# hkchengrex/Cutie

Measured on AMD Instinct MI355X. Metric: frames/sec (480p, 3 objects), higher is better.
Workload: dtype bf16

## Files before the change

### cutie_amd/_lib.py

```python
import ctypes
import os

_HERE = os.path.dirname(os.path.abspath(__file__))
LIB_PATH = os.environ.get('CUTIE_AMD_LIB') or os.path.join(_HERE, 'libcutie_hip.so')
ABI_VERSION = 11
OP_STRUCT_SIZE = 256

_lib = None


class HipLibraryError(RuntimeError):
    pass


def load():
    global _lib
    if _lib is not None:
        return _lib
    if not os.path.exists(LIB_PATH):
        raise HipLibraryError(
            f'{LIB_PATH} not found: build it with `python -c "import __graft_entry__ as g; g.build()"` '
            f'(or `make -C cutie_amd/csrc`).  cutie_amd has no CPU fallback.')
    lib = ctypes.CDLL(LIB_PATH)
    lib.cutie_exec.argtypes = [ctypes.c_void_p, ctypes.c_int, ctypes.c_void_p]
    lib.cutie_exec.restype = ctypes.c_int
    lib.cutie_exec_one.argtypes = [ctypes.c_void_p, ctypes.c_void_p]
    lib.cutie_exec_one.restype = ctypes.c_int
    lib.cutie_graph_capture.argtypes = [ctypes.c_void_p, ctypes.c_int, ctypes.c_void_p]
    lib.cutie_graph_capture.restype = ctypes.c_void_p
    lib.cutie_graph_launch.argtypes = [ctypes.c_void_p, ctypes.c_void_p]
    lib.cutie_graph_launch.restype = ctypes.c_int
    lib.cutie_graph_destroy.argtypes = [ctypes.c_void_p]
    lib.cutie_graph_destroy.restype = None
    lib.cutie_time_ops.argtypes = [ctypes.c_void_p, ctypes.c_int, ctypes.c_int, ctypes.c_void_p]
    lib.cutie_time_ops.restype = ctypes.c_float
    lib.cutie_hip_last_error.argtypes = []
    lib.cutie_hip_last_error.restype = ctypes.c_char_p
    lib.cutie_hip_abi_version.restype = ctypes.c_int
    lib.cutie_op_struct_size.restype = ctypes.c_int
    lib.cutie_hip_build_flags.restype = ctypes.c_int
    if lib.cutie_hip_abi_version() != ABI_VERSION or lib.cutie_op_struct_size() != OP_STRUCT_SIZE:
        raise HipLibraryError(f'{LIB_PATH} is stale (ABI {lib.cutie_hip_abi_version()}, '
                              f'op size {lib.cutie_op_struct_size()}); rebuild it.')
    _lib = lib
    return lib


EXPORTED_SYMBOLS = ['cutie_exec', 'cutie_exec_one', 'cutie_graph_capture', 'cutie_graph_launch',
                    'cutie_graph_destroy', 'cutie_time_ops', 'cutie_hip_last_error',
                    'cutie_hip_abi_version', 'cutie_op_struct_size', 'cutie_hip_build_flags']


def has_diag_kernels():
    return bool(load().cutie_hip_build_flags() & 1)


def has_png_decode():
    return bool(load().cutie_hip_build_flags() & 2)


def has_jpeg_batch():
    return bool(load().cutie_hip_build_flags() & 4)


def has_mixed_lockstep():
    return bool(load().cutie_hip_build_flags() & 8)


def has_track_stats():
    return bool(load().cutie_hip_build_flags() & 16)


class HipExecutor:
    is_mock = False

    def __init__(self):
        import torch
        self.lib = load()
        if not torch.cuda.is_available():
            raise HipLibraryError('no HIP device visible: cutie_amd runs on MI355X only (no CPU fallback).')
        self._torch = torch
        self._raw_stream = getattr(torch._C, '_cuda_getCurrentRawStream', None)
        self.graph_stats = [0, 0]
        self._warned = False

    def stream(self):
        raw = self._raw_stream
        if raw is not None:
            return raw(self._torch.cuda.current_device())
        return self._torch.cuda.current_stream().cuda_stream

    def run(self, arr):
        rc = self.lib.cutie_exec(arr.ctypes.data, len(arr), self.stream())
        if rc != 0:
            raise RuntimeError('cutie_exec failed: ' + self.lib.cutie_hip_last_error().decode())

    def run_on(self, arr, stream):
        rc = self.lib.cutie_exec(arr.ctypes.data, len(arr), stream.cuda_stream)
        if rc != 0:
            raise RuntimeError('cutie_exec failed: ' + self.lib.cutie_hip_last_error().decode())

    GRAPH_CACHE_ENTRIES = 24

    def run_cached(self, arr, cache, head=0):
        if head:
            self.run(arr[:head])
            arr = arr[head:]
        key = arr['p'].tobytes()
        ent = cache.get(key)
        if ent is None:
            if len(cache) >= self.GRAPH_CACHE_ENTRIES:
                old = cache.pop(next(iter(cache)))
                if old not in (0, -1):
                    self.lib.cutie_graph_destroy(old)
            cache[key] = 0
            self.graph_stats[0] += 1
            return self.run(arr)
        if ent == 0:
            ent = self.lib.cutie_graph_capture(arr.ctypes.data, len(arr), self.stream()) or -1
            cache[key] = ent
            if ent == -1 and not self._warned:
                self._warned = True
                import warnings
                warnings.warn('HIP graph capture of a launch plan failed (%s); such plans keep running launch by launch'
                              % self.lib.cutie_hip_last_error().decode())
        if ent == -1:
            self.graph_stats[0] += 1
            return self.run(arr)
        self.graph_stats[1] += 1
        if self.lib.cutie_graph_launch(ent, self.stream()) != 0:
            raise RuntimeError('cutie_graph_launch failed: ' + self.lib.cutie_hip_last_error().decode())

    def time_ops(self, arr, iters):
        ms = self.lib.cutie_time_ops(arr.ctypes.data, len(arr), iters, self.stream())
        if ms < 0:
            raise RuntimeError('cutie_time_ops failed: ' + self.lib.cutie_hip_last_error().decode())
        return ms


_executor = None


def get_executor():
    global _executor
    if _executor is None:
        _executor = HipExecutor()
    return _executor


def set_executor_for_testing(ex):
    global _executor
    _executor = ex
```

### cutie_amd/csrc/api.hip

```cpp
#include "common.h"
#include <stdarg.h>
#include <stdio.h>
#include <string.h>

static thread_local char g_err[512] = "";

void cutie_set_error(const char* fmt, ...) {
    va_list ap;
    va_start(ap, fmt);
    vsnprintf(g_err, sizeof(g_err), fmt, ap);
    va_end(ap);
}

static int dispatch(const cutie_op* op, hipStream_t s) {
    switch (op->kind) {
        case CUTIE_OP_CONV: return launch_conv(op, s);
        case CUTIE_OP_QUERY_INIT: return (op->flags & 1) ? launch_attention(op, s) : launch_elementwise(op, s);
        case CUTIE_OP_QFFN: return launch_qchain(op, s);
        case CUTIE_OP_STEM: return launch_stem(op, s);
        case CUTIE_OP_ATTN_Q2P: case CUTIE_OP_ATTN_SELF: case CUTIE_OP_ATTN_P2Q:
            return (op->flags & 12) ? launch_qchain(op, s) : launch_attention(op, s);
        case CUTIE_OP_AUX_MASK:
            return launch_attention(op, s);
        case CUTIE_OP_KEY_PREP: case CUTIE_OP_AFF_SCORE: case CUTIE_OP_AFF_SELECT: case CUTIE_OP_AFF_READOUT:
            return launch_affinity(op, s);
        case CUTIE_OP_RANK_SELECT: case CUTIE_OP_GATHER_ROWS: case CUTIE_OP_CONSOL_AFF: case CUTIE_OP_CONSOL_READ:
            return launch_bank(op, s);
        default:
            if (op->kind > 0 && op->kind < CUTIE_OP__COUNT) return launch_elementwise(op, s);
            cutie_set_error("cutie_exec: unknown op kind %d", op->kind);
            return -3;
    }
}

extern "C" {

int cutie_exec(const cutie_op* ops, int n, void* stream) {
    hipStream_t s = (hipStream_t)stream;
    for (int k = 0; k < n; ++k) {
        int rc = dispatch(&ops[k], s);
        if (rc != 0) {
            if (rc > 0) cutie_set_error("op %d (kind %d): HIP error %d (%s)", k, ops[k].kind, rc, hipGetErrorString((hipError_t)rc));
            else {
                char tmp[400];
                snprintf(tmp, sizeof(tmp), "%s", g_err);
                cutie_set_error("op %d (kind %d): %s", k, ops[k].kind, tmp);
            }
            return rc > 0 ? -1 : rc;
        }
    }
    return 0;
}

int cutie_exec_one(const cutie_op* op, void* stream) { return cutie_exec(op, 1, stream); }

struct GraphHandle { hipGraph_t graph; hipGraphExec_t exec; };

void* cutie_graph_capture(const cutie_op* ops, int n, void* stream) {
    (void)stream;
    static thread_local hipStream_t cap = nullptr;
    if (!cap && hipStreamCreateWithFlags(&cap, hipStreamNonBlocking) != hipSuccess) {
        cap = nullptr;
        (void)hipGetLastError();
        cutie_set_error("graph: cannot create the capture stream");
        return nullptr;
    }
    hipGraph_t graph = nullptr;
    if (hipStreamBeginCapture(cap, hipStreamCaptureModeThreadLocal) != hipSuccess) {
        (void)hipGetLastError();
        cutie_set_error("graph: begin capture failed");
        return nullptr;
    }
    int rc = cutie_exec(ops, n, (void*)cap);
    hipError_t e = hipStreamEndCapture(cap, &graph);
    if (rc != 0 || e != hipSuccess || !graph) {
        if (graph) hipGraphDestroy(graph);
        if (rc == 0) cutie_set_error("graph: end capture failed (%d)", (int)e);
        (void)hipGetLastError();
        return nullptr;
    }
    hipGraphExec_t exec = nullptr;
    if (hipGraphInstantiate(&exec, graph, nullptr, nullptr, 0) != hipSuccess) {
        hipGraphDestroy(graph);
        (void)hipGetLastError();
        cutie_set_error("graph: instantiate failed");
        return nullptr;
    }
    GraphHandle* h = new GraphHandle{graph, exec};
    return h;
}

int cutie_graph_launch(void* graph, void* stream) {
    GraphHandle* h = (GraphHandle*)graph;
    if (!h) { cutie_set_error("graph: null handle"); return -4; }
    hipError_t e = hipGraphLaunch(h->exec, (hipStream_t)stream);
    if (e != hipSuccess) { cutie_set_error("graph launch: %s", hipGetErrorString(e)); return -1; }
    return 0;
}

void cutie_graph_destroy(void* graph) {
    GraphHandle* h = (GraphHandle*)graph;
    if (!h) return;
    hipGraphExecDestroy(h->exec);
    hipGraphDestroy(h->graph);
    delete h;
}

float cutie_time_ops(const cutie_op* ops, int n, int iters, void* stream) {
    hipStream_t s = (hipStream_t)stream;
    hipEvent_t a, b;
    if (hipEventCreate(&a) != hipSuccess || hipEventCreate(&b) != hipSuccess) { cutie_set_error("time: event create failed"); return -1.f; }
    if (cutie_exec(ops, n, stream) != 0) return -1.f;
    hipEventRecord(a, s);
    for (int it = 0; it < iters; ++it)
        if (cutie_exec(ops, n, stream) != 0) return -1.f;
    hipEventRecord(b, s);
    hipEventSynchronize(b);
    float ms = 0.f;
    hipEventElapsedTime(&ms, a, b);
    hipEventDestroy(a);
    hipEventDestroy(b);
    return ms / (float)iters;
}

const char* cutie_hip_last_error(void) { return g_err; }
int cutie_hip_abi_version(void) { return 11; }
int cutie_op_struct_size(void) { return (int)sizeof(cutie_op); }
int cutie_hip_build_flags(void) {
    const int forms = 2 | 4 | 8 | 16;
#ifdef CUTIE_DIAG
    return forms | 1;
#else
    return forms;
#endif
}

}
```

### cutie_amd/csrc/common.h

```cpp
#pragma once
#include <hip/hip_runtime.h>
#include <stdint.h>
#include "../../include/cutie_hip.h"

typedef unsigned short bf16_t;
typedef __attribute__((ext_vector_type(8))) __bf16 bf16x8;
typedef __attribute__((ext_vector_type(4))) float f32x4;

__device__ __forceinline__ float bf2f(bf16_t v) { return __uint_as_float(((uint32_t)v) << 16); }

typedef __attribute__((ext_vector_type(2))) __bf16 bf16x2_t;
__device__ __forceinline__ bf16_t f2bf(float f) { return __builtin_bit_cast(bf16_t, (__bf16)f); }

__device__ __forceinline__ uint32_t pack_bf2(float a, float b) {
    const bf16x2_t v = {(__bf16)a, (__bf16)b};
    return __builtin_bit_cast(uint32_t, v);
}

__device__ __forceinline__ uint32_t relu_bf2(uint32_t w) {
    uint32_t neg = (w >> 15) & 0x00010001u;
    return w & ~(neg * 0xffffu);
}

__device__ __forceinline__ float sigmoidf_(float x) { return 1.0f / (1.0f + __expf(-x)); }

__device__ __forceinline__ float rows_max(float v) {
    unsigned u = __float_as_uint(v);
    auto r = __builtin_amdgcn_permlane16_swap(u, u, false, false);
    unsigned a = __float_as_uint(fmaxf(__uint_as_float(r[0]), __uint_as_float(r[1])));
    auto r2 = __builtin_amdgcn_permlane32_swap(a, a, false, false);
    return fmaxf(__uint_as_float(r2[0]), __uint_as_float(r2[1]));
}
__device__ __forceinline__ float rows_sum(float v) {
    unsigned u = __float_as_uint(v);
    auto r = __builtin_amdgcn_permlane16_swap(u, u, false, false);
    unsigned a = __float_as_uint(__uint_as_float(r[0]) + __uint_as_float(r[1]));
    auto r2 = __builtin_amdgcn_permlane32_swap(a, a, false, false);
    return __uint_as_float(r2[0]) + __uint_as_float(r2[1]);
}

__device__ __forceinline__ int wave_sum_i32(int v) {
    v += __builtin_amdgcn_update_dpp(0, v, 0xB1, 0xf, 0xf, false);
    v += __builtin_amdgcn_update_dpp(0, v, 0x4E, 0xf, 0xf, false);
    v += __builtin_amdgcn_update_dpp(0, v, 0x141, 0xf, 0xf, false);
    v += __builtin_amdgcn_update_dpp(0, v, 0x140, 0xf, 0xf, false);
    auto r = __builtin_amdgcn_permlane16_swap((unsigned)v, (unsigned)v, false, false);
    const unsigned a = r[0] + r[1];
    auto r2 = __builtin_amdgcn_permlane32_swap(a, a, false, false);
    return (int)(r2[0] + r2[1]);
}

__device__ __forceinline__ float wave_sum(float v) {
#pragma unroll
    for (int o = 32; o > 0; o >>= 1) v += __shfl_xor(v, o, 64);
    return v;
}
__device__ __forceinline__ float wave_sum_dpp(float v) {
    v += __uint_as_float(__builtin_amdgcn_update_dpp(0, (int)__float_as_uint(v), 0xB1, 0xf, 0xf, false));
    v += __uint_as_float(__builtin_amdgcn_update_dpp(0, (int)__float_as_uint(v), 0x4E, 0xf, 0xf, false));
    v += __uint_as_float(__builtin_amdgcn_update_dpp(0, (int)__float_as_uint(v), 0x141, 0xf, 0xf, false));
    v += __uint_as_float(__builtin_amdgcn_update_dpp(0, (int)__float_as_uint(v), 0x140, 0xf, 0xf, false));
    return rows_sum(v);
}
__device__ __forceinline__ float wave_max(float v) {
#pragma unroll
    for (int o = 32; o > 0; o >>= 1) v = fmaxf(v, __shfl_xor(v, o, 64));
    return v;
}

__host__ __device__ __forceinline__ int mixed_count(unsigned word, int clip) { return (int)((word >> (3 * clip)) & 7u); }
__host__ __device__ __forceinline__ int mixed_start(unsigned word, int clip) {
    int s = 0;
    for (int c = 0; c < clip; ++c) s += mixed_count(word, c);
    return s;
}
__host__ __device__ __forceinline__ int mixed_clip_of(unsigned word, int b, int& start) {
    int c = 0, s = 0;
#pragma unroll
    for (int q = 0; q < 7; ++q) {
        const int n = mixed_count(word, c);
        const bool past = b >= s + n;
        s += past ? n : 0;
        c += past ? 1 : 0;
    }
    start = s;
    return c;
}
static inline int mixed_clips(unsigned word, int* objects) {
    int n = 0, total = 0;
    if (word >> 24) { *objects = 0; return 0; }
    while (n < 8 && mixed_count(word, n)) total += mixed_count(word, n++);
    if (n < 8 && (word >> (3 * n))) { *objects = 0; return 0; }
    *objects = total;
    return n;
}

int launch_conv(const cutie_op* op, hipStream_t s);
int launch_elementwise(const cutie_op* op, hipStream_t s);
int launch_attention(const cutie_op* op, hipStream_t s);
int launch_stem(const cutie_op* op, hipStream_t s);
int launch_qchain(const cutie_op* op, hipStream_t s);
int launch_affinity(const cutie_op* op, hipStream_t s);
int launch_bank(const cutie_op* op, hipStream_t s);
int launch_resize_ingest(const cutie_op* op, hipStream_t s);
int launch_jpeg(const cutie_op* op, hipStream_t s);
int launch_png_decode(const cutie_op* op, hipStream_t s);
int launch_png_deflate(const cutie_op* op, int H, int W, hipStream_t s);
int launch_rle_encode(const cutie_op* op, hipStream_t s);
int launch_jf_counts(const cutie_op* op, hipStream_t s);
int launch_jpeg_encode(const cutie_op* op, hipStream_t s);
int launch_matte_composite(const cutie_op* op, hipStream_t s);
int launch_matte_soft(const cutie_op* op, hipStream_t s);
int launch_track_stats(const cutie_op* op, hipStream_t s);
void cutie_set_error(const char* fmt, ...);
```

### cutie_amd/csrc/conv_common.h

```cpp
#pragma once
#include "common.h"

struct ConvParams {
    const bf16_t* x1; const bf16_t* x2; const bf16_t* w; const float* bias; const bf16_t* res; void* y;
    int B, H, W, C1, C2, ldx1, ldx2, OH, OW, Cout, ldy, KH, KW, stride, pad, ldr, Kpad;
    int flags, M, Cin, OHW;
    float* part; int splitk, ldp, Kslice;
    long long* gap; unsigned long long* zero; int nzero;
    const unsigned char* pf; int pf_bytes;
    const unsigned char* pf2; int pf2_bytes;
    int res_grp_rows, res_grp_stride;
};
#define GAP_FIXED_SCALE 16777216.f
#define GAP_ELEM_SHIFT 4
__device__ __forceinline__ long long conv_gapfx(float v) {
    if (__builtin_expect(fabsf(v) < 2048.f, 1)) return (long long)__float2int_rn(v * 1048576.f);
    if (v != v) return 0;
    const float c = fminf(fmaxf(v, -1048576.f), 1048576.f);
    const float hi = truncf(c);
    return (long long)(int)hi * 1048576LL + (long long)__float2int_rn((c - hi) * 1048576.f);
}

typedef __attribute__((ext_vector_type(4))) unsigned int u32x4;
typedef const __attribute__((address_space(1))) u32x4* gptr16;
#define GLOAD16(ptr) (*(gptr16)(ptr))

template <int CPR>
__device__ __forceinline__ int swz(int row) {
    return CPR == 4 ? ((row >> 3) & 1) * 3 : (row & (CPR - 1));
}

__device__ __forceinline__ int conv_res_row(const ConvParams& p, int m) {
    if (!(p.flags & CUTIE_F_RES_BCAST)) return m;
    int r = m % p.OHW;
    if (p.res_grp_rows > 0) r += (m / p.res_grp_rows) * p.res_grp_stride;
    return r;
}

__device__ __forceinline__ void conv_finish(const ConvParams& p, float* v, int m, int ch0) {
    const int act = (p.flags >> CUTIE_ACT_SHIFT) & 7;
    const bool out_f32 = p.flags & CUTIE_F_OUT_F32;
    const bool vec_y = out_f32 ? ((p.ldy & 3) == 0) : ((p.ldy & 7) == 0);
    const bool vec_r = (p.ldr & 7) == 0;
    const bool full = ch0 + 7 < p.Cout;
    if (p.bias) {
        if (full && (reinterpret_cast<uintptr_t>(p.bias) & 15) == 0) {
            const float4 b0 = *reinterpret_cast<const float4*>(p.bias + ch0), b1 = *reinterpret_cast<const float4*>(p.bias + ch0 + 4);
            v[0] += b0.x; v[1] += b0.y; v[2] += b0.z; v[3] += b0.w; v[4] += b1.x; v[5] += b1.y; v[6] += b1.z; v[7] += b1.w;
        } else {
#pragma unroll
            for (int r = 0; r < 8; ++r) if (ch0 + r < p.Cout) v[r] += p.bias[ch0 + r];
        }
    }
    if (p.res) {
        const int mres = conv_res_row(p, m);
        const bf16_t* rp = p.res + (long)mres * p.ldr + ch0;
        if (full && vec_r) {
            const uint4 rr = *reinterpret_cast<const uint4*>(rp);
            v[0] += __uint_as_float(rr.x << 16); v[1] += __uint_as_float(rr.x & 0xffff0000u);
            v[2] += __uint_as_float(rr.y << 16); v[3] += __uint_as_float(rr.y & 0xffff0000u);
            v[4] += __uint_as_float(rr.z << 16); v[5] += __uint_as_float(rr.z & 0xffff0000u);
            v[6] += __uint_as_float(rr.w << 16); v[7] += __uint_as_float(rr.w & 0xffff0000u);
        } else {
#pragma unroll
            for (int r = 0; r < 8; ++r) if (ch0 + r < p.Cout) v[r] += bf2f(rp[r]);
        }
    }
#pragma unroll
    for (int r = 0; r < 8; ++r) {
        if (act == CUTIE_ACT_RELU) v[r] = fmaxf(v[r], 0.f);
        else if (act == CUTIE_ACT_SIGMOID) v[r] = sigmoidf_(v[r]);
        else if (act == CUTIE_ACT_SQ1) v[r] = v[r] * v[r] + 1.f;
    }
    if (out_f32) {
        float* yp = reinterpret_cast<float*>(p.y) + (long)m * p.ldy + ch0;
        if (full && vec_y) {
            *reinterpret_cast<float4*>(yp) = make_float4(v[0], v[1], v[2], v[3]);
            *reinterpret_cast<float4*>(yp + 4) = make_float4(v[4], v[5], v[6], v[7]);
        } else {
#pragma unroll
            for (int r = 0; r < 8; ++r) if (ch0 + r < p.Cout) yp[r] = v[r];
        }
    } else {
        bf16_t* yp = reinterpret_cast<bf16_t*>(p.y) + (long)m * p.ldy + ch0;
        if (full && vec_y) {
            *reinterpret_cast<uint4*>(yp) = make_uint4(pack_bf2(v[0], v[1]), pack_bf2(v[2], v[3]), pack_bf2(v[4], v[5]), pack_bf2(v[6], v[7]));
        } else {
#pragma unroll
            for (int r = 0; r < 8; ++r) if (ch0 + r < p.Cout) yp[r] = f2bf(v[r]);
        }
    }
}

template <int BM, int BN, int BK, int WK>
constexpr int conv_lds_bytes() {
    constexpr int pipe = WK * 2 * (BM + BN) * (BK / 8) * 16, epi = BM * (BN + 4) * 4;
    return pipe > epi ? pipe : epi;
}

__device__ __forceinline__ void conv_preload_args(const ConvParams& p) {
#ifndef CONV_NO_PRELOAD
    asm volatile("" :: "s"(p.x1), "s"(p.w), "s"(p.bias), "s"(p.res), "s"(p.y), "s"(p.zero),
                 "s"(p.B), "s"(p.H), "s"(p.W), "s"(p.C1), "s"(p.C2), "s"(p.ldx1), "s"(p.ldx2), "s"(p.OH), "s"(p.OW), "s"(p.Cout), "s"(p.ldy),
                 "s"(p.KH), "s"(p.KW), "s"(p.stride), "s"(p.pad), "s"(p.ldr), "s"(p.Kpad), "s"(p.flags), "s"(p.M), "s"(p.Cin), "s"(p.OHW),
                 "s"(p.nzero), "s"(gridDim.x), "s"(gridDim.y));
#endif
}

#ifdef CONV_TIMELINE
#define TL_MAX 96
#define TL_BYTES (16 * TL_MAX * 8)
#define TL_DECL(...) unsigned long long* const tlp_ = reinterpret_cast<unsigned long long*>(__VA_ARGS__) + wave * TL_MAX; int tln_ = 0;
#define TL_PUT_(ID, CAP) { if (tln_ < (CAP)) { const unsigned long long t_ = (__builtin_readcyclecounter() << 8) | (unsigned)(ID); if ((threadIdx.x & 63) == 0) tlp_[tln_] = t_; ++tln_; } }
#define TL(ID) TL_PUT_(ID, TL_MAX - 6)
#define TLE(ID) TL_PUT_(ID, TL_MAX)
#define TL_DUMP(LOGICAL, NB, NWAVES)                                                                                        \
    {                                                                                                                       \
        const int slot_ = (LOGICAL) == 0 ? 0 : (LOGICAL) == 1 ? 1 : (LOGICAL) == (NB) / 2 ? 2 : (LOGICAL) == (NB) - 1 ? 3 : -1; \
        if (slot_ >= 0 && p.part) {                                                                                         \
            __builtin_amdgcn_s_waitcnt(0);                                                                                  \
            unsigned long long* o_ = reinterpret_cast<unsigned long long*>(p.part) + ((long)slot_ * 16 + wave) * (TL_MAX + 2); \
            if ((threadIdx.x & 63) == 0) { o_[0] = 0x544c0000ull | (unsigned)tln_; o_[1] = ((unsigned long long)(LOGICAL) << 32) | (unsigned)(NWAVES); } \
            for (int q_ = threadIdx.x & 63; q_ < tln_; q_ += 64) o_[2 + q_] = tlp_[q_];                                     \
        }                                                                                                                   \
    }
#else
#define TL_BYTES 0
#define TL_DECL(...)
#define TL(ID)
#define TLE(ID)
#define TL_DUMP(LOGICAL, NB, NWAVES)
#endif

int launch_conv_dma(const ConvParams& p, int tile, hipStream_t s);
int launch_conv_pc(const ConvParams& p, int tile, hipStream_t s);
```

### cutie_amd/csrc/conv_igemm.hip

```cpp
#include "conv_common.h"

template <int BM, int BN, int WM, int WN, int BK, int S, int OCC, int WK>
__global__ __launch_bounds__(WM * WN * WK * 64) void conv_igemm_kernel(ConvParams p) {
    if (p.flags & CUTIE_F_PRIO) __builtin_amdgcn_s_setprio(1);
    constexpr int NTB = WM * WN * WK * 64;
    constexpr int NT = WM * WN * 64;
    constexpr int CPR = BK / 8;
    constexpr int RPT = NT / CPR;
    constexpr int NX = (BM * CPR) / NT;
    constexpr int NWC = (BN * CPR + NT - 1) / NT;
    constexpr int TM = BM / WM / 16;
    constexpr int TN = BN / WN / 16;
    constexpr int KSUB = BK / 32;
    constexpr int NWRAP = BK == 32 ? 4 : BK / 32;
    static_assert((NT == 256 || NT == 512) && NTB <= 1024 && NX >= 1 && TM >= 1 && TN >= 1 && S >= 2 && (BM * CPR) % NT == 0, "bad tile");
    constexpr int LDC = BN + 4;
    constexpr int GRP_CHUNKS = 2 * (BM + BN) * CPR;
    extern __shared__ __attribute__((aligned(16))) u32x4 smem_raw[];
    const int grp = threadIdx.x / NT;
    u32x4 (*smem)[(BM + BN) * CPR] = reinterpret_cast<u32x4 (*)[(BM + BN) * CPR]>(smem_raw + grp * GRP_CHUNKS);

    const int tid = threadIdx.x % NT, lane = tid & 63, wave = tid >> 6;
    int m0, n0;
    {
// ... 119 lines not shown
                afr[t] = __builtin_bit_cast(bf16x8, smem[buf][(BM + row) * CPR + ((j * 4 + l4) ^ swz<CPR>(row))]); \
            }                                                                                              \
            _Pragma("unroll") for (int a = 0; a < TN; ++a)                                                 \
                _Pragma("unroll") for (int b = 0; b < TM; ++b)                                             \
                    acc[a][b] = __builtin_amdgcn_mfma_f32_16x16x32_bf16(afr[a], bfr[b], acc[a][b], 0, 0, 0); \
        }                                                                                                  \
        if (DO_STORE) STORE_TILE(buf ^ 1, ((U) + 1) % S);                                                  \
        __syncthreads();                                                                                   \
    }
    int ks0 = 0;
    for (; ks0 + 2 * S - 1 <= nk; ks0 += S) {
#pragma unroll
        for (int u = 0; u < S; ++u) K_ITER(ks0 + u, u, true, true)
    }
    for (; ks0 < nk; ks0 += S) {
#pragma unroll
        for (int u = 0; u < S; ++u) {
            const int ks = ks0 + u;
            if (ks < nk) K_ITER(ks, u, ks + S - 1 < nk, ks + 1 < nk)
        }
    }

    float* ctile = reinterpret_cast<float*>(smem_raw);
#pragma unroll
    for (int g = WK - 1; g >= 0; --g) {
        if (grp == g) {
#pragma unroll
            for (int b = 0; b < TM; ++b)
#pragma unroll
                for (int a = 0; a < TN; ++a) {
                    const int px = pm0 + b * 16 + l15, ch = cn0 + a * 16 + l4 * 4;
                    f32x4* dst = reinterpret_cast<f32x4*>(ctile + px * LDC + ch);
                    if (g == WK - 1) *dst = acc[a][b];
                    else { f32x4 t = *dst; t[0] += acc[a][b][0]; t[1] += acc[a][b][1]; t[2] += acc[a][b][2]; t[3] += acc[a][b][3]; *dst = t; }
                }
        }
        __syncthreads();
    }
    constexpr int CH8 = BN / 8;
    if (p.splitk == 1) {
        for (int q = threadIdx.x; q < BM * CH8; q += NTB) {
            const int px = q / CH8, c8 = q - px * CH8;
            const int m = m0 + px, ch0 = n0 + c8 * 8;
            if (m >= p.M || ch0 >= p.Cout) continue;
            const f32x4 lo = *reinterpret_cast<const f32x4*>(ctile + px * LDC + c8 * 8);
            const f32x4 hi = *reinterpret_cast<const f32x4*>(ctile + px * LDC + c8 * 8 + 4);
            float v[8] = {lo[0], lo[1], lo[2], lo[3], hi[0], hi[1], hi[2], hi[3]};
            conv_finish(p, v, m, ch0);
        }
        return;
    }
    float* part = p.part + (long)blockIdx.z * p.M * p.ldp;
    for (int q = threadIdx.x; q < BM * CH8; q += NTB) {
        const int px = q / CH8, c8 = q - px * CH8;
        const int m = m0 + px, ch0 = n0 + c8 * 8;
        if (m >= p.M || ch0 >= p.Cout) continue;
        float* dst = part + (long)m * p.ldp + ch0;
        *reinterpret_cast<f32x4*>(dst) = *reinterpret_cast<const f32x4*>(ctile + px * LDC + c8 * 8);
        *reinterpret_cast<f32x4*>(dst + 4) = *reinterpret_cast<const f32x4*>(ctile + px * LDC + c8 * 8 + 4);
    }
}

__global__ __launch_bounds__(256) void conv_splitk_reduce_kernel(ConvParams p) {
    const int c8n = p.ldp >> 3;
    const long q = (long)blockIdx.x * 256 + threadIdx.x;
    if (q >= (long)p.M * c8n) return;
    const int m = (int)(q / c8n), ch0 = (int)(q - (long)m * c8n) * 8;
    float v[8] = {0.f, 0.f, 0.f, 0.f, 0.f, 0.f, 0.f, 0.f};
    for (int z = 0; z < p.splitk; ++z) {
        const float* src = p.part + ((long)z * p.M + m) * p.ldp + ch0;
        const f32x4 lo = *reinterpret_cast<const f32x4*>(src);
        const f32x4 hi = *reinterpret_cast<const f32x4*>(src + 4);
        v[0] += lo[0]; v[1] += lo[1]; v[2] += lo[2]; v[3] += lo[3];
        v[4] += hi[0]; v[5] += hi[1]; v[6] += hi[2]; v[7] += hi[3];
    }
    conv_finish(p, v, m, ch0);
}

__global__ __launch_bounds__(256) void conv_cout1_kernel(ConvParams p) {
    if (p.flags & CUTIE_F_PRIO) __builtin_amdgcn_s_setprio(1);
    extern __shared__ __attribute__((aligned(16))) unsigned char wlds_raw[];
    u32x4* wlds = reinterpret_cast<u32x4*>(wlds_raw);
    const int LP = p.Cin >> 3;
    const int ntap = p.KH * p.KW;
    const int ppb = 256 / LP;
    const int sub = threadIdx.x / LP, cl = threadIdx.x % LP;
    const int m = blockIdx.x * ppb + sub;
    const bool is33 = p.KH == 3 && p.KW == 3;
    const bool relu_in = p.flags & CUTIE_F_RELU_IN;
    const float bias0 = p.bias ? p.bias[0] : 0.f;
    u32x4 xv[9];
    float ok[9];
    if (is33) {
        const int mc = min(m, p.M - 1);
        const int b = mc / p.OHW, rem = mc - b * p.OHW, oh = rem / p.OW, ow = rem - oh * p.OW;
#pragma unroll
        for (int t = 0; t < 9; ++t) {
            const int ih = oh * p.stride - p.pad + t / 3, iw = ow * p.stride - p.pad + t % 3;
            const bool v = (unsigned)ih < (unsigned)p.H && (unsigned)iw < (unsigned)p.W;
            const int ihc = min(max(ih, 0), p.H - 1), iwc = min(max(iw, 0), p.W - 1);
            xv[t] = *reinterpret_cast<const u32x4*>(p.x1 + (((long)b * p.H + ihc) * p.W + iwc) * p.ldx1 + cl * 8);
            ok[t] = v ? 1.f : 0.f;
        }
    }
    for (int t = threadIdx.x; t < ntap * LP; t += 256) wlds[t] = *reinterpret_cast<const u32x4*>(p.w + (long)t * 8);
    __syncthreads();
    float acc = 0.f;
    if (m < p.M) {
        const int b = m / p.OHW, rem = m - b * p.OHW, oh = rem / p.OW, ow = rem - oh * p.OW;
        if (is33) {
#pragma unroll
            for (int t = 0; t < 9; ++t) {
                u32x4 x = xv[t];
                if (relu_in) { x.x = relu_bf2(x.x); x.y = relu_bf2(x.y); x.z = relu_bf2(x.z); x.w = relu_bf2(x.w); }
                const u32x4 wv = wlds[t * LP + cl];
                float a = 0.f;
#pragma unroll
                for (int i = 0; i < 4; ++i) {
                    a += __uint_as_float(x[i] << 16) * __uint_as_float(wv[i] << 16);
                    a += __uint_as_float(x[i] & 0xffff0000u) * __uint_as_float(wv[i] & 0xffff0000u);
                }
                acc += a * ok[t];
            }
        } else
        for (int kh = 0; kh < p.KH; ++kh) {
            const int ih = oh * p.stride - p.pad + kh;
            if ((unsigned)ih >= (unsigned)p.H) continue;
            for (int kw = 0; kw < p.KW; ++kw) {
                const int iw = ow * p.stride - p.pad + kw;
                if ((unsigned)iw >= (unsigned)p.W) continue;
                u32x4 xv = *reinterpret_cast<const u32x4*>(p.x1 + (((long)b * p.H + ih) * p.W + iw) * p.ldx1 + cl * 8);
                if (relu_in) { xv.x = relu_bf2(xv.x); xv.y = relu_bf2(xv.y); xv.z = relu_bf2(xv.z); xv.w = relu_bf2(xv.w); }
                const u32x4 wv = wlds[(kh * p.KW + kw) * LP + cl];
#pragma unroll
                for (int i = 0; i < 4; ++i) {
                    acc += __uint_as_float(xv[i] << 16) * __uint_as_float(wv[i] << 16);
                    acc += __uint_as_float(xv[i] & 0xffff0000u) * __uint_as_float(wv[i] & 0xffff0000u);
                }
            }
        }
    }
    for (int o = LP >> 1; o > 0; o >>= 1) acc += __shfl_xor(acc, o, 64);
    if (cl == 0 && m < p.M) {
        float v = acc + bias0;
        const int act = (p.flags >> CUTIE_ACT_SHIFT) & 7;
        if (act == CUTIE_ACT_RELU) v = fmaxf(v, 0.f);
        else if (act == CUTIE_ACT_SIGMOID) v = sigmoidf_(v);
        else if (act == CUTIE_ACT_SQ1) v = v * v + 1.f;
        if (p.flags & CUTIE_F_OUT_F32) reinterpret_cast<float*>(p.y)[(long)m * p.ldy] = v;
        else reinterpret_cast<bf16_t*>(p.y)[(long)m * p.ldy] = f2bf(v);
    }
}

template <int TR>
__global__ __launch_bounds__(256) void conv_cout1_tile_kernel(ConvParams p) {
    if (p.flags & CUTIE_F_PRIO) __builtin_amdgcn_s_setprio(1);
    static_assert(TR % 4 == 0, "rows per wave");
    constexpr int TC = 16, PW = TC + 2, NPIX = (TR + 2) * PW, RW = TR / 4;
    __shared__ u32x4 tile[NPIX * 16];
    const int tid = threadIdx.x, lane = tid & 63, wave = tid >> 6, n = lane & 15, g = lane >> 4;
    const int tiles_x = (p.W + TC - 1) / TC, tiles_y = (p.H + TR - 1) / TR;
    const int b = blockIdx.x / (tiles_x * tiles_y), rem = blockIdx.x - b * tiles_x * tiles_y;
    const int ty = rem / tiles_x, tx = rem - ty * tiles_x;
    const int x0 = tx * TC, y0 = ty * TR;
    const bool relu_in = p.flags & CUTIE_F_RELU_IN;
    const float bias0 = p.bias ? p.bias[0] : 0.f;
    __shared__ u32x4 wl[36 * 4];
    const u32x4 wmine = tid < 144 ? *reinterpret_cast<const u32x4*>(p.w + (long)((tid >> 4) * 16 + (tid & 15)) * 8) : (u32x4){0u, 0u, 0u, 0u};
    constexpr int NCH = (NPIX * 16 + 255) / 256;
    u32x4 st[NCH];
#pragma unroll
    for (int i = 0; i < NCH; ++i) {
        const int q = tid + 256 * i, px = q >> 4, c = q & 15;
        const int iy = y0 + px / PW - 1, ix = x0 + px % PW - 1;
        const bool in = q < NPIX * 16 && (unsigned)iy < (unsigned)p.H && (unsigned)ix < (unsigned)p.W;
        const long o = in ? (((long)b * p.H + iy) * p.W + ix) * p.ldx1 + c * 8 : 0;
        const u32x4 v = *reinterpret_cast<const u32x4*>(p.x1 + o);
        st[i] = in ? v : (u32x4){0u, 0u, 0u, 0u};
    }
#pragma unroll
    for (int i = 0; i < NCH; ++i) {
        const int q = tid + 256 * i, px = q >> 4, c = q & 15;
        u32x4 v = st[i];
        if (relu_in) { v.x = relu_bf2(v.x); v.y = relu_bf2(v.y); v.z = relu_bf2(v.z); v.w = relu_bf2(v.w); }
        if (q < NPIX * 16) tile[px * 16 + (c ^ (px & 15))] = v;
    }
    if (tid < 144) wl[tid] = wmine;
    __syncthreads();
    f32x4 acc[RW];
#pragma unroll
    for (int r = 0; r < RW; ++r) acc[r] = (f32x4){0.f, 0.f, 0.f, 0.f};
    const u32x4 zero4 = {0u, 0u, 0u, 0u};
#pragma unroll
    for (int sidx = 0; sidx < 36; ++sidx) {
        const int tap = sidx >> 2, ky = tap / 3, kx = tap - 3 * ky, ch = (sidx & 3) * 4 + g;
        const u32x4 wv = wl[sidx * 4 + g];
        const bf16x8 wb = __builtin_bit_cast(bf16x8, n == 0 ? wv : zero4);
#pragma unroll
        for (int r = 0; r < RW; ++r) {
            const int px = (wave * RW + r + ky) * PW + n + kx;
            const bf16x8 a = __builtin_bit_cast(bf16x8, tile[px * 16 + (ch ^ (px & 15))]);
            acc[r] = __builtin_amdgcn_mfma_f32_16x16x32_bf16(a, wb, acc[r], 0, 0, 0);
        }
    }
    if (n == 0) {
        const int act = (p.flags >> CUTIE_ACT_SHIFT) & 7;
#pragma unroll
        for (int r = 0; r < RW; ++r) {
            const int oy = y0 + wave * RW + r;
#pragma unroll
            for (int q = 0; q < 4; ++q) {
                const int x = x0 + 4 * g + q;
                if (x < p.W && oy < p.H) {
                    float v = acc[r][q] + bias0;
                    if (act == CUTIE_ACT_RELU) v = fmaxf(v, 0.f);
                    else if (act == CUTIE_ACT_SIGMOID) v = sigmoidf_(v);
                    else if (act == CUTIE_ACT_SQ1) v = v * v + 1.f;
                    const long m = ((long)b * p.H + oy) * p.W + x;
                    if (p.flags & CUTIE_F_OUT_F32) reinterpret_cast<float*>(p.y)[m * p.ldy] = v;
                    else reinterpret_cast<bf16_t*>(p.y)[m * p.ldy] = f2bf(v);
                }
            }
        }
    }
}

template <int R>
__global__ __launch_bounds__(256) void conv_cout1_rows_kernel(ConvParams p) {
    if (p.flags & CUTIE_F_PRIO) __builtin_amdgcn_s_setprio(1);
    const int LP = p.Cin >> 3;
    const int ppb = 256 / LP;
    const int sub = threadIdx.x / LP, cl = threadIdx.x % LP;
    const int tiles_x = (p.W + ppb - 1) / ppb, tiles_y = (p.H + R - 1) / R;
    const int b = blockIdx.x / (tiles_x * tiles_y), rem = blockIdx.x - b * tiles_x * tiles_y;
    const int ty = rem / tiles_x, tx = rem - ty * tiles_x;
    const int x = tx * ppb + sub, y0 = ty * R;
    const bool relu_in = p.flags & CUTIE_F_RELU_IN;
    const float bias0 = p.bias ? p.bias[0] : 0.f;
    u32x4 wv[9];
#pragma unroll
    for (int t = 0; t < 9; ++t) wv[t] = *reinterpret_cast<const u32x4*>(p.w + (long)(t * LP + cl) * 8);
    u32x4 xv[R + 2][3];
    float okc[3];
#pragma unroll
    for (int kx = 0; kx < 3; ++kx) okc[kx] = ((unsigned)(x + kx - 1) < (unsigned)p.W) ? 1.f : 0.f;
#pragma unroll
    for (int r = 0; r < R + 2; ++r) {
        const int iy = min(max(y0 + r - 1, 0), p.H - 1);
#pragma unroll
        for (int kx = 0; kx < 3; ++kx) {
            const int ix = min(max(x + kx - 1, 0), p.W - 1);
            xv[r][kx] = *reinterpret_cast<const u32x4*>(p.x1 + (((long)b * p.H + iy) * p.W + ix) * p.ldx1 + cl * 8);
        }
    }
    if (relu_in) {
#pragma unroll
        for (int r = 0; r < R + 2; ++r)
#pragma unroll
            for (int kx = 0; kx < 3; ++kx) { u32x4& v = xv[r][kx]; v.x = relu_bf2(v.x); v.y = relu_bf2(v.y); v.z = relu_bf2(v.z); v.w = relu_bf2(v.w); }
    }
    const int act = (p.flags >> CUTIE_ACT_SHIFT) & 7;
#pragma unroll
    for (int j = 0; j < R; ++j) {
        const int oy = y0 + j;
        float acc = 0.f;
#pragma unroll
        for (int ky = 0; ky < 3; ++ky) {
            const float okr = ((unsigned)(oy + ky - 1) < (unsigned)p.H) ? 1.f : 0.f;
#pragma unroll
            for (int kx = 0; kx < 3; ++kx) {
                const u32x4 xx = xv[j + ky][kx], ww = wv[ky * 3 + kx];
                float a = 0.f;
#pragma unroll
                for (int i = 0; i < 4; ++i) {
                    a += __uint_as_float(xx[i] << 16) * __uint_as_float(ww[i] << 16);
                    a += __uint_as_float(xx[i] & 0xffff0000u) * __uint_as_float(ww[i] & 0xffff0000u);
                }
                acc += a * (okr * okc[kx]);
            }
        }
        for (int o = LP >> 1; o > 0; o >>= 1) acc += __shfl_xor(acc, o, 64);
        if (cl == 0 && x < p.W && oy < p.H) {
            float v = acc + bias0;
            if (act == CUTIE_ACT_RELU) v = fmaxf(v, 0.f);
            else if (act == CUTIE_ACT_SIGMOID) v = sigmoidf_(v);
            else if (act == CUTIE_ACT_SQ1) v = v * v + 1.f;
            const long m = ((long)b * p.H + oy) * p.W + x;
            if (p.flags & CUTIE_F_OUT_F32) reinterpret_cast<float*>(p.y)[m * p.ldy] = v;
            else reinterpret_cast<bf16_t*>(p.y)[m * p.ldy] = f2bf(v);
        }
    }
}

template <int BM, int BN, int WM, int WN, int BK, int S, int OCC, int WK = 1>
static int launch_cfg(ConvParams p, hipStream_t s) {
    if (p.Kpad % BK) { cutie_set_error("conv: Kpad %d not a multiple of BK %d", p.Kpad, BK); return -2; }
    if (BK > 32 && p.Cin < 32) { cutie_set_error("conv: BK %d needs Cin >= 32 (Cin=%d)", BK, p.Cin); return -2; }
    const int nk_all = p.Kpad / BK;
    if (p.splitk > nk_all) { cutie_set_error("conv: splitk %d > K tiles %d", p.splitk, nk_all); return -2; }
    if (nk_all % (p.splitk * WK)) { cutie_set_error("conv: splitk %d x %d K groups must divide the %d K tiles", p.splitk, WK, nk_all); return -2; }
    p.Kslice = p.Kpad / p.splitk;
    constexpr int lds = conv_lds_bytes<BM, BN, BK, WK>();
    static bool attr_set = false;
    if (!attr_set) {
        if (lds > 65536 && hipFuncSetAttribute(reinterpret_cast<const void*>(conv_igemm_kernel<BM, BN, WM, WN, BK, S, OCC, WK>),
                                               hipFuncAttributeMaxDynamicSharedMemorySize, lds) != hipSuccess) {
            cutie_set_error("conv: cannot raise the dynamic LDS limit to %d bytes", lds);
            return -2;
        }
        attr_set = true;
    }
    dim3 grid((p.M + BM - 1) / BM, (p.Cout + BN - 1) / BN, p.splitk);
    hipLaunchKernelGGL((conv_igemm_kernel<BM, BN, WM, WN, BK, S, OCC, WK>), grid, dim3(WM * WN * WK * 64), lds, s, p);
    if (p.splitk > 1) {
        const long nq = (long)p.M * (p.ldp >> 3);
        hipLaunchKernelGGL(conv_splitk_reduce_kernel, dim3((unsigned)((nq + 255) / 256)), dim3(256), 0, s, p);
    }
    return (int)hipGetLastError();
}

int launch_conv(const cutie_op* op, hipStream_t s) {
    ConvParams p;
    p.x1 = (const bf16_t*)op->p[0]; p.x2 = (const bf16_t*)op->p[1]; p.w = (const bf16_t*)op->p[2];
    p.bias = (const float*)op->p[3]; p.res = (const bf16_t*)op->p[4]; p.y = (void*)op->p[5];
    const int32_t* i = op->i;
    p.B = i[0]; p.H = i[1]; p.W = i[2]; p.C1 = i[3]; p.C2 = i[4]; p.ldx1 = i[5]; p.ldx2 = i[6];
    p.OH = i[7]; p.OW = i[8]; p.Cout = i[9]; p.ldy = i[10]; p.KH = i[11]; p.KW = i[12];
    p.stride = i[13]; p.pad = i[14]; p.ldr = i[15]; p.Kpad = i[16];
    p.flags = op->flags; p.OHW = p.OH * p.OW; p.M = p.B * p.OHW; p.Cin = p.C1 + p.C2;
    p.splitk = i[19] > 1 ? i[19] : 1; p.part = (float*)op->p[6];
    p.ldp = (p.Cout + 7) & ~7;
    p.gap = (long long*)op->p[7]; p.zero = (unsigned long long*)op->p[8]; p.nzero = i[21];
    p.pf = (const unsigned char*)op->p[9]; p.pf_bytes = op->p[9] ? i[22] : 0;
    p.pf2 = (const unsigned char*)op->p[10]; p.pf2_bytes = op->p[10] ? i[23] : 0;
    p.res_grp_rows = p.res_grp_stride = 0;
    if ((p.flags & CUTIE_F_RES_BCAST) && op->f[0] > 0.f) {
        const int kg = (int)op->f[0];
        if (kg <= 0 || p.B % kg || op->f[1] < (float)p.OHW || op->f[1] != (float)(int)op->f[1]) { cutie_set_error("conv: residual groups of %d objects do not divide B = %d (or stride %g < OH*OW)", kg, p.B, (double)op->f[1]); return -2; }
        p.res_grp_rows = kg * p.OHW; p.res_grp_stride = (int)op->f[1];
    }
    if ((p.gap || p.zero) && (i[17] < 60 || i[17] >= 200 || ((p.flags & CUTIE_F_OUT_F32) && p.gap) || (p.Cout & 7) || (p.ldy & 7) || (p.res && (p.ldr & 7)))) {
        cutie_set_error("conv: GAP accumulation / zero job need an LDS-DMA tile (60..199), bf16 output, Cout %% 8 == 0 (tile %d)", i[17]);
        return -2;
    }
    if (p.splitk > 1 && (!p.part || (long)p.splitk * p.M * p.ldp > (long)i[20] * 1024)) {
        cutie_set_error("conv: split-K %d needs the fp32 partial scratch (p6, capacity i20 KiB-floats)", p.splitk);
        return -2;
    }
    if ((p.C1 & 7) || (p.C2 & 7) || (p.ldx1 & 7) || (p.C2 && (p.ldx2 & 7)) || (p.Kpad & 31) ||
        p.Kpad < p.KH * p.KW * p.Cin || p.M <= 0 || p.Cout <= 0) {
        cutie_set_error("conv: bad geometry C1=%d C2=%d ldx1=%d ldx2=%d Kpad=%d M=%d Cout=%d",
                        p.C1, p.C2, p.ldx1, p.ldx2, p.Kpad, p.M, p.Cout);
        return -2;
    }
    if (i[17] == 19) {
        const int LP = p.Cin >> 3;
        if (p.Cout != 1 || p.C2 != 0 || p.res || LP > 64 || (LP & (LP - 1)) || LP < 1) {
            cutie_set_error("conv cout1: needs Cout=1, single source, no residual, Cin/8 a power of two <= 64 (Cin=%d)", p.Cin);
            return -2;
        }
        const int ppb = 256 / LP;
        if (!(p.flags & CUTIE_F_PLAIN) && p.KH == 3 && p.KW == 3 && p.stride == 1 && p.pad == 1 && p.OH == p.H && p.OW == p.W && LP >= 8 && LP <= 32 && p.H * p.W >= 4096) {
            if (LP == 16 && !(p.flags & CUTIE_F_TILE_OFF)) {
                constexpr int TR = 8;
                const int blocks = p.B * ((p.H + TR - 1) / TR) * ((p.W + 15) / 16);
                hipLaunchKernelGGL(conv_cout1_tile_kernel<TR>, dim3(blocks), dim3(256), 0, s, p);
                return (int)hipGetLastError();
            }
            constexpr int R = 4;
            const int blocks = p.B * ((p.H + R - 1) / R) * ((p.W + ppb - 1) / ppb);
            hipLaunchKernelGGL(conv_cout1_rows_kernel<R>, dim3(blocks), dim3(256), 0, s, p);
            return (int)hipGetLastError();
        }
        hipLaunchKernelGGL(conv_cout1_kernel, dim3((p.M + ppb - 1) / ppb), dim3(256), (size_t)p.KH * p.KW * LP * 16, s, p);
        return (int)hipGetLastError();
    }
    if (i[17] >= 60 && i[17] < 90) return launch_conv_dma(p, i[17], s);
    if (i[17] >= 100 && i[17] < 200) return launch_conv_pc(p, i[17], s);
    switch (i[17]) {
        case 0: return launch_cfg<128, 128, 2, 2, 32, 4, 2>(p, s);
        case 1: return launch_cfg<128, 64, 2, 2, 32, 4, 3>(p, s);
        case 2: return launch_cfg<64, 64, 2, 2, 32, 4, 4>(p, s);
        case 3: return launch_cfg<256, 16, 4, 1, 32, 4, 3>(p, s);
        case 4: return launch_cfg<64, 128, 2, 2, 32, 4, 3>(p, s);
        case 5: return launch_cfg<64, 64, 2, 2, 64, 4, 3>(p, s);
        case 6: return launch_cfg<64, 128, 2, 2, 64, 3, 2>(p, s);
        case 7: return launch_cfg<128, 128, 2, 2, 64, 2, 2>(p, s);
        case 8: return launch_cfg<64, 64, 2, 2, 128, 3, 2>(p, s);
        case 9: return launch_cfg<32, 64, 2, 2, 64, 4, 4>(p, s);
        case 10: return launch_cfg<128, 64, 2, 2, 64, 3, 2>(p, s);
        case 11: return launch_cfg<32, 64, 2, 2, 128, 3, 3>(p, s);
        case 12: return launch_cfg<32, 128, 2, 2, 64, 3, 2>(p, s);
        case 13: return launch_cfg<64, 64, 2, 4, 64, 4, 5>(p, s);
        case 14: return launch_cfg<128, 64, 4, 2, 64, 4, 4>(p, s);
        case 15: return launch_cfg<64, 128, 2, 4, 64, 4, 4>(p, s);
        case 16: return launch_cfg<128, 128, 2, 4, 64, 3, 3>(p, s);
        case 17: return launch_cfg<64, 64, 2, 4, 128, 3, 4>(p, s);
        case 18: return launch_cfg<128, 128, 2, 4, 32, 4, 4>(p, s);
        case 20: return launch_cfg<64, 64, 2, 2, 64, 4, 3, 2>(p, s);
        case 21: return launch_cfg<64, 64, 2, 2, 128, 3, 2, 2>(p, s);
        case 22: return launch_cfg<32, 64, 2, 2, 128, 3, 3, 2>(p, s);
        case 23: return launch_cfg<128, 64, 2, 2, 64, 3, 2, 2>(p, s);
        case 24: return launch_cfg<64, 128, 2, 2, 64, 3, 2, 2>(p, s);
        case 25: return launch_cfg<128, 128, 2, 2, 64, 2, 2, 2>(p, s);
        case 26: return launch_cfg<32, 64, 2, 2, 64, 4, 4, 2>(p, s);
        case 27: return launch_cfg<64, 64, 2, 2, 64, 3, 3, 4>(p, s);
        case 28: return launch_cfg<32, 64, 2, 2, 64, 4, 4, 4>(p, s);
        case 29: return launch_cfg<64, 128, 2, 2, 32, 4, 3, 2>(p, s);
        case 30: return launch_cfg<64, 64, 2, 2, 32, 4, 4, 2>(p, s);
        default: cutie_set_error("conv: bad tile id %d", i[17]); return -2;
    }
}
```

### cutie_amd/csrc/elementwise.hip

```cpp
#include "common.h"
#include <math.h>

#define GRID1D(n, bs) dim3((unsigned)(((long)(n) + (bs) - 1) / (bs)))
__global__ void memset32_kernel(uint32_t* d, long n, uint32_t v);

__global__ void maxpool_kernel(const uint4* __restrict__ x, uint4* __restrict__ y, int B, int H, int W, int C8,
                               int OH, int OW, int relu) {
    long idx = (long)blockIdx.x * blockDim.x + threadIdx.x;
    long total = (long)B * OH * OW * C8;
    if (idx >= total) return;
    int c = idx % C8; long t = idx / C8;
    int ow = t % OW; t /= OW; int oh = t % OH; int b = t / OH;
    float m[8];
#pragma unroll
    for (int i = 0; i < 8; ++i) m[i] = relu ? 0.f : -INFINITY;
    for (int dy = 0; dy < 3; ++dy) {
        int ih = oh * 2 - 1 + dy;
        if ((unsigned)ih >= (unsigned)H) continue;
        for (int dx = 0; dx < 3; ++dx) {
            int iw = ow * 2 - 1 + dx;
            if ((unsigned)iw >= (unsigned)W) continue;
            uint4 v = x[(((long)b * H + ih) * W + iw) * C8 + c];
            uint32_t u[4] = {v.x, v.y, v.z, v.w};
#pragma unroll
            for (int i = 0; i < 4; ++i) {
                m[2 * i] = fmaxf(m[2 * i], __uint_as_float(u[i] << 16));
                m[2 * i + 1] = fmaxf(m[2 * i + 1], __uint_as_float(u[i] & 0xffff0000u));
            }
        }
    }
    y[idx] = make_uint4(pack_bf2(m[0], m[1]), pack_bf2(m[2], m[3]), pack_bf2(m[4], m[5]), pack_bf2(m[6], m[7]));
}

__global__ void img_prep_kernel(const float* __restrict__ img, const float* __restrict__ masks, uint4* __restrict__ y,
                                int h0, int w0, int H, int W, int pl, int pt, int K,
                                float m0, float m1, float m2, float s0, float s1, float s2) {
    long idx = (long)blockIdx.x * blockDim.x + threadIdx.x;
    long HW = (long)H * W;
    if (idx >= HW * K) return;
    int k = idx / HW; long pix = idx - (long)k * HW;
    int yy = pix / W, xx = pix - (long)yy * W;
    int sy = yy - pt, sx = xx - pl;
    float r = 0.f, g = 0.f, b = 0.f;
    if ((unsigned)sy < (unsigned)h0 && (unsigned)sx < (unsigned)w0) {
        long o = (long)sy * w0 + sx, plane = (long)h0 * w0;
        r = img[o]; g = img[plane + o]; b = img[2 * plane + o];
    }
    r = (r - m0) / s0; g = (g - m1) / s1; b = (b - m2) / s2;
    float mk = 0.f, others = 0.f;
    if (masks) {
        float sum = 0.f;
        for (int j = 0; j < K; ++j) sum += masks[(long)j * HW + pix];
        mk = masks[(long)k * HW + pix];
        others = fminf(fmaxf(sum - mk, 0.f), 1.f);
    }
    y[idx] = make_uint4(pack_bf2(r, g), pack_bf2(b, mk), pack_bf2(others, 0.f), 0u);
}

__device__ __forceinline__ void up_coord(int o, int n_in, float scale, int& i0, int& i1, float& lam) {
    float src = ((float)o + 0.5f) * scale - 0.5f;
    if (src < 0.f) src = 0.f;
    i0 = (int)src;
    if (i0 > n_in - 1) i0 = n_in - 1;
    i1 = i0 + (i0 < n_in - 1 ? 1 : 0);
    lam = src - (float)i0;
}

template <bool MIXED = false>
__global__ void upsample2x_add_kernel(const uint4* __restrict__ g, const uint4* __restrict__ skip, uint4* __restrict__ y,
                                      int B, int h, int w, int C8, int Kg, long gstride, int prio) {
    if (prio) __builtin_amdgcn_s_setprio(1);
    long idx = (long)blockIdx.x * blockDim.x + threadIdx.x;
    int OH = 2 * h, OW = 2 * w;
    long total = (long)B * OH * OW * C8;
    if (idx >= total) return;
    int c = idx % C8; long t = idx / C8;
    int ox = t % OW; t /= OW; int oy = t % OH; int b = t / OH;
    int y0, y1, x0, x1; float ly, lx;
    up_coord(oy, h, 0.5f, y0, y1, ly);
    up_coord(ox, w, 0.5f, x0, x1, lx);
    const uint4* gb = g + (long)b * h * w * C8;
    uint4 v00 = gb[((long)y0 * w + x0) * C8 + c], v01 = gb[((long)y0 * w + x1) * C8 + c];
    uint4 v10 = gb[((long)y1 * w + x0) * C8 + c], v11 = gb[((long)y1 * w + x1) * C8 + c];
    long grp;
    if (MIXED) { int st; grp = mixed_clip_of((unsigned)Kg, b, st); }
    else grp = Kg > 0 ? b / Kg : 0;
    uint4 sk = skip[(grp * gstride + (long)oy * OW + ox) * C8 + c];
    const uint32_t* a = &v00.x; const uint32_t* bq = &v01.x; const uint32_t* cq = &v10.x; const uint32_t* d = &v11.x;
    const uint32_t* s = &sk.x;
    float w00 = (1.f - ly) * (1.f - lx), w01 = (1.f - ly) * lx, w10 = ly * (1.f - lx), w11 = ly * lx;
    uint32_t out[4];
#pragma unroll
    for (int i = 0; i < 4; ++i) {
        float lo = w00 * __uint_as_float(a[i] << 16) + w01 * __uint_as_float(bq[i] << 16) +
                   w10 * __uint_as_float(cq[i] << 16) + w11 * __uint_as_float(d[i] << 16) + __uint_as_float(s[i] << 16);
        float hi = w00 * __uint_as_float(a[i] & 0xffff0000u) + w01 * __uint_as_float(bq[i] & 0xffff0000u) +
                   w10 * __uint_as_float(cq[i] & 0xffff0000u) + w11 * __uint_as_float(d[i] & 0xffff0000u) +
                   __uint_as_float(s[i] & 0xffff0000u);
        out[i] = pack_bf2(lo, hi);
    }
    y[idx] = make_uint4(out[0], out[1], out[2], out[3]);
}

template <int R = 0>
__device__ __forceinline__ void area_down_bf16_body(const bf16_t* __restrict__ x, bf16_t* __restrict__ y, int B, int H, int W, int C,
                                                    int ldx, int ldy, int rrt, long idx) {
    const int r = R > 0 ? R : rrt;
    int C8 = C >> 3, OH = H / r, OW = W / r;
    long total = (long)B * OH * OW * C8;
    if (idx >= total) return;
    int c = idx % C8; long t = idx / C8;
    int ox = t % OW; t /= OW; int oy = t % OH; int b = t / OH;
    float acc[8] = {0, 0, 0, 0, 0, 0, 0, 0};
    if (R > 0) {
        uint4 v[R > 0 ? R * R : 1];
#pragma unroll
        for (int dy = 0; dy < R; ++dy)
#pragma unroll
            for (int dx = 0; dx < R; ++dx)
                v[dy * R + dx] = *reinterpret_cast<const uint4*>(x + (((long)b * H + oy * R + dy) * W + ox * R + dx) * ldx + c * 8);
#pragma unroll
        for (int e = 0; e < R * R; ++e) {
            const uint32_t* u = &v[e].x;
#pragma unroll
            for (int i = 0; i < 4; ++i) {
                acc[2 * i] += __uint_as_float(u[i] << 16);
                acc[2 * i + 1] += __uint_as_float(u[i] & 0xffff0000u);
            }
        }
    } else
    for (int dy = 0; dy < r; ++dy)
        for (int dx = 0; dx < r; ++dx) {
            const uint4 v = *reinterpret_cast<const uint4*>(x + (((long)b * H + oy * r + dy) * W + ox * r + dx) * ldx + c * 8);
            const uint32_t* u = &v.x;
#pragma unroll
            for (int i = 0; i < 4; ++i) {
                acc[2 * i] += __uint_as_float(u[i] << 16);
                acc[2 * i + 1] += __uint_as_float(u[i] & 0xffff0000u);
            }
        }
    float inv = 1.f / (float)(r * r);
    uint4 o = make_uint4(pack_bf2(acc[0] * inv, acc[1] * inv), pack_bf2(acc[2] * inv, acc[3] * inv),
                         pack_bf2(acc[4] * inv, acc[5] * inv), pack_bf2(acc[6] * inv, acc[7] * inv));
    *reinterpret_cast<uint4*>(y + (((long)b * OH + oy) * OW + ox) * ldy + c * 8) = o;
}
__global__ void area_down_bf16_kernel(const bf16_t* __restrict__ x, bf16_t* __restrict__ y, int B, int H, int W, int C,
                                      int ldx, int ldy, int r) {
    area_down_bf16_body(x, y, B, H, W, C, ldx, ldy, r, (long)blockIdx.x * blockDim.x + threadIdx.x);
}

template <int R = 0>
__device__ __forceinline__ void area_down_f32_body(const float* __restrict__ x, bf16_t* __restrict__ y, int B, int H, int W, int C,
                                                   int ldx, int ldy, int rrt, int Cz, long idx) {
    const int r = R > 0 ? R : rrt;
    int OH = H / r, OW = W / r;
    long total = (long)B * OH * OW;
    if (idx >= total) return;
    int ox = idx % OW; long t = idx / OW; int oy = t % OH; int b = t / OH;
    float inv = 1.f / (float)(r * r);
    bf16_t* yp = y + idx * ldy;
    for (int c = 0; c < C; ++c) {
        float acc = 0.f;
        if (R > 0) {
            float v[R > 0 ? R * R : 1];
#pragma unroll
            for (int dy = 0; dy < R; ++dy)
#pragma unroll
                for (int dx = 0; dx < R; ++dx) v[dy * R + dx] = x[(((long)b * H + oy * R + dy) * W + ox * R + dx) * ldx + c];
#pragma unroll
            for (int e = 0; e < R * R; ++e) acc += v[e];
        } else
        for (int dy = 0; dy < r; ++dy)
            for (int dx = 0; dx < r; ++dx) acc += x[(((long)b * H + oy * r + dy) * W + ox * r + dx) * ldx + c];
        yp[c] = f2bf(acc * inv);
    }
    for (int c = C; c < Cz; ++c) yp[c] = 0;
}
__global__ void area_down_f32_kernel(const float* __restrict__ x, bf16_t* __restrict__ y, int B, int H, int W, int C,
                                     int ldx, int ldy, int r, int Cz) {
    area_down_f32_body(x, y, B, H, W, C, ldx, ldy, r, Cz, (long)blockIdx.x * blockDim.x + threadIdx.x);
}
struct AreaSeg { const void* x; bf16_t* y; int B, H, W, C, ldx, ldy, r, Cz, f32; long n; };
struct Area3 { AreaSeg s[3]; int rt; int prio; };
__global__ void area_down3_kernel(Area3 a) {
    const int prio = a.prio;
    if (prio) __builtin_amdgcn_s_setprio(1);
    long idx = (long)blockIdx.x * blockDim.x + threadIdx.x;
#pragma unroll
    for (int q = 0; q < 3; ++q) {
        const AreaSeg& g = a.s[q];
        if (idx < g.n) {
            const int rr = a.rt ? 0 : g.r;
            if (g.f32) {
                if (rr == 2) area_down_f32_body<2>((const float*)g.x, g.y, g.B, g.H, g.W, g.C, g.ldx, g.ldy, 2, g.Cz, idx);
                else if (rr == 4) area_down_f32_body<4>((const float*)g.x, g.y, g.B, g.H, g.W, g.C, g.ldx, g.ldy, 4, g.Cz, idx);
                else area_down_f32_body<0>((const float*)g.x, g.y, g.B, g.H, g.W, g.C, g.ldx, g.ldy, g.r, g.Cz, idx);
            } else {
                if (rr == 2) area_down_bf16_body<2>((const bf16_t*)g.x, g.y, g.B, g.H, g.W, g.C, g.ldx, g.ldy, 2, idx);
                else if (rr == 4) area_down_bf16_body<4>((const bf16_t*)g.x, g.y, g.B, g.H, g.W, g.C, g.ldx, g.ldy, 4, idx);
                else area_down_bf16_body<0>((const bf16_t*)g.x, g.y, g.B, g.H, g.W, g.C, g.ldx, g.ldy, g.r, idx);
            }
            return;
        }
        idx -= g.n;
    }
}

__global__ void mask_down_mean_kernel(const float* __restrict__ m, float* __restrict__ m16, int K, int H, int W, int r) {
    int h = H / r, w = W / r;
    long idx = (long)blockIdx.x * (blockDim.x >> 6) + (threadIdx.x >> 6);
    int lane = threadIdx.x & 63;
    if (idx >= (long)K * h * w) return;
    int ox = idx % w; long t = idx / w; int oy = t % h; int k = t / h;
    float acc = 0.f;
    for (int e = lane; e < r * r; e += 64) {
        int dy = e / r, dx = e - dy * r;
        acc += m[((long)k * H + oy * r + dy) * W + ox * r + dx];
    }
    acc = wave_sum(acc);
    if (lane == 0) m16[idx] = acc / (float)(r * r);
}
__global__ void mask_down_pair_kernel(const float* __restrict__ m, float* __restrict__ m16, uint4* __restrict__ y, int K, int H, int W, int r,
                                      int ld8) {
    const int h = H / r, w = W / r, hw = h * w;
    const long px = (long)blockIdx.x * (blockDim.x >> 6) + (threadIdx.x >> 6);
    const int lane = threadIdx.x & 63;
    if (px >= hw) return;
    const int ox = px % w, oy = px / w;
    float sum = 0.f;
    for (int k0 = 0; k0 < K; k0 += 4) {
        float acc[4] = {0.f, 0.f, 0.f, 0.f};
        for (int e = lane; e < r * r; e += 64) {
            const int dy = e / r, dx = e - dy * r;
            float v[4];
#pragma unroll
            for (int u = 0; u < 4; ++u) v[u] = m[((long)min(k0 + u, K - 1) * H + oy * r + dy) * W + ox * r + dx];
#pragma unroll
            for (int u = 0; u < 4; ++u) acc[u] += v[u];
        }
#pragma unroll
        for (int u = 0; u < 4; ++u) {
            if (k0 + u >= K) break;
            const float a = wave_sum(acc[u]) / (float)(r * r);
            sum += a;
            if (lane == 0) m16[(long)(k0 + u) * hw + px] = a;
        }
    }
    if (lane == 0)
        for (int k = 0; k < K; ++k) {
            const float mk = m16[(long)k * hw + px];
            const float others = fminf(fmaxf(sum - mk, 0.f), 1.f);
            y[((long)k * hw + px) * ld8] = make_uint4(pack_bf2(mk, others), 0u, 0u, 0u);
        }
}
__global__ void mask_pair_kernel(const float* __restrict__ m16, uint4* __restrict__ y, int K, int hw) {
    long idx = (long)blockIdx.x * blockDim.x + threadIdx.x;
    if (idx >= (long)K * hw) return;
    int k = idx / hw; int p = idx - (long)k * hw;
    float sum = 0.f;
    for (int j = 0; j < K; ++j) sum += m16[(long)j * hw + p];
    float mk = m16[idx];
    float others = fminf(fmaxf(sum - mk, 0.f), 1.f);
    y[idx] = make_uint4(pack_bf2(mk, others), 0u, 0u, 0u);
}

__global__ __launch_bounds__(256) void gap_partial_kernel(const bf16_t* __restrict__ x, float* __restrict__ part, int HW, int C) {
    __shared__ float red[2048 + 32];
    const int b = blockIdx.y, p0 = blockIdx.x * 64;
    const int C8 = C >> 3;
    const int c8 = threadIdx.x % C8, rg = threadIdx.x / C8, nrg = 256 / C8;
    float acc[8] = {0, 0, 0, 0, 0, 0, 0, 0};
    for (int r = rg; r < 64; r += nrg) {
        int p = p0 + r;
        if (p < HW) {
            uint4 v = *reinterpret_cast<const uint4*>(x + ((long)b * HW + p) * C + c8 * 8);
            acc[0] += __uint_as_float(v.x << 16); acc[1] += __uint_as_float(v.x & 0xffff0000u);
            acc[2] += __uint_as_float(v.y << 16); acc[3] += __uint_as_float(v.y & 0xffff0000u);
            acc[4] += __uint_as_float(v.z << 16); acc[5] += __uint_as_float(v.z & 0xffff0000u);
            acc[6] += __uint_as_float(v.w << 16); acc[7] += __uint_as_float(v.w & 0xffff0000u);
        }
    }
#pragma unroll
    for (int i = 0; i < 8; ++i) red[rg * (C + 1) + c8 * 8 + i] = acc[i];
    __syncthreads();
    for (int c = threadIdx.x; c < C; c += 256) {
        float sum = 0.f;
        for (int g = 0; g < nrg; ++g) sum += red[g * (C + 1) + c];
        part[((long)b * gridDim.x + blockIdx.x) * C + c] = sum;
    }
}
__global__ void gap_final_kernel(const float* __restrict__ part, float* __restrict__ y, int nchunk, int C, float inv) {
    const int b = blockIdx.x;
    for (int c = threadIdx.x; c < C; c += blockDim.x) {
        float sum = 0.f;
        for (int k = 0; k < nchunk; ++k) sum += part[((long)b * nchunk + k) * C + c];
        y[(long)b * C + c] = sum * inv;
    }
}
// ... 913 lines not shown
    const float v = alpha * src[r * slds + (W - 1 - x)];
    float* d = dst + r * dlds + x;
    *d = beta != 0.f ? v + beta * *d : v;
}

template <typename OUT>
__global__ void prob_to_id_kernel(const float* __restrict__ prob, const int* __restrict__ lut, OUT* __restrict__ out,
                                  int P, int H, int W, long plane, int ldrow) {
    const long idx = (long)blockIdx.x * blockDim.x + threadIdx.x;
    if (idx >= (long)H * W) return;
    const int yy = (int)(idx / W), xx = (int)(idx - (long)yy * W);
    const float* src = prob + (long)yy * ldrow + xx;
    float best = src[0];
    int arg = 0;
    for (int q = 1; q < P; ++q) {
        const float v = src[(long)q * plane];
        if (v > best) { best = v; arg = q; }
    }
    out[idx] = (OUT)lut[arg];
}

template <typename OUT>
__global__ void prob_to_id_resample_kernel(const float* __restrict__ prob, const int* __restrict__ lut, OUT* __restrict__ out,
                                           int P, int H, int W, int OH, int OW, long plane, int ldrow, int packed) {
    const int OW4 = (OW + 3) >> 2;
    const long idx = (long)blockIdx.x * blockDim.x + threadIdx.x;
    if (idx >= (long)OH * OW4) return;
    const int oy = (int)(idx / OW4), ox0 = (int)(idx - (long)oy * OW4) * 4;
    const float sy = (float)H / (float)OH, sx = (float)W / (float)OW;
    const float fy = fmaxf((oy + 0.5f) * sy - 0.5f, 0.f);
    const int y0 = min((int)fy, H - 1), y1 = min(y0 + 1, H - 1);
    const float ly = fy - (float)y0;
    int x0[4], x1[4];
    float lx[4], best[4];
    int arg[4];
#pragma unroll
    for (int k = 0; k < 4; ++k) {
        const int ox = min(ox0 + k, OW - 1);
        const float fx = fmaxf((ox + 0.5f) * sx - 0.5f, 0.f);
        x0[k] = min((int)fx, W - 1);
        x1[k] = min(x0[k] + 1, W - 1);
        lx[k] = fx - (float)x0[k];
        arg[k] = 0;
    }
    for (int q = 0; q < P; ++q) {
        const float* r0 = prob + (long)q * plane + (long)y0 * ldrow;
        const float* r1 = prob + (long)q * plane + (long)y1 * ldrow;
#pragma unroll
        for (int k = 0; k < 4; ++k) {
            const float a = r0[x0[k]], b = r0[x1[k]], cc = r1[x0[k]], d = r1[x1[k]];
            const float v = (1.f - ly) * ((1.f - lx[k]) * a + lx[k] * b) + ly * ((1.f - lx[k]) * cc + lx[k] * d);
            if (q == 0) best[k] = v;
            else if (v > best[k]) { best[k] = v; arg[k] = q; }
        }
    }
    OUT* o = out + (long)oy * OW + ox0;
    if constexpr (sizeof(OUT) == 1) {
        if (packed) {
            *(uint32_t*)o = (uint32_t)(uint8_t)lut[arg[0]] | (uint32_t)(uint8_t)lut[arg[1]] << 8 | (uint32_t)(uint8_t)lut[arg[2]] << 16 |
                            (uint32_t)(uint8_t)lut[arg[3]] << 24;
            return;
        }
    } else {
        if (packed) {
            *(int4*)o = make_int4(lut[arg[0]], lut[arg[1]], lut[arg[2]], lut[arg[3]]);
            return;
        }
    }
#pragma unroll
    for (int k = 0; k < 4; ++k)
        if (ox0 + k < OW) o[k] = (OUT)lut[arg[k]];
}

template <typename OUT>
__global__ void prob_to_id_merge_kernel(const uint64_t* __restrict__ srcs, const int4* __restrict__ geom, const int* __restrict__ lut,
                                        OUT* __restrict__ out, int S, int P, int OH, int OW, int packed) {
    const int OW4 = (OW + 3) >> 2;
    const long idx = (long)blockIdx.x * blockDim.x + threadIdx.x;
    if (idx >= (long)OH * OW4) return;
    const int oy = (int)(idx / OW4), ox0 = (int)(idx - (long)oy * OW4) * 4;
    int best[4], arg[4];
#pragma unroll
    for (int k = 0; k < 4; ++k) { best[k] = 0; arg[k] = 0; }
    for (int q = 0; q < P; ++q) {
        int sum[4] = {0, 0, 0, 0};
        for (int sI = 0; sI < S; ++sI) {
            const int4 g = geom[sI];
            const int H = g.x, W = g.y;
            if (H < 1 || W < 1) continue;
            const float* prob = (const float*)srcs[sI] + (long)q * g.z;
            const float sy = (float)H / (float)OH, sx = (float)W / (float)OW;
            const float fy = fmaxf((oy + 0.5f) * sy - 0.5f, 0.f);
            const int y0 = min((int)fy, H - 1), y1 = min(y0 + 1, H - 1);
            const float ly = fy - (float)y0;
            const float* r0 = prob + (long)y0 * g.w;
            const float* r1 = prob + (long)y1 * g.w;
#pragma unroll
            for (int k = 0; k < 4; ++k) {
                const int ox = min(ox0 + k, OW - 1);
                const float fx = fmaxf((ox + 0.5f) * sx - 0.5f, 0.f);
                const int x0 = min((int)fx, W - 1), x1 = min(x0 + 1, W - 1);
                const float lx = fx - (float)x0;
                const float a = r0[x0], b = r0[x1], cc = r1[x0], d = r1[x1];
                const float v = (1.f - ly) * ((1.f - lx) * a + lx * b) + ly * ((1.f - lx) * cc + lx * d);
                sum[k] += (int)(uint8_t)(int)(v * 255.f);
            }
        }
#pragma unroll
        for (int k = 0; k < 4; ++k)
            if (q == 0 || sum[k] > best[k]) { best[k] = sum[k]; arg[k] = q; }
    }
    OUT* o = out + (long)oy * OW + ox0;
    if constexpr (sizeof(OUT) == 1) {
        if (packed) {
            *(uint32_t*)o = (uint32_t)(uint8_t)lut[arg[0]] | (uint32_t)(uint8_t)lut[arg[1]] << 8 | (uint32_t)(uint8_t)lut[arg[2]] << 16 |
                            (uint32_t)(uint8_t)lut[arg[3]] << 24;
            return;
        }
    } else {
        if (packed) {
            *(int4*)o = make_int4(lut[arg[0]], lut[arg[1]], lut[arg[2]], lut[arg[3]]);
            return;
        }
    }
#pragma unroll
    for (int k = 0; k < 4; ++k)
        if (ox0 + k < OW) o[k] = (OUT)lut[arg[k]];
}

int launch_elementwise(const cutie_op* op, hipStream_t s) {
    const int32_t* i = op->i;
    const uint64_t* p = op->p;
    const int BS = 256;
    const int PRIO = (op->flags & CUTIE_F_PRIO) ? 1 : 0;
    switch (op->kind) {
        case CUTIE_OP_MAXPOOL: {
            int C8 = i[3] / 8;
            long n = (long)i[0] * i[4] * i[5] * C8;
            hipLaunchKernelGGL(maxpool_kernel, GRID1D(n, BS), dim3(BS), 0, s, (const uint4*)p[0], (uint4*)p[1], i[0], i[1], i[2], C8, i[4], i[5], op->flags & 1);
            break;
        }
        case CUTIE_OP_IMG_PREP: {
            int K = p[1] ? i[6] : 1;
            long n = (long)i[2] * i[3] * K;
            hipLaunchKernelGGL(img_prep_kernel, GRID1D(n, BS), dim3(BS), 0, s, (const float*)p[0], (const float*)p[1], (uint4*)p[2],
                               i[0], i[1], i[2], i[3], i[4], i[5], K, op->f[0], op->f[1], op->f[2], op->f[3], op->f[4], op->f[5]);
            break;
        }
        case CUTIE_OP_UPSAMPLE2X_ADD: {
            int C8 = i[3] / 8;
            long n = (long)i[0] * 4 * i[1] * i[2] * C8;
            if (i[6]) {
                int objs; const int nc = mixed_clips((unsigned)i[6], &objs);
                if (nc < 1 || objs != i[0] || i[4] != 0 || i[5] < 4 * i[1] * i[2]) { cutie_set_error("upsample2x_add (mixed form): the counts 0x%x do not add up to B = %d (or i4 != 0, or the stride is below one map)", i[6], i[0]); return -2; }
                hipLaunchKernelGGL(upsample2x_add_kernel<true>, GRID1D(n, BS), dim3(BS), 0, s, (const uint4*)p[0], (const uint4*)p[1], (uint4*)p[2], i[0], i[1], i[2], C8, i[6], (long)i[5], PRIO);
                break;
            }
            if (i[4] < 0 || (i[4] > 0 && (i[0] % i[4] || i[5] < 4 * i[1] * i[2]))) { cutie_set_error("upsample2x_add: skip groups of %d objects do not divide B = %d (or their stride is below one map)", i[4], i[0]); return -2; }
            hipLaunchKernelGGL(upsample2x_add_kernel<false>, GRID1D(n, BS), dim3(BS), 0, s, (const uint4*)p[0], (const uint4*)p[1], (uint4*)p[2], i[0], i[1], i[2], C8, i[4], (long)i[5], PRIO);
            break;
        }
        case CUTIE_OP_AREA_DOWN: {
            int r = i[6];
            long np = (long)i[0] * (i[1] / r) * (i[2] / r);
            if (op->flags & 1)
                hipLaunchKernelGGL(area_down_f32_kernel, GRID1D(np, BS), dim3(BS), 0, s, (const float*)p[0], (bf16_t*)p[1], i[0], i[1], i[2], i[3], i[4], i[5], r, i[7]);
            else
                hipLaunchKernelGGL(area_down_bf16_kernel, GRID1D(np * (i[3] / 8), BS), dim3(BS), 0, s, (const bf16_t*)p[0], (bf16_t*)p[1], i[0], i[1], i[2], i[3], i[4], i[5], r);
            break;
        }
        case CUTIE_OP_AREA_DOWN3: {
            Area3 a;
            long total = 0;
            for (int q = 0; q < 3; ++q) {
                const int32_t* j = i + 8 * q;
                AreaSeg& g = a.s[q];
                g.x = (const void*)p[2 * q]; g.y = (bf16_t*)p[2 * q + 1];
                g.B = j[0]; g.H = j[1]; g.W = j[2]; g.C = j[3]; g.ldx = j[4]; g.ldy = j[5]; g.r = j[6]; g.Cz = j[7];
                g.f32 = (op->flags >> q) & 1;
                if (g.r < 1 || (!g.f32 && (g.C & 7))) { cutie_set_error("area_down3: segment %d: r >= 1, C %% 8 for bf16 input", q); return -2; }
                const long np = (long)g.B * (g.H / g.r) * (g.W / g.r);
                g.n = g.f32 ? np : np * (g.C / 8);
                total += g.n;
            }
            a.rt = (op->flags >> 3) & 1;
            a.prio = PRIO;
            hipLaunchKernelGGL(area_down3_kernel, GRID1D(total, BS), dim3(BS), 0, s, a);
            break;
        }
        case CUTIE_OP_MASK_DOWN: {
            int K = i[0], r = i[3], h = i[1] / r, w = i[2] / r;
            long n = (long)K * h * w;
            float* m16 = (float*)p[2];
            if (!m16) { cutie_set_error("mask_down: m16 buffer required"); return -2; }
            hipLaunchKernelGGL(mask_down_pair_kernel, GRID1D((long)h * w * 64, BS), dim3(BS), 0, s, (const float*)p[0], m16, (uint4*)p[1], K, i[1], i[2], r,
                               i[4] > 8 ? i[4] / 8 : 1);
            break;
        }
        case CUTIE_OP_GAP: {
            if (i[2] > 256 || (i[2] & 7) || 256 % (i[2] / 8)) { cutie_set_error("gap: C must divide 256 octet-wise (C=%d)", i[2]); return -2; }
            if (!p[2]) { cutie_set_error("gap: scratch buffer required"); return -2; }
            int nchunk = (i[1] + 63) / 64;
            hipLaunchKernelGGL(gap_partial_kernel, dim3(nchunk, i[0]), dim3(256), 0, s, (const bf16_t*)p[0], (float*)p[2], i[1], i[2]);
            if (!(op->flags & 1))
                hipLaunchKernelGGL(gap_final_kernel, dim3(i[0]), dim3(256), 0, s, (const float*)p[2], (float*)p[1], nchunk, i[2], 1.f / (float)i[1]);
            break;
        }
        case CUTIE_OP_ECA_APPLY: {
            if (i[2] > 256 || (i[2] & 7)) { cutie_set_error("eca: C <= 256, C %% 8"); return -2; }
            if (p[6] && (i[2] != 256 || !p[8])) { cutie_set_error("eca: the fused 1x1 head needs C = 256 and an output"); return -2; }
            int nchunk = (i[1] + 63) / 64;
            hipLaunchKernelGGL(eca_apply_kernel, dim3((i[1] + 31) / 32, i[0]), dim3(256), 0, s, (const bf16_t*)p[0], (const float*)p[5], (const float*)p[2],
                               (const bf16_t*)p[3], (bf16_t*)p[4], (float*)p[1], i[1], i[2], nchunk, (op->flags & 1) ? (const long long*)p[5] : nullptr,
                               (const bf16_t*)p[6], (const float*)p[7], (float*)p[8], PRIO);
            break;
        }
        case CUTIE_OP_GRU: {
            long n = (long)i[0] * i[1];
            if (!(op->flags & 1) && (i[1] & 3) == 0 && (((uintptr_t)p[0] | (uintptr_t)p[1]) & 15) == 0 && ((uintptr_t)p[2] & 7) == 0)
                hipLaunchKernelGGL(gru4_kernel, GRID1D(n / 4, BS), dim3(BS), 0, s, (const float*)p[0], (float*)p[1], (bf16_t*)p[2], (long)i[0], i[1], PRIO);
            else
                hipLaunchKernelGGL(gru_kernel, GRID1D(n, BS), dim3(BS), 0, s, (const float*)p[0], (float*)p[1], (bf16_t*)p[2], (long)i[0], i[1]);
            break;
        }
        case CUTIE_OP_SEG_AGG:
            hipLaunchKernelGGL(seg_agg_kernel, GRID1D(i[1], BS), dim3(BS), 0, s, (const float*)p[0], (float*)p[1], i[0], i[1]);
            break;
        case CUTIE_OP_UP4_SOFTMAX: {
            long n = (long)16 * i[1] * i[2];
            if (op->flags & 1) {
                if (i[0] > 16) { cutie_set_error("up4_softmax: the fused form holds P <= 16 planes in registers (P=%d)", i[0]); return -2; }
                const bool vec = !(op->flags & 2) && i[0] <= 8 && (((uintptr_t)p[1] | (uintptr_t)p[2]) & 15) == 0;
                const int nclip = i[4] > 1 ? i[4] : 1;
                if (nclip > 1 && !vec) { cutie_set_error("up4_softmax: several clips per launch need the four-pixel form (P <= 8, aligned outputs)"); return -2; }
                if (i[5]) {
                    int objs; const int nc = mixed_clips((unsigned)i[5], &objs);
                    if (nc < 1 || nc != i[4] || !vec || (op->flags & 8)) { cutie_set_error("up4_softmax (mixed form): %d clips in the counts 0x%x, i4 = %d; needs the four-pixel form with compile-time object counts", nc, i[5], i[4]); return -2; }
                    if (op->flags & 4) {
                        if (!p[3] || !p[4] || (i[1] & 3) || (i[2] & 3) || i[3] < 8 || (i[3] & 7)) { cutie_set_error("up4_softmax: the mask-down form needs h, w multiples of 4, m16 and pair"); return -2; }
                        const int ncell = (i[1] / 4) * (i[2] / 4);
                        if (op->flags & 16)
                            hipLaunchKernelGGL((up4_softmax_md_mixed_kernel<8, false>), dim3((ncell + 3) / 4, nc), dim3(256), 0, s, (const float*)p[0], (float*)p[1], (float*)p[2], (unsigned)i[5],
                                               i[1], i[2], (float*)p[3], (uint4*)p[4], i[3] / 8, PRIO);
                        else
                            hipLaunchKernelGGL((up4_softmax_md_mixed_kernel<8, true>), dim3((ncell + 3) / 4, nc), dim3(256), 0, s, (const float*)p[0], (float*)p[1], (float*)p[2], (unsigned)i[5],
                                               i[1], i[2], (float*)p[3], (uint4*)p[4], i[3] / 8, PRIO);
                    } else {
                        const long n4 = (long)4 * i[1] * i[2];
                        hipLaunchKernelGGL(up4_softmax_fused4_mixed_kernel<8>, dim3((unsigned)((n4 + BS - 1) / BS), nc), dim3(BS), 0, s, (const float*)p[0], (float*)p[1], (float*)p[2], (unsigned)i[5], i[1], i[2], PRIO);
                    }
                    break;
                }
                if (op->flags & 4) {
                    if (!vec || !p[3] || !p[4] || (i[1] & 3) || (i[2] & 3) || i[3] < 8 || (i[3] & 7)) { cutie_set_error("up4_softmax: the mask-down form needs P <= 8, h, w multiples of 4, m16 and pair"); return -2; }
                    const int ncell = (i[1] / 4) * (i[2] / 4);
#define UP4_MD_(KC, SH) hipLaunchKernelGGL((up4_softmax_md_kernel<8, KC, SH>), dim3((ncell + 3) / 4, nclip), dim3(256), 0, s, (const float*)p[0], (float*)p[1], (float*)p[2], i[0] - 1, \
                                       i[1], i[2], (float*)p[3], (uint4*)p[4], i[3] / 8, PRIO)
#define UP4_MD(KC) { if (op->flags & 16) UP4_MD_(KC, false); else UP4_MD_(KC, true); }
                    switch ((op->flags & 8) ? 0 : i[0] - 1) {
                        case 1: UP4_MD(1); break; case 2: UP4_MD(2); break; case 3: UP4_MD(3); break; case 4: UP4_MD(4); break;
                        case 5: UP4_MD(5); break; case 6: UP4_MD(6); break; case 7: UP4_MD(7); break; default: UP4_MD(0); break;
                    }
#undef UP4_MD
#undef UP4_MD_
                    break;
                }
                if (vec) {
                    const long n4 = (long)4 * i[1] * i[2];
#define UP4_F4(KC) hipLaunchKernelGGL((up4_softmax_fused4_kernel<8, KC>), dim3((unsigned)((n4 + BS - 1) / BS), nclip), dim3(BS), 0, s, (const float*)p[0], (float*)p[1], (float*)p[2], i[0] - 1, i[1], i[2], PRIO)
                    switch ((op->flags & 8) ? 0 : i[0] - 1) {
                        case 1: UP4_F4(1); break; case 2: UP4_F4(2); break; case 3: UP4_F4(3); break; case 4: UP4_F4(4); break;
                        case 5: UP4_F4(5); break; case 6: UP4_F4(6); break; case 7: UP4_F4(7); break; default: UP4_F4(0); break;
                    }
#undef UP4_F4
                    break;
                }
                if (i[0] <= 8) hipLaunchKernelGGL(up4_softmax_fused_kernel<8>, GRID1D(n, BS), dim3(BS), 0, s, (const float*)p[0], (float*)p[1], (float*)p[2], i[0] - 1, i[1], i[2]);
                else hipLaunchKernelGGL(up4_softmax_fused_kernel<16>, GRID1D(n, BS), dim3(BS), 0, s, (const float*)p[0], (float*)p[1], (float*)p[2], i[0] - 1, i[1], i[2]);
                break;
            }
            hipLaunchKernelGGL(up4_softmax_kernel, GRID1D(n, BS), dim3(BS), 0, s, (const float*)p[0], (float*)p[1], (float*)p[2], i[0], i[1], i[2]);
            break;
        }
        case CUTIE_OP_MASK_MERGE: {
            long n = (long)i[2] * i[3];
            hipLaunchKernelGGL(mask_merge_kernel, GRID1D(n, BS), dim3(BS), 0, s, (const void*)p[0], (const float*)p[1], (const int*)p[2], (float*)p[3],
                               i[0], i[1], i[2], i[3], i[4], i[5], i[6], i[7], i[8], op->flags & 1);
            break;
        }
        case CUTIE_OP_AGG_SOFTMAX:
            hipLaunchKernelGGL(agg_softmax_kernel, GRID1D(i[1], BS), dim3(BS), 0, s, (const float*)p[0], (float*)p[1], i[0], (long)i[1]);
            break;
        case CUTIE_OP_LINEAR: {
            if ((i[2] & 7) || (i[3] & 3) || i[2] < 256) { cutie_set_error("linear: Kd %% 8, ldx %% 4, Kd >= 256 required (Kd=%d)", i[2]); return -2; }
            const int add_rows = i[5] > 0 ? i[5] : 1;
            const bool ln = op->flags & 2;
            if (ln && (i[2] != 256 || !p[6] || !p[7] || (i[3] & 3))) { cutie_set_error("linear: fused LayerNorm needs Kd == 256, gamma and beta"); return -2; }
            if ((ln || i[6] > 0) && (i[2] & 127)) { cutie_set_error("linear: LayerNorm / add_cols need Kd %% 128 == 0"); return -2; }
            if (i[6] > 0 && (i[6] & 15)) { cutie_set_error("linear: add_cols must be a multiple of 16"); return -2; }
            if ((i[2] & 511) == 0 && i[2] >= 1024 && !ln)
                hipLaunchKernelGGL(linear_mfma_kernel<16>, dim3((i[1] + 15) / 16, (i[0] + 15) / 16), dim3(1024), 0, s, (const float*)p[0], (const float*)p[1], (const bf16_t*)p[2],
                                   (const float*)p[3], (const float*)p[4], (float*)p[5], i[0], i[1], i[2], i[3], i[4], add_rows, op->flags & 1, i[6],
                                   (const float*)nullptr, (const float*)nullptr, (float*)nullptr, 1e-5f);
            else if ((i[2] & 127) == 0)
                hipLaunchKernelGGL(linear_mfma_kernel<4>, dim3((i[1] + 15) / 16, (i[0] + 15) / 16), dim3(256), 0, s, (const float*)p[0], (const float*)p[1], (const bf16_t*)p[2],
                                   (const float*)p[3], (const float*)p[4], (float*)p[5], i[0], i[1], i[2], i[3], i[4], add_rows, op->flags & 1, i[6],
                                   ln ? (const float*)p[6] : nullptr, (const float*)p[7], (float*)p[8], op->f[0] > 0.f ? op->f[0] : 1e-5f);
            else if (i[2] >= 512)
                hipLaunchKernelGGL(linear_small_kernel<64>, dim3((i[1] + 3) / 4, (i[0] + 15) / 16), dim3(256), 0, s, (const float*)p[0], (const float*)p[1], (const bf16_t*)p[2],
                                   (const float*)p[3], (const float*)p[4], (float*)p[5], i[0], i[1], i[2], i[3], i[4], add_rows, op->flags & 1);
            else
                hipLaunchKernelGGL(linear_small_kernel<32>, dim3((i[1] + 7) / 8, (i[0] + 15) / 16), dim3(256), 0, s, (const float*)p[0], (const float*)p[1], (const bf16_t*)p[2],
// ... 157 lines not shown
```

### cutie_amd/model/plans.py

```python
import math
import os

import numpy as np
import torch

from .. import _lib
from .. import ops as O
from ..ops import Dyn
from .param_spec import resnet_layers

BF16, F32 = torch.bfloat16, torch.float32


class Act:
    __slots__ = ('t', 'B', 'H', 'W', 'C', 'ld')

    def __init__(self, t, B, H, W, C, ld=None):
        self.t, self.B, self.H, self.W, self.C, self.ld = t, B, H, W, C, (C if ld is None else ld)


def positional_encoding(h, w, dim_total, scale, temperature):
    dim = int(math.ceil(dim_total / 4) * 2)
    inv_freq = 1.0 / (temperature ** (torch.arange(0, dim, 2).float() / dim))
    py = torch.arange(h, dtype=torch.float32)
    px = torch.arange(w, dtype=torch.float32)
    py = py / (py[-1] + 1e-6) * scale
    px = px / (px[-1] + 1e-6) * scale
    sy, sx = py[:, None] * inv_freq[None], px[:, None] * inv_freq[None]
    ey = torch.stack((sy.sin(), sy.cos()), -1).flatten(-2)
    ex = torch.stack((sx.sin(), sx.cos()), -1).flatten(-2)
    emb = torch.zeros(h, w, dim * 2)
    emb[:, :, :dim] = ex[None]
    emb[:, :, dim:] = ey[:, None]
    return emb


TILE_CACHE_ENV = 'CUTIE_AMD_TILE_CACHE'
TUNE_REPS, TUNE_ITERS = (int(v) for v in os.environ.get('CUTIE_AMD_TUNE', '3x8').lower().split('x'))


GRAPHS = os.environ.get('CUTIE_AMD_GRAPHS', '0') not in ('', '0')
GRAPH_MIN_OPS = 8
QINIT_SKIP = os.environ.get('CUTIE_AMD_QINIT_SKIP', '1') not in ('', '0')
AUTOTUNE = os.environ.get('CUTIE_AMD_AUTOTUNE', '0') not in ('', '0')
PACKAGED_TILES = os.path.join(os.path.dirname(os.path.abspath(__file__)), '..', 'tiles_gfx950.json')


def load_tile_cache():
    import json
    path = os.environ.get(TILE_CACHE_ENV)
    if path == 'none':
        return {}
    cache = {}
    for f in (PACKAGED_TILES, path):
        if f and os.path.exists(f):
            try:
                cache.update({tuple(k): tuple(v) for k, v in json.load(open(f))['tiles']})
            except Exception:
                pass
    return cache


def save_tile_cache(cache):
    import json
    path = os.environ.get(TILE_CACHE_ENV)
    if not path or path == 'none':
        return
    tmp = path + '.tmp%d' % os.getpid()
    with open(tmp, 'w') as f:
        json.dump({'tiles': [[list(k), list(v)] for k, v in cache.items()]}, f)
    os.replace(tmp, path)


ARENA_POISON = os.environ.get('CUTIE_AMD_ARENA_POISON', '0') not in ('', '0')
ARENA_ALIGN = 256


class Arena:

    def __init__(self, device):
        self.device = device
        self.tensor = None
        self.size = 0
        self.plans = []

    def require(self, nbytes):
        if nbytes <= self.size:
            return
        self.size = -(-int(nbytes * 1.1) // (1 << 20)) * (1 << 20)
        if self.tensor is not None:
            self._old = [self.tensor]
        self.tensor = torch.zeros(self.size, dtype=torch.uint8, device=self.device)
        for p in self.plans:
            p.rebind_arena()

    def base(self):
        return self.tensor.data_ptr()


_USE_COUNT = getattr(torch._C, '_storage_Use_Count', None)


def _storage_users(t):
    return _USE_COUNT(t.untyped_storage()._cdata) - 2


class SlotPool:
    SLOTS = int(os.environ.get('CUTIE_AMD_POOL_SLOTS', '6'))

    IDLE_FRAMES = int(os.environ.get('CUTIE_AMD_POOL_IDLE', '512'))

    def __init__(self):
        self.groups = {}
        self.last_used = {}
        self.frame = 0
        self.offset = 0

    def tick(self):
        self.frame += 1
        if self.frame % 64 == 0 and self.IDLE_FRAMES > 0:
            for k in [k for k, f in self.last_used.items() if self.frame - f > self.IDLE_FRAMES]:
                self.groups.pop(k, None)
                del self.last_used[k]

    @staticmethod
    def _make_slot(specs, dev):
        names = tuple(specs)
        tensors = [torch.zeros(sh, dtype=dt, device=dev) for (sh, dt, z) in specs.values()]
        stores = [t.untyped_storage() for t in tensors]
        return names, tensors, stores, [st._cdata for st in stores]

    @staticmethod
    def _free(slot):
        for c in slot[3]:
            if _USE_COUNT(c) != 2:
                return False
        return True

    @staticmethod
    def _hand_out(slot):
        return {nm: t.detach() for nm, t in zip(slot[0], slot[1])}

    def get(self, key, specs, dev):
        if self.SLOTS <= 0 or _USE_COUNT is None:
            return {n: (torch.zeros if z else torch.empty)(sh, dtype=dt, device=dev) for n, (sh, dt, z) in specs.items()}
        slots = self.groups.get(key)
        if slots is None:
            slots = self.groups[key] = {}
        self.last_used[key] = self.frame
        i = (self.frame + self.offset) % self.SLOTS
        slot = slots.get(i)
        if slot is None:
            slot = slots[i] = self._make_slot(specs, dev)
        if self._free(slot):
            return self._hand_out(slot)
        return {n: (torch.zeros if z else torch.empty)(sh, dtype=dt, device=dev) for n, (sh, dt, z) in specs.items()}

    def get_ring(self, key, specs, dev, ring=3):
        if self.SLOTS <= 0 or _USE_COUNT is None:
            return {n: (torch.zeros if z else torch.empty)(sh, dtype=dt, device=dev) for n, (sh, dt, z) in specs.items()}
        slots = self.groups.setdefault(key, {'next': 0})
        self.last_used[key] = self.frame
        i = slots['next'] % ring
        slots['next'] = i + 1
        slot = slots.get(i)
        if slot is None:
            slot = slots[i] = self._make_slot(specs, dev)
        if self._free(slot):
            return self._hand_out(slot)
        return {n: (torch.zeros if z else torch.empty)(sh, dtype=dt, device=dev) for n, (sh, dt, z) in specs.items()}


def weights_go_cold(px16, K=None):
    return 1400 <= px16 < 4500 if K is None else 4800 <= px16 * (1 + K) < 18000


class Plan:
    def __init__(self, eng, touch=True, prio=True):
        self.eng = eng
        self.prio = prio
        self.dev = eng.device
        self.ol = O.OpList(scratch_owner=eng, touch_next_weights=touch, prio=prio)
        self.bufs = {}
        self.meta = {}
        self.tuned = False
        self.persistent = set()
        self.arena = None
        self._arena_slots = []
        self._arena_views = {}
        self._graphs = {}
        self.korder_ref = 0
        self.mixed = None
        self.kref = {}

    def buf(self, name, shape, dtype=BF16, persistent=False):
        assert name not in self.bufs, name
        t = torch.zeros(tuple(int(s) for s in shape), dtype=dtype, device=self.dev)
        self.bufs[name] = t
        if persistent:
            self.persistent.add(name)
        return t

    def pack_into(self, arena):
        arr = self.ol.finalize()
        ptrs = arr['p'].astype(np.int64)
        items = []
        for name, t in self.bufs.items():
            if name in self.persistent or t.numel() == 0:
                continue
            base, nbytes = t.data_ptr(), t.numel() * t.element_size()
            hit = (ptrs >= base) & (ptrs < base + nbytes)
            if not hit.any():
                continue
            rows = np.nonzero(hit.any(axis=1))[0]
            items.append(dict(name=name, base=base, nbytes=nbytes, first=int(rows[0]), last=int(rows[-1]), hit=hit, t=t))
        items.sort(key=lambda b: (b['first'], -b['nbytes']))
        placed = []
        total = 0
        for b in items:
            size = -(-b['nbytes'] // ARENA_ALIGN) * ARENA_ALIGN
            live = sorted((o, e) for (o, e, last) in placed if last >= b['first'])
            off = 0
            for o, e in live:
                if off + size <= o:
                    break
                off = max(off, e)
            b['off'] = off
            placed.append((off, off + size, b['last']))
            total = max(total, off + size)
        self.arena = arena
        self._arena_slots = []
        for b in items:
            idx, slot = np.nonzero(b['hit'])
            for i, sl in zip(idx, slot):
                self._arena_slots.append((int(i), int(sl), b['off'] + int(ptrs[i, sl] - b['base'])))
            self._arena_views[b['name']] = (b['off'], tuple(b['t'].shape), b['t'].dtype)
        self.ol.keep = [k for k in self.ol.keep if not any(k is b['t'] for b in items)]
        arena.plans.append(self)
        arena.require(total)
        self.rebind_arena()
        self.meta['arena_bytes'] = total
        self.meta['unpacked_bytes'] = sum(b['nbytes'] for b in items)

    def rebind_arena(self):
        if self.arena is None or self.arena.tensor is None:
            return
        base = self.arena.base()
        p = self.ol.arr['p']
        for (i, sl, off) in self._arena_slots:
            p[i, sl] = base + off
            self.ol.recs[i][4][sl] = base + off
        for name, (off, shape, dtype) in self._arena_views.items():
            n = int(np.prod(shape)) * torch.empty((), dtype=dtype).element_size()
            self.bufs[name] = self.arena.tensor[off:off + n].view(dtype).view(shape)

    graph_head = 0

    def run(self, **dyn):
        if not self.tuned:
            self.tuned = True
            self.autotune_convs(**dyn)
        if ARENA_POISON and self.arena is not None and self.arena.tensor is not None:
            self.arena.tensor.fill_(0xFF)
        ol = self.ol
        ex = _lib.get_executor()
        if GRAPHS and len(ol.recs) >= GRAPH_MIN_OPS and hasattr(ex, 'run_cached'):
            if ol.arr is None:
                ol.finalize()
            if dyn:
                ol.bind(**dyn)
            ex.run_cached(ol.arr, self._graphs, self.graph_head)
        else:
            ol.run(**dyn)

    def run_part(self, lo, hi, first=True, **dyn):
        if not self.tuned:
            self.tuned = True
            self.autotune_convs(**dyn)
        if first and ARENA_POISON and self.arena is not None and self.arena.tensor is not None:
            self.arena.tensor.fill_(0xFF)
        ol = self.ol
        if ol.arr is None:
            ol.finalize()
        if dyn:
            ol.bind(**dyn)
        _lib.get_executor().run(ol.arr[lo:hi])

    def autotune_convs(self, **dyn):
        from .. import _lib
        ex = _lib.get_executor()
        ex = getattr(ex, 'ex', ex)
        if ex.is_mock or not hasattr(ex, 'time_ops'):
            return
        ol = self.ol
        if ol.arr is None:
            ol.finalize()
        ol.bind(**dyn)
        arr = ol.arr
        cache = self.eng.tile_cache
        tuned_any = False
        for n in range(len(arr)):
            if arr['kind'][n] != O.CONV:
                continue
            i = arr['i'][n]
            M, cout, cin = int(i[0]) * int(i[7]) * int(i[8]), int(i[9]), int(i[3]) + int(i[4])
            fl = int(arr['flags'][n])
            key = O.conv_tile_key(M, cout, cin, int(i[11]), int(i[13]), fl & O.F_RELU_IN, fl & O.F_OUT_F32, int(i[1]), int(i[2]))
            best = cache.get(key)
            twin = self.korder_ref and int(i[0]) % self.korder_ref == 0
            kref = self.kref.get(n)
            twin = twin or kref is not None
            if twin:
                M1 = M // self.korder_ref if kref is None else M * kref // int(i[0])
                key1 = (M1,) + key[1:]
                ref = cache.get(key1) or (O.static_tile(M1, cout, cin, int(i[11]), int(i[4]), cout1=int(i[17]) == O.COUT1_TILE), 1)
                want = O.korder_class(*ref)
                if isinstance(want, str) and cache.get(key + (want,)) is not None:
                    best = cache[key + (want,)]
                if best is None or O.korder_class(*best) != want:
                    best = (int(i[17]), 1) if O.korder_class(int(i[17]), int(i[19])) == want else tuple(ref)
                assert O.korder_class(*best) == want, (key, best, ref)
            if best is None and not getattr(self.eng, 'autotune', AUTOTUNE):
                continue
            if best is None:
                one = arr[n:n + 1].copy()
                best, best_t = (int(i[17]), 1), None
                cands = O.tile_candidates(M, cout, cin, int(i[16]),
                                          geom=dict(kh=int(i[11]), stride=int(i[13]), pad=int(i[14]), W=int(i[2]), c2=int(i[4])))
                if int(i[4]) or arr['p'][n, 4]:
                    cands = [t for t in cands if t != O.COUT1_TILE]
                for t in cands:
                    for sk in O.splitk_candidates(M, cout, int(i[16]), t):
                        one['i'][0, 17], one['i'][0, 19] = t, sk
                        ms = min(ex.time_ops(one, TUNE_ITERS) for _ in range(TUNE_REPS))
                        if best_t is None or ms < best_t:
                            best, best_t = (t, sk), ms
                cache[key] = best
                tuned_any = True
            apply = True
            if (best[0] in O.DMA_TILES or best[0] in O.PC_TILES) and not O.dma_tiles_enabled():
                apply = False
            if (arr['p'][n, 7] or arr['p'][n, 8]) and best[0] not in O.DMA_TILES and best[0] not in O.PC_TILES:
                apply = False
            if apply:
                arr['i'][n, 17], arr['i'][n, 19] = best
            if twin:
                assert O.korder_class(int(arr['i'][n, 17]), int(arr['i'][n, 19])) == want, (key, int(arr['i'][n, 17]), int(arr['i'][n, 19]), want)
        ol.wire_next_weights()
        self.tuned = True
        if tuned_any:
            save_tile_cache(cache)

    def conv(self, wname, x, *, name=None, out=None, stride=1, pad=None, x2=None, res=None, res_bcast=False,
             relu_in=False, act=O.ACT_NONE, out_f32=False, ldy=None, gap_acc=None, zero=None, persistent=False, res_group=None):
        w = self.eng.w[wname]
        if pad is None:
            pad = (w.kh - 1) // 2
        OH = (x.H + 2 * pad - w.kh) // stride + 1
        OW = (x.W + 2 * pad - w.kw) // stride + 1
        if out is None:
            t = self.buf(name or wname, (x.B, OH, OW, w.cout), F32 if out_f32 else BF16, persistent=persistent)
            out = Act(t, x.B, OH, OW, w.cout, w.cout if ldy is None else ldy)
        else:
            assert out.B == x.B and out.H == OH and out.W == OW and out.C == w.cout, (wname, out.B, out.H, out.W, out.C, OH, OW, w.cout)
        if res is not None:
            assert res.C == w.cout and res.H == OH and res.W == OW

        def emit(s0, s1, zero):
            whole = s0 == 0 and s1 == x.B
            cut = (lambda a, elem: a.t) if whole else (lambda a, elem: _objects_from(a, s0, elem))
            return self.ol.conv(cut(x, 2), w, cut(out, 4 if out_f32 else 2), B=s1 - s0, H=x.H, W=x.W, C1=x.C, ldx1=x.ld, OH=OH, OW=OW, ldy=out.ld, stride=stride,
                                pad=pad, x2=None if x2 is None else cut(x2, 2), C2=0 if x2 is None else x2.C,
                                ldx2=0 if x2 is None else x2.ld, res=None if res is None else (res.t if res_bcast else cut(res, 2)),
                                ldr=0 if res is None else res.ld, res_bcast=res_bcast, relu_in=relu_in, act=act, out_f32=out_f32,
                                gap_acc=gap_acc if (gap_acc is None or whole) else gap_acc[s0:], zero=zero, prio=self.prio, res_group=res_group)
        if self.mixed is None or x.B != sum(self.mixed):
            emit(0, x.B, zero)
            return out
        assert res_group is None
        counts, st = self.mixed, O.clip_starts(self.mixed)
        side = gap_acc is not None or zero is not None
        cin = x.C + (0 if x2 is None else x2.C)

        def one_clip_class(Kc):
            M1 = Kc * OH * OW
            key1 = O.conv_tile_key(M1, w.cout, cin, w.kh, stride, relu_in, out_f32, x.H, x.W)
            static = O.static_tile(M1, w.cout, cin, w.kh, 0 if x2 is None else x2.C, res is not None, side)
            return O.korder_class(*(self.eng.tile_cache.get(key1) or (static, 1)))
        cls = [one_clip_class(k) for k in counts]
        c0 = 0
        for c in range(1, len(counts) + 1):
            if c < len(counts) and cls[c] == cls[c0]:
                continue
            z = zero
            if zero is not None and c - c0 < len(counts):
                per_obj = zero.dim() == 2 and zero.shape[0] == x.B
                z = zero[st[c0]:st[c]] if per_obj else (zero if c0 == 0 else None)
            n = emit(st[c0], st[c], z)
            if c - c0 > 1:
                self.kref[n] = counts[c0]
            c0 = c
        return out

    def ca_block(self, prefix, x, name, out=None, head=None):
        if head is not None:
            head = (self.eng.w[head[0]], head[1])
        w = self.eng.w[prefix + '.conv2']
        gap = self.buf(name + '.gap', (x.B, x.C), F32)
        HW = x.H * x.W
        if O.conv_side_jobs_ok(cin=x.C, cout=w.cout, kh=w.kh):
            sums = self.buf(name + '.gapsum', (x.B, x.C), torch.int64)
            t1 = self.conv(prefix + '.conv1', x, name=name + '.t1', relu_in=True, act=O.ACT_RELU, zero=sums)
            t2 = self.conv(prefix + '.conv2', t1, name=name + '.t2', gap_acc=sums)
            if out is None:
                out = Act(self.buf(name + '.out', (x.B, x.H, x.W, x.C)), x.B, x.H, x.W, x.C)
            self.ol.eca_apply(t2.t, gap, self.eng.w[prefix + '.conv.weight'], x.t, out.t, B=x.B, HW=HW, C=x.C, fixed_sums=sums, head=head)
            return out
        t1 = self.conv(prefix + '.conv1', x, name=name + '.t1', relu_in=True, act=O.ACT_RELU)
        t2 = self.conv(prefix + '.conv2', t1, name=name + '.t2')
        self.ol.gap(t2.t, gap, B=x.B, HW=HW, C=x.C, partial_only=True)
        if out is None:
            out = Act(self.buf(name + '.out', (x.B, x.H, x.W, x.C)), x.B, x.H, x.W, x.C)
        self.ol.eca_apply(t2.t, gap, self.eng.w[prefix + '.conv.weight'], x.t, out.t, B=x.B, HW=HW, C=x.C, head=head)
        return out

    def fusion_block(self, prefix, x, g, name, out=None, xt=None, xt_group=None):
        if xt is None:
            xt = self.conv(prefix + '.distributor.x_transform', x, name=name + '.xt')
        if xt_group is not None and not isinstance(xt_group[0], int):
            counts, stride = xt_group
            xte = self.buf(name + '.xte', (g.B, xt.H, xt.W, xt.C))
            self.ol.copy2d(xt.t, xte, rows=g.B, rowbytes=xt.H * xt.W * xt.C * 2, src_stride=stride * xt.ld * 2, dst_stride=xt.H * xt.W * xt.C * 2, clips=counts)
            g0 = self.conv(prefix + '.distributor.g_transform', g, name=name + '.g0', res=Act(xte, g.B, xt.H, xt.W, xt.C))
        else:
            g0 = self.conv(prefix + '.distributor.g_transform', g, name=name + '.g0', res=xt, res_bcast=True, res_group=xt_group)
        g1 = self.ca_block(prefix + '.block1', g0, name + '.b1')
        return self.ca_block(prefix + '.block2', g1, name + '.b2', out=out)

    def resnet(self, prefix, x, taps=None):
        bottleneck, layers = resnet_layers(self.eng.m, prefix)
        feats = {}
        for (lname, planes, nb, lstride) in layers:
            for bi in range(nb):
                p = f'{prefix}.{lname}.{bi}'
                s = lstride if bi == 0 else 1
                last = bi == nb - 1
                out = taps.get(lname) if (taps and last) else None
                if bottleneck:
                    t1 = self.conv(p + '.conv1', x, act=O.ACT_RELU)
                    t2 = self.conv(p + '.conv2', t1, stride=s, act=O.ACT_RELU)
                    r = self.conv(p + '.downsample.0', x, stride=s) if (p + '.downsample.0') in self.eng.w else x
                    x = self.conv(p + '.conv3', t2, res=r, act=O.ACT_RELU, out=out)
                else:
                    t1 = self.conv(p + '.conv1', x, stride=s, act=O.ACT_RELU)
                    r = self.conv(p + '.downsample.0', x, stride=s) if (p + '.downsample.0') in self.eng.w else x
                    x = self.conv(p + '.conv2', t1, res=r, act=O.ACT_RELU, out=out)
            feats[lname] = x
        return x, feats


def _objects_from(a, s0, elem):
    per_obj = a.H * a.W * a.ld
    if isinstance(a.t, Dyn):
        return Dyn(a.t.name, a.t.offset + s0 * per_obj * elem)
    assert a.t.is_contiguous() and a.t.element_size() == elem, (a.t.shape, a.t.dtype, elem)
    return a.t.reshape(-1)[s0 * per_obj:]


MIXED_FUSION_EXTRA = 1


def clip_layout(K, clips):
    if isinstance(clips, int):
        counts = (int(K),) * clips
    else:
        counts = tuple(int(k) for k in clips)
    return len(counts), counts, O.clip_starts(counts), len(set(counts)) > 1


def stem_ok(eng, name):
    w = eng.w.get(name)
    return w is not None and w.cout == 64 and w.kh == 7 and w.kw == 7 and w.cin_padded == 8 and w.bias is not None


def build_encode(eng, h0, w0, H, W, pad_left, pad_top, B=1, qrows=64):
    P = Plan(eng, touch=weights_go_cold(B * (H // 16) * (W // 16)), prio=False)
    m = eng.m
    img = (lambda b: Dyn('image')) if B == 1 else (lambda b: Dyn('image%d' % b))
    if stem_ok(eng, 'pixel_encoder.conv1'):
        pool = P.buf('pool', (B, H // 4, W // 4, 64))
        SM = O.OpList.STEM_MAX_IMAGES
        for b0 in range(0, B, SM):
            P.ol.stem(img(b0), None, eng.w['pixel_encoder.conv1'], pool[b0:], h0=h0, w0=w0, H=H, W=W, pad_left=pad_left, pad_top=pad_top, K=1,
                      mean=m['pixel_mean'], std=m['pixel_std'], relu=True, more_images=[img(b) for b in range(b0 + 1, min(B, b0 + SM))])
        x = Act(pool, B, H // 4, W // 4, 64)
    else:
        img8 = P.buf('img8', (B, H, W, 8))
        for b in range(B):
            P.ol.img_prep(img(b), None, img8[b], h0=h0, w0=w0, H=H, W=W, pad_left=pad_left, pad_top=pad_top, K=1,
                          mean=m['pixel_mean'], std=m['pixel_std'])
        x = P.conv('pixel_encoder.conv1', Act(img8, B, H, W, 8), stride=2, pad=3, act=O.ACT_RELU)
        pool = P.buf('pool', (B, x.H // 2, x.W // 2, 64))
        P.ol.maxpool(x.t, pool, B=B, H=x.H, W=x.W, C=64)
        x = Act(pool, B, x.H // 2, x.W // 2, 64)
    h4, w4, h8, w8, h, w = H // 4, W // 4, H // 8, W // 8, H // 16, W // 16
    ms = m['pixel_encoder']['ms_dims']
    taps = {'res2': Act(Dyn('f4'), B, h4, w4, ms[2]), 'layer2': Act(Dyn('f8'), B, h8, w8, ms[1]),
            'layer3': Act(Dyn('f16'), B, h, w, ms[0])}
    f16, _ = P.resnet('pixel_encoder', x, taps)
    pix = P.conv('pix_feat_proj', f16, out=Act(Dyn('pix_feat'), B, h, w, m['pixel_dim']))
    build_key_ops(P, f16, h, w, qrows)
    W_ = eng.w
    for wname, src, dname in (('mask_decoder.decoder_feat_proc.transforms.0', taps['layer2'], 'f8p'),
                              ('mask_decoder.decoder_feat_proc.transforms.1', taps['res2'], 'f4p'),
                              ('pixel_fuser.fuser.distributor.x_transform', pix, 'fuse_xt')):
        P.conv(wname, src, out=Act(Dyn(dname), B, src.H, src.W, W_[wname].cout))
    P.meta.update(h=h, w=w, B=B)
    if B > 1:
        P.korder_ref = B
    return P


def build_key_ops(P, f16, h, w, qrows=64):
    m = P.eng.m
    CK = m['key_dim']
    B = f16.B
    kx = P.conv('key_proj.pix_feat_proj', f16, name='keyx')
    P.conv('key_proj.key_proj', kx, out=Act(Dyn('key'), B, h, w, CK), out_f32=True)
# ... 25 lines not shown
        P.ol.keep.append(pair)
    else:
        pair = P.buf('pair', (K, h, w, 64), persistent=True)
        m16 = P.buf('m16', (K, h, w), F32)
        for c in range(G):
            P.ol.mask_down(Dyn('last_mask' if G == 1 else 'last_mask%d' % c), pair[st[c]:], m16[st[c]:], K=counts[c], H=16 * h, W=16 * w, pair_channels=64)
    if G > 1 and not stacked:
        px = P.buf('pixel_all', (K, h, w, m['value_dim']))
        nb = h * w * m['value_dim'] * 2
        P.ol.bank_write([(Dyn('pixel%d' % c), px[st[c]:], counts[c] * nb) for c in range(G)])
        pixel = Act(px, K, h, w, m['value_dim'])
    else:
        pixel = Act(Dyn('pixel'), K, h, w, m['value_dim'])
    p16 = P.conv('pixel_fuser.sensory_compress', Act(Dyn('sensory_bf16'), K, h, w, m['sensory_dim']),
                 x2=Act(pair, K, h, w, 64), res=pixel, name='p16')
    xt = Act(Dyn('fuse_xt'), G, h, w, eng.w['pixel_fuser.fuser.distributor.x_transform'].cout) if pre else None
    P.fusion_block('pixel_fuser.fuser', Act(Dyn('pix_feat'), 1, h, w, m['pixel_dim']), p16, 'fuse',
                   out=Act(Dyn('fused'), K, h, w, m['embed_dim']), xt=xt, xt_group=(counts if mixed else counts[0], wstride * h * w) if G > 1 else None)
    if G > 1 and not mixed:
        P.korder_ref = G
    return P


def build_readout_query(eng, K, h, w, last_aux=True, fresh=True, clips=1):
    G, counts, st, mixed = clip_layout(K, clips)
    K = st[-1]
    Kc = counts if mixed else counts[0]
    P = Plan(eng, touch=weights_go_cold(h * w, K))
    P.mixed = counts if mixed else None
    if G > 1 and not mixed:
        P.korder_ref = G
    m, ol, W = eng.m, P.ol, eng.w
    ot = m['object_transformer']
    C, Q, heads, nb = m['embed_dim'], ot['num_queries'], ot['num_heads'], ot['num_blocks']
    HW, M = h * w, K * Q
    t = 'object_transformer'
    f = lambda name, shape: P.buf(name, shape, F32)
    query, query_emb = eng.query_bufs(K)
    use_chain = C == 256 and Q == 16 and heads == 8 and HW <= 24576 and ot['ff_dim'] % 64 == 0
    assert G == 1 or use_chain, 'clips in lock step need the chain form of the query side'
    qacc = P.buf('qacc', (3 * nb, M, C), torch.int64) if use_chain else None
    zero_on_conv = None
    if C == 256 and Q == 16:
        if fresh or not use_chain:
            ol.query_init2(Dyn('obj_mem'), query, query_emb, rows=M, w_init=W[t + '.summary_to_query_init'], res_init=eng.rep_embedding('query_init', K),
                           w_emb=W[t + '.summary_to_query_emb'], res_emb=eng.rep_embedding('query_emb', K), zero=qacc)
        elif O.conv_side_jobs_ok(cin=C, cout=C, kh=1):
            zero_on_conv = qacc
        else:
            ol.memset32(qacc, 2 * qacc.numel(), 0)
    else:
        vals = f('vals', (M, C))
        ol.query_init(Dyn('obj_mem'), vals, rows=M, C=C)
        ol.linear(vals, W[t + '.summary_to_query_init'], query, M=M, res=eng.rep_embedding('query_init', K))
        ol.linear(vals, W[t + '.summary_to_query_emb'], query_emb, M=M, res=eng.rep_embedding('query_emb', K))
    pix_in = Act(Dyn('pixel'), K, h, w, C)
    pixel = P.conv(t + '.pixel_init_proj', pix_in, name='pixel_init', zero=zero_on_conv)
    aux = P.buf('aux_logits', (nb + 1, K, HW), F32, persistent=True)
    fused_mask = HW <= 24576
    fg = None if fused_mask else P.buf('fg', (K, HW), torch.uint8)
    nfg = None if fused_mask else P.buf('nfg', (K,), torch.int32)
    P.conv(t + '.mask_pred.0.1', pixel, relu_in=True, out_f32=True, out=Act(aux[0], K, h, w, 1))
    if not fused_mask:
        ol.aux_mask(aux[0], fg, nfg, K=K, HW=HW)
    x = query
    prev_acc = q_pre = xn_next = None
    for b in range(nb):
        q = f'{t}.blocks.{b}'
        n = f'b{b}.'
        kvq = P.conv(q + '.pixel_proj_x', pixel, x2=pix_in, name=n + 'kvq', res=Act(eng.pe_rb(h, w, b), 1, h, w, 3 * C), res_bcast=True)
        ln = lambda name: (W[q + name + '.weight'], W[q + name + '.bias'])
        xn = xn_next if xn_next is not None else f(n + 'xn', (M, C))
        xn_next = None
        fuse_proj = fused_mask and C == 256
        chain = fuse_proj and use_chain
        if chain:
            Wo1, Wo2 = W[q + '.read_from_pixel.out'], W[q + '.self_attn.out']
            W1, W2 = W[q + '.ffn.linear1'], W[q + '.ffn.linear2']
            a1, a2, a3 = qacc[3 * b], qacc[3 * b + 1], qacc[3 * b + 2]
            if q_pre is not None:
                ol.attn_q2p(None, kvq.t, None, None, None, K=K, Q=Q, HW=HW, C=C, heads=heads, ldkv=3 * C, voff=C, logits=aux[b],
                            q_pre=q_pre, out_proj=(Wo1, a1), clip_objects=Kc)
            else:
                ol.attn_q2p(None, kvq.t, None, None, None, K=K, Q=Q, HW=HW, C=C, heads=heads, ldkv=3 * C, voff=C, logits=aux[b],
                            proj=dict(x=x, W=W[q + '.read_from_pixel.q'], emb=query_emb, ln=ln('.read_from_pixel.norm'), ln_out=xn),
                            acc_in=prev_acc, out_proj=(Wo1, a1), clip_objects=Kc)
            y = f(n + 'y', (M, C))
            ol.attn_self(None, None, None, K=K, Q=Q, C=C, heads=heads,
                         proj=dict(x=xn, W=W[q + '.self_attn.qkv'], emb=query_emb, ln=ln('.self_attn.norm'), ln_out=y),
                         acc_in=(a1, Wo1.bias), out_proj=(Wo2, a2))
            x2 = f(n + 'x2', (M, C))
            ol.qffn(y, x2, a3, rows=M, ln=ln('.ffn.norm'), W1=W1, W2=W2, acc_in=(a2, Wo2.bias), hid_slice=64)
            x = x2
            prev_acc = (a3, W2.bias)
            next_q = None
            if b + 1 < nb:
                qn = f'{t}.blocks.{b + 1}'
                q_pre, xn_next = f(f'b{b + 1}.q', (M, C)), f(f'b{b + 1}.xn', (M, C))
                next_q = dict(ln=(W[qn + '.read_from_pixel.norm.weight'], W[qn + '.read_from_pixel.norm.bias']), W=W[qn + '.read_from_pixel.q'],
                              q_out=q_pre, xn_out=xn_next)
            else:
                q_pre = None
            pa = P.buf(n + 'pa', (K, h, w, C))
            ol.attn_p2q(kvq.t.view(-1)[2 * C:], None, None, pa, K=K, Q=Q, HW=HW, C=C, heads=heads, ldq=3 * C,
                        proj=dict(x=x, W=W[q + '.read_from_query.kv'], emb=query_emb), acc_in=prev_acc, next_q=next_q)
        else:
            att = f(n + 'att', (M, C))
            if fuse_proj:
                ol.attn_q2p(None, kvq.t, None, None, att, K=K, Q=Q, HW=HW, C=C, heads=heads, ldkv=3 * C, voff=C, logits=aux[b],
                            proj=dict(x=x, W=W[q + '.read_from_pixel.q'], emb=query_emb, ln=ln('.read_from_pixel.norm'), ln_out=xn))
            else:
                qp = f(n + 'qp', (M, C))
                ol.linear(x, W[q + '.read_from_pixel.q'], qp, M=M, x_add=query_emb, add_rows=M, ln=ln('.read_from_pixel.norm'), ln_out=xn)
                ol.attn_q2p(qp, kvq.t, fg, nfg, att, K=K, Q=Q, HW=HW, C=C, heads=heads, ldkv=3 * C, voff=C, logits=aux[b] if fused_mask else None)
            x1 = f(n + 'x1', (M, C))
            ol.linear(att, W[q + '.read_from_pixel.out'], x1, M=M, res=xn)
            y = f(n + 'y', (M, C))
            sa = f(n + 'sa', (M, C))
            if fuse_proj:
                ol.attn_self(None, None, sa, K=K, Q=Q, C=C, heads=heads,
                             proj=dict(x=x1, W=W[q + '.self_attn.qkv'], emb=query_emb, ln=ln('.self_attn.norm'), ln_out=y))
            else:
                qkv = f(n + 'qkv', (M, 3 * C))
                ol.linear(x1, W[q + '.self_attn.qkv'], qkv, M=M, x_add=query_emb, add_rows=M, add_cols=2 * C, ln=ln('.self_attn.norm'), ln_out=y)
                ol.attn_self(qkv, qkv.view(-1)[2 * C:], sa, K=K, Q=Q, C=C, heads=heads, ldqk=3 * C, ldv=3 * C)
            x2 = f(n + 'x2', (M, C))
            ol.linear(sa, W[q + '.self_attn.out'], x2, M=M, res=y)
            hid = f(n + 'hid', (M, ot['ff_dim']))
            ol.linear(x2, W[q + '.ffn.linear1'], hid, M=M, relu=True, ln=ln('.ffn.norm'))
            x3 = f(n + 'x3', (M, C))
            ol.linear(hid, W[q + '.ffn.linear2'], x3, M=M, res=x2)
            x = x3
            pa = P.buf(n + 'pa', (K, h, w, C))
            if fuse_proj:
                ol.attn_p2q(kvq.t.view(-1)[2 * C:], None, None, pa, K=K, Q=Q, HW=HW, C=C, heads=heads, ldq=3 * C,
                            proj=dict(x=x, W=W[q + '.read_from_query.kv'], emb=query_emb))
            else:
                kv2 = f(n + 'kv2', (M, 2 * C))
                ol.linear(x, W[q + '.read_from_query.kv'], kv2, M=M, x_add=query_emb, add_rows=M, add_cols=C)
                ol.attn_p2q(kvq.t.view(-1)[2 * C:], kv2, kv2.view(-1)[C:], pa, K=K, Q=Q, HW=HW, C=C, heads=heads, ldq=3 * C, ldkv=2 * C)
        pf = P.conv(q + '.read_from_query.out', Act(pa, K, h, w, C), name=n + 'pf', res=pixel)
        last = b == nb - 1
        want_aux = not last or last_aux
        fuse_head = want_aux and C == 256
        pixel = P.ca_block(q + '.pixel_ffn.conv', pf, n + 'ffn', out=Act(Dyn('out'), K, h, w, C) if last else None,
                           head=(f'{t}.mask_pred.{b + 1}.1', aux[b + 1]) if fuse_head else None)
        if want_aux and not fuse_head:
            P.conv(f'{t}.mask_pred.{b + 1}.1', pixel, relu_in=True, out_f32=True, out=Act(aux[b + 1], K, h, w, 1))
        if not last and not fused_mask:
            ol.aux_mask(aux[b + 1], fg, nfg, K=K, HW=HW)
    return P


def build_segment(eng, K, h, w, update_sensory, pre=False, md=False, clips=1, wstride=1):
    G, counts, st, mixed = clip_layout(K, clips)
    K = st[-1]
    Kc = max(counts)
    assert G == 1 or (pre and Kc + 1 <= 8), 'clips in lock step: image-only decoder convs from the encoder plan, <= 7 objects per clip'
    P = Plan(eng, touch=weights_go_cold(h * w, K))
    P.mixed = counts if mixed else None
    gkey = counts if mixed else G
    sgrp = counts if mixed else counts[0]
    if G > 1 and not mixed:
        P.korder_ref = G
    m, ol = eng.m, P.ol
    up = m['mask_decoder']['up_dims']
    ms = m['pixel_encoder']['ms_dims']
    CS = m['sensory_dim']
    h8, w8, h4, w4 = 2 * h, 2 * w, 4 * h, 4 * w
    if pre:
        f8p, f4p = Act(Dyn('f8p'), G, h8, w8, up[0]), Act(Dyn('f4p'), G, h4, w4, up[1])
    else:
        f8p = P.conv('mask_decoder.decoder_feat_proc.transforms.0', Act(Dyn('f8'), 1, h8, w8, ms[1]), name='f8p')
        f4p = P.conv('mask_decoder.decoder_feat_proc.transforms.1', Act(Dyn('f4'), 1, h4, w4, ms[2]), name='f4p')
    p16 = Act(Dyn('p16'), K, h, w, up[0])
    u8 = P.buf('u8', (K, h8, w8, up[0]))
    ol.upsample2x_add(p16.t, f8p.t, u8, B=K, h=h, w=w, C=up[0], skip_group=(sgrp, wstride * h8 * w8) if G > 1 else None)
    u8 = Act(u8, K, h8, w8, up[0])
    t1 = P.conv('mask_decoder.up_16_8.out_conv.conv1', u8, relu_in=True, act=O.ACT_RELU)
    ds = P.conv('mask_decoder.up_16_8.out_conv.downsample', u8)
    p8 = P.conv('mask_decoder.up_16_8.out_conv.conv2', t1, res=ds, name='p8')
    u4 = P.buf('u4', (K, h4, w4, up[1]))
    ol.upsample2x_add(p8.t, f4p.t, u4, B=K, h=h8, w=w8, C=up[1], skip_group=(sgrp, wstride * h4 * w4) if G > 1 else None)
    u4 = Act(u4, K, h4, w4, up[1])
    t2 = P.conv('mask_decoder.up_8_4.out_conv.conv1', u4, relu_in=True, act=O.ACT_RELU)
    p4 = P.conv('mask_decoder.up_8_4.out_conv.conv2', t2, res=u4, name='p4')
    logits = P.buf('logits', (K, h4, w4), F32)
    P.conv('mask_decoder.pred', p4, relu_in=True, out_f32=True, out=Act(logits, K, h4, w4, 1))
    P.meta['logits_done'] = len(ol.recs)
    if update_sensory:
        CT = up[1] + up[2] + 64
        gcat = P.buf('gcat', (K, h, w, CT), persistent=True)
        ol.area_down3([dict(x=p8.t, y=gcat, B=K, H=h8, W=w8, C=up[1], ldx=up[1], ldy=CT, r=2),
                       dict(x=p4.t, y=gcat.view(-1)[up[1]:], B=K, H=h4, W=w4, C=up[2], ldx=up[2], ldy=CT, r=4),
                       dict(x=logits, y=gcat.view(-1)[up[1] + up[2]:], B=K, H=h4, W=w4, C=1, ldx=1, ldy=CT, r=4, f32_in=True, Cz=8)])
        g3 = P.conv('mask_decoder.sensory_update.g_all', p16, x2=Act(gcat, K, h, w, CT), name='g3')
        vals = P.conv('mask_decoder.sensory_update.transform', g3, x2=Act(Dyn('sensory_bf16'), K, h, w, CS),
                      out_f32=True, name='gru_vals')
        ol.gru(vals.t, Dyn('sensory_f32'), Dyn('sensory_bf16'), n=K * h * w, C=CS)
    if Kc + 1 <= 16:
        ol.up4_softmax(logits, Dyn('prob'), Dyn('logits_up'), P=Kc + 1, h=h4, w=w4, from_logits=True, clips=counts if mixed else G,
                       mask_down=(eng.mask_down_bufs(K, h, w, gkey)[1], eng.mask_down_bufs(K, h, w, gkey)[0], 64) if md else None)
    else:
        agg = P.buf('agg', (K + 1, h4, w4), F32)
        ol.seg_agg(logits, agg, K=K, hw=h4 * w4)
        ol.up4_softmax(agg, Dyn('prob'), Dyn('logits_up'), P=K + 1, h=h4, w=w4)
    return P


def build_encode_mask(eng, K, h0, w0, H, W, pad_left, pad_top, deep_update=True, pre_md=False, clips=1, wstride=1):
    G, counts, st, mixed = clip_layout(K, clips)
    K = st[-1]
    Kc = counts[0]
    P = Plan(eng, touch=weights_go_cold((H // 16) * (W // 16), K))
    P.mixed = counts if mixed else None
    if G > 1 and not mixed:
        P.korder_ref = G
    m, ol = eng.m, P.ol
    h, w = H // 16, W // 16
    CV, CS, CE, Q = m['value_dim'], m['sensory_dim'], m['embed_dim'], m['object_summarizer']['num_summaries']
    masks_of = (lambda c: Dyn('masks')) if G == 1 else (lambda c: Dyn('masks', 4 * (st[c] + c + 1) * H * W))
    assert G == 1 or stem_ok(eng, 'mask_encoder.conv1')
    if stem_ok(eng, 'mask_encoder.conv1'):
        pool = P.buf('pool', (K, H // 4, W // 4, 64))
        iname = lambda c: Dyn('image' if G == 1 else 'image%d' % c)
        SM = O.OpList.STEM_MAX_IMAGES
        for c0 in range(0, G, SM):
            ol.stem(iname(c0), masks_of(c0), eng.w['mask_encoder.conv1'], pool[st[c0]:], h0=h0, w0=w0, H=H, W=W, pad_left=pad_left, pad_top=pad_top,
                    K=Kc, mean=m['pixel_mean'], std=m['pixel_std'], relu=True, more_images=[iname(c) for c in range(c0 + 1, min(G, c0 + SM))],
                    mask_stride=(Kc + 1) * H * W, counts=counts if mixed else None)
    else:
        x8 = P.buf('x8', (K, H, W, 8))
        ol.img_prep(Dyn('image'), Dyn('masks'), x8, h0=h0, w0=w0, H=H, W=W, pad_left=pad_left, pad_top=pad_top, K=K,
                    mean=m['pixel_mean'], std=m['pixel_std'])
        x = P.conv('mask_encoder.conv1', Act(x8, K, H, W, 8), stride=2, pad=3)
        pool = P.buf('pool', (K, x.H // 2, x.W // 2, 64))
        ol.maxpool(x.t, pool, B=K, H=x.H, W=x.W, C=64, relu=True)
    g16, _ = P.resnet('mask_encoder', Act(pool, K, H // 4, W // 4, 64))
    xt = xt_group = None
    if G > 1:
        wx = eng.w['mask_encoder.fuser.distributor.x_transform']
        xt_t = P.buf('fuse.xt', (G, h, w, wx.cout))
        for c in range(G):
            P.conv('mask_encoder.fuser.distributor.x_transform', Act(Dyn('pix_feat', 2 * c * wstride * h * w * m['pixel_dim']), 1, h, w, m['pixel_dim']),
                   out=Act(xt_t[c:c + 1], 1, h, w, wx.cout))
        xt, xt_group = Act(xt_t, G, h, w, wx.cout), (counts if mixed else Kc, h * w)
    value = P.fusion_block('mask_encoder.fuser', Act(Dyn('pix_feat'), 1, h, w, m['pixel_dim']), g16, 'fuse',
                           out=Act(Dyn('value'), K, h, w, CV), xt=xt, xt_group=xt_group)
    P.meta['value_done'] = len(ol.recs)
    if deep_update:
        vals = P.conv('mask_encoder.sensory_update.transform', value, x2=Act(Dyn('sensory_bf16'), K, h, w, CS),
                      out_f32=True, name='gru_vals')
        ol.gru(vals.t, Dyn('sensory_f32'), Dyn('sensory_bf16'), n=K * h * w, C=CS)
    if pre_md:
        m16 = eng.mask_down_bufs(K, h, w, counts if mixed else G)[1]
    else:
        pair = P.buf('pair', (K, h, w, 8))
        m16 = P.buf('m16', (K, h, w), F32)
        for c in range(G):
            ol.mask_down(masks_of(c), pair[st[c]:], m16[st[c]:], K=counts[c], H=H, W=W)
    fw1 = P.conv('object_summarizer.in_fw0', value, res=Act(eng.pe_sum(h, w), 1, h, w, 2 * CE), res_bcast=True, act=O.ACT_RELU, name='sum.fw1')
    fw2 = P.conv('object_summarizer.fw2', fw1, out_f32=True, name='sum.fw2')
    ol.summarize(fw2.t, fw2.t.view(-1)[CE:], m16, Dyn('summ'), K=K, HW=h * w, C=CE, Q=Q, feat_f32=True, ldf=CE + Q, ldw=CE + Q)
    return P


def build_mask_to_prob(eng, Knew, Kold, h0, w0, H, W, pad_left, pad_top, float_mode, nfloat):
    P = Plan(eng)
    planes = P.buf('planes', (Knew, H, W), F32)
    P.ol.mask_merge(Dyn('inmask'), Dyn('pred'), Dyn('src'), planes, h0=h0, w0=w0, H=H, W=W, pad_left=pad_left,
                    pad_top=pad_top, Knew=Knew, Kold=Kold, nfloat=nfloat, float_mode=float_mode)
    P.ol.agg_softmax(planes, Dyn('prob'), K=Knew, HW=H * W)
    return P
```

### cutie_amd/ops.py

```python
import os

import numpy as np
import torch

from . import _lib

NI, NF, NP = 24, 6, 16
OP_DTYPE = np.dtype([('kind', '<i4'), ('flags', '<i4'), ('i', '<i4', (NI,)), ('f', '<f4', (NF,)), ('p', '<u8', (NP,))])
assert OP_DTYPE.itemsize == _lib.OP_STRUCT_SIZE

(CONV, MAXPOOL, IMG_PREP, UPSAMPLE2X_ADD, AREA_DOWN, MASK_DOWN, GAP, ECA_APPLY, GRU, SEG_AGG, UP4_SOFTMAX,
 MASK_MERGE, AGG_SOFTMAX, LINEAR, LAYERNORM, QUERY_INIT, AUX_MASK, ATTN_Q2P, ATTN_SELF, ATTN_P2Q, SUMMARIZE,
 ADD_PE, KEY_PREP, AFF_SCORE, AFF_SELECT, AFF_READOUT, MEMSET32, COPY2D, AXPY, USAGE_TICK, RANK_SELECT,
 GATHER_ROWS, CONSOL_AFF, CONSOL_READ, CAST, PROB_TO_ID, RESIZE, FLIP_W, AREA_DOWN3, QFFN, STEM, BANK_WRITE) = range(1, 43)

KIND_NAMES = {}
for _n in ('CONV MAXPOOL IMG_PREP UPSAMPLE2X_ADD AREA_DOWN MASK_DOWN GAP ECA_APPLY GRU SEG_AGG UP4_SOFTMAX MASK_MERGE '
           'AGG_SOFTMAX LINEAR LAYERNORM QUERY_INIT AUX_MASK ATTN_Q2P ATTN_SELF ATTN_P2Q SUMMARIZE ADD_PE KEY_PREP '
           'AFF_SCORE AFF_SELECT AFF_READOUT MEMSET32 COPY2D AXPY USAGE_TICK RANK_SELECT GATHER_ROWS CONSOL_AFF '
           'CONSOL_READ CAST PROB_TO_ID RESIZE FLIP_W AREA_DOWN3 QFFN STEM').split():
    KIND_NAMES[globals()[_n]] = _n

F_RELU_IN, F_OUT_F32, F_RES_BCAST = 1, 2, 4
F_PRIO, F_AFF_PRIO = 256, 64
F_TILE_OFF = 128 if os.environ.get('CUTIE_AMD_COUT1_TILE', '1') in ('', '0') else 0
ACT_NONE, ACT_RELU, ACT_SIGMOID, ACT_SQ1 = 0, 1, 2, 3
ACT_SHIFT = 4
AREA_RT = 8 if os.environ.get('CUTIE_AMD_AREA_R', '1') in ('', '0') else 0
GRU_SCALAR = 1 if os.environ.get('CUTIE_AMD_GRU4', '1') in ('', '0') else 0
KEYPREP_LOOP = 2 if os.environ.get('CUTIE_AMD_KEYPREP_LOOP', '0') not in ('', '0') else 0
UP4_LANES = 16 if os.environ.get('CUTIE_AMD_UP4_SHARED', '1') in ('', '0') else 0
SELECT_COARSE = 2 if os.environ.get('CUTIE_AMD_SELECT_FINE', '1') in ('', '0') else 0
UP4_RTK = 8 if os.environ.get('CUTIE_AMD_UP4_KC', '1') in ('', '0') else 0

TILES = {0: (128, 128, 32), 1: (128, 64, 32), 2: (64, 64, 32), 3: (256, 16, 32), 4: (64, 128, 32),
         5: (64, 64, 64), 6: (64, 128, 64), 7: (128, 128, 64), 8: (64, 64, 128), 9: (32, 64, 64),
         10: (128, 64, 64), 11: (32, 64, 128), 12: (32, 128, 64),
         13: (64, 64, 64), 14: (128, 64, 64), 15: (64, 128, 64), 16: (128, 128, 64), 17: (64, 64, 128), 18: (128, 128, 32),
         20: (64, 64, 64), 21: (64, 64, 128), 22: (32, 64, 128), 23: (128, 64, 64), 24: (64, 128, 64), 25: (128, 128, 64),
         26: (32, 64, 64), 27: (64, 64, 64), 28: (32, 64, 64), 29: (64, 128, 32), 30: (64, 64, 32)}
TILE_WK = {20: 2, 21: 2, 22: 2, 23: 2, 24: 2, 25: 2, 26: 2, 27: 4, 28: 4, 29: 2, 30: 2}

DMA_TILES = {60: (128, 128, 64), 61: (128, 128, 64), 62: (128, 128, 64), 63: (128, 64, 64), 64: (64, 128, 64), 65: (64, 64, 64),
             66: (64, 64, 64), 67: (32, 64, 64), 68: (256, 128, 64), 69: (32, 128, 64), 70: (128, 128, 64), 71: (128, 64, 64),
             72: (64, 64, 64), 73: (64, 64, 64), 74: (64, 64, 64), 75: (32, 64, 64), 76: (128, 64, 64), 77: (64, 128, 64), 78: (32, 128, 64),
             80: (64, 64, 128), 81: (64, 64, 128), 82: (32, 64, 128), 83: (32, 64, 128), 84: (64, 128, 128), 85: (128, 64, 128),
             86: (96, 64, 64), 87: (96, 64, 64), 88: (64, 64, 64), 89: (64, 64, 64)}


PC_TILES = {100: (64, 64, 64), 101: (64, 64, 64), 102: (32, 64, 64), 103: (128, 64, 64), 104: (64, 128, 64), 105: (128, 128, 64),
            106: (128, 128, 64), 107: (64, 64, 64), 108: (128, 128, 64), 109: (32, 64, 64), 110: (96, 64, 64), 111: (96, 128, 64),
            120: (64, 64, 64), 121: (64, 64, 64), 122: (128, 64, 64), 123: (128, 128, 64), 124: (64, 128, 64), 125: (32, 64, 64),
            126: (128, 128, 64), 127: (64, 128, 64), 129: (96, 64, 64), 130: (32, 64, 64), 131: (64, 128, 64),
            132: (64, 64, 64), 133: (96, 128, 64), 134: (320, 64, 64),
            140: (64, 64, 64), 141: (96, 64, 64), 142: (96, 64, 64), 143: (32, 64, 64), 144: (128, 64, 64),
            145: (96, 64, 64), 146: (128, 64, 64), 147: (32, 64, 64)}
PC_HALO = {120: (8, 8), 121: (4, 16), 122: (8, 16), 123: (8, 16), 124: (8, 8), 125: (4, 8), 126: (8, 16), 127: (4, 16),
           129: (10, 9), 130: (5, 6), 131: (6, 9), 132: (6, 9), 133: (10, 9), 134: (20, 16),
           145: (10, 9), 146: (8, 16), 147: (5, 6)}

ALL_TILES = {**TILES, **DMA_TILES, **PC_TILES}


def korder_class(tile, splitk=1):
    if tile in PC_HALO:
        return 'halo'
    if tile in TILE_WK or splitk != 1:
        return ('split', tile, splitk)
    if tile in (3, COUT1_TILE):
        return ('small', tile)
    return 'stream' if (tile in DMA_TILES or tile in PC_TILES) else 'igemm'


def pc_tile_ok(tile, *, cin, kh, stride=1, pad=None, c2=0):
    if cin % 64 or (c2 and (c2 % 64 or (cin - c2) % 64)) or kh > 5:
        return False
    if tile in PC_HALO:
        return kh == 3 and stride == 1 and (pad is None or pad == 1)
    return True


def pc_blocks(tile, B, OH, OW, cout):
    bm, bn, _ = PC_TILES[tile]
    if tile in PC_HALO:
        th, tw = PC_HALO[tile]
        return B * -(-OH // th) * -(-OW // tw) * -(-cout // bn)
    return -(-(B * OH * OW) // bm) * -(-cout // bn)


def dma_tiles_enabled():
    return os.environ.get('CUTIE_AMD_DMA_TILES', '1') not in ('', '0')


def dma_tile_ok(tile, *, cin, kh, c2=0):
    bk = DMA_TILES[tile][2]
    return cin % bk == 0 and (c2 == 0 or (c2 % bk == 0 and (cin - c2) % bk == 0)) and kh * kh <= 32


def conv_side_jobs_ok(*, cin, cout, kh, c2=0):
    return dma_tiles_enabled() and dma_tile_ok(60, cin=cin, kh=kh, c2=c2) and cout % 8 == 0 and cout > 16


NUM_CU = 256
WEIGHT_PREFETCH = int(os.environ.get('CUTIE_AMD_WPF', str(8 << 20)))
WEIGHT_PREFETCH_BLOCK = int(os.environ.get('CUTIE_AMD_WPF_BLOCK', str(48 << 10)))


COUT1_TILE = 19


def cout1_ok(cout, cin, c2=0, res=False):
    lp = cin // 8
    return cout == 1 and c2 == 0 and not res and cin % 8 == 0 and 1 <= lp <= 64 and (lp & (lp - 1)) == 0


def tile_candidates(M, cout, cin, kpad=None, geom=None):
    if cout <= 16:
        return [3] + ([COUT1_TILE] if cout1_ok(cout, cin) else [])
    out = []
    for t, (bm, bn, bk) in TILES.items():
        if t == 3 or (bk > 32 and cin < 32):
            continue
        wk = TILE_WK.get(t, 1)
        if wk > 1 and (kpad is None or (kpad // bk) % wk or kpad // bk < 2 * wk):
            continue
        if bn == 128 and cout <= 64:
            continue
        if bm * 2 > max(M, 64) * 2 and bm > 64:
            continue
        out.append(t)
    if dma_tiles_enabled() and geom is not None and dma_tile_ok(60, cin=cin, kh=geom['kh'], c2=geom.get('c2', 0)):
        for t, (bm, bn, bk) in DMA_TILES.items():
            if not (bn == 128 and cout <= 64) and not (bm > 64 and bm > max(M, 64)) and not (bm == 256 and M < 16384) \
                    and dma_tile_ok(t, cin=cin, kh=geom['kh'], c2=geom.get('c2', 0)):
                out.append(t)
    if dma_tiles_enabled() and geom is not None:
        for t, (bm, bn, bk) in PC_TILES.items():
            if pc_tile_ok(t, cin=cin, kh=geom['kh'], stride=geom.get('stride', 1), pad=geom.get('pad'), c2=geom.get('c2', 0)) \
                    and not (bn == 128 and cout <= 64) and not (bm > 64 and bm > max(M, 64)) and not (bm == 256 and M < 16384):
                out.append(t)
    return out


SPLITK_PART_FLOATS = 16 << 20
_splitk_scratch = {}


def splitk_scratch(device, owner=None):
    dev = torch.device(device)
    store = _splitk_scratch if owner is None else owner.__dict__.setdefault('_splitk_part', {})
    key = str(dev)
    if key not in store:
        n = SPLITK_PART_FLOATS if dev.type == 'cuda' else 1024
        store[key] = torch.zeros(n, dtype=torch.float32, device=device)
    return store[key]


def splitk_candidates(M, cout, kpad, tile):
    if tile == COUT1_TILE or tile == 3 or tile in DMA_TILES or tile in PC_TILES:
        return [1]
    bm, bn, bk = TILES[tile]
    blocks = -(-M // bm) * -(-cout // bn)
    nk = kpad // bk // TILE_WK.get(tile, 1)
    ldp = (cout + 7) & ~7
    out = [1]
    for sk in (2, 3, 4, 6, 8, 9, 12, 16, 18):
        if blocks >= NUM_CU or blocks * sk > 6 * NUM_CU or nk // sk < 2:
            break
        if sk * M * ldp > SPLITK_PART_FLOATS:
            break
        if nk % sk == 0:
            out.append(sk)
    return out


def pick_tile(M, cout, cin=64, geom=None):
    if cout <= 16:
        return 3
    if geom is not None and dma_tiles_enabled() and dma_tile_ok(60, cin=cin, kh=geom['kh'], c2=geom.get('c2', 0)):
        cands = [t for t in (108, 103, 110, 101, 102) if pc_tile_ok(t, cin=cin, kh=geom['kh'], c2=geom.get('c2', 0))]
    else:
        cands = [6, 5, 9] if cin >= 32 else [4, 2]
    if cout <= 64:
        cands = [c for c in cands if ALL_TILES[c][1] <= 64] or [2]
    best, best_blocks = None, -1
    for t in cands:
        bm, bn, _ = ALL_TILES[t]
        blocks = -(-M // bm) * -(-cout // bn)
        if blocks >= NUM_CU:
            return t
        if blocks > best_blocks:
            best, best_blocks = t, blocks
    return best


def static_tile(M, cout, cin, kh, c2=0, res=False, side=False, cout1=None):
    if (cout1_ok(cout, cin, c2, res) and not side) if cout1 is None else cout1:
        return COUT1_TILE
    return pick_tile(M, cout, cin, dict(kh=kh, c2=c2))


def conv_tile_key(M, cout, cin, kh, stride, relu_in, out_f32, H, W):
    return (int(M), int(cout), int(cin), int(kh), int(stride), (1 if relu_in else 0) | (2 if out_f32 else 0), int(H), int(W))


def aa_taps(n_in, n_out):
    f32 = np.float32
    i = np.arange(n_out)
    if n_in == n_out:
        return i, np.ones(n_out, dtype=np.int64), np.ones((n_out, 1), dtype=f32)
    scale = f32(n_in) / f32(n_out)
    support = scale if scale >= 1 else f32(1.0)
    invscale = f32(1.0 / np.float64(scale)) if scale >= 1 else f32(1.0)
    max_taps = int(np.ceil(support)) * 2 + 1
    center = (np.float64(scale) * (i + 0.5)).astype(f32)
    first = np.maximum(((center - support).astype(np.float64) + 0.5).astype(np.int64), 0)
    count = np.minimum(((center + support).astype(np.float64) + 0.5).astype(np.int64), n_in) - first
    count = np.clip(count, 0, max_taps)
    j = np.arange(max_taps)
    pos = (first[:, None] + j[None, :]).astype(f32)
    arg = (((pos - center[:, None]).astype(np.float64) + 0.5) * np.float64(invscale)).astype(f32)
    arg = np.abs(arg)
    w = np.where(arg < 1, f32(1.0) - arg, f32(0.0)).astype(f32)
    w[j[None, :] >= count[:, None]] = 0
    total = np.zeros(n_out, dtype=f32)
    for k in range(max_taps):
        total = (total + w[:, k]).astype(f32)
    nz = total != 0
    w[nz] = (w[nz] / total[nz, None]).astype(f32)
    return first, count, w


def resize_aa_table(H, W, OH, OW):
    parts = [aa_taps(W, OW), aa_taps(H, OH)]
    K = max(int(w.shape[1]) for _, _, w in parts)
    tab = np.zeros((OW + OH, K + 2), dtype=np.int32)
    r = 0
    for first, count, w in parts:
        n = len(first)
        tab[r:r + n, 0], tab[r:r + n, 1] = first, count
        tab[r:r + n, 2:2 + w.shape[1]] = w.view(np.int32)
        r += n
    return tab


def pack_counts(counts):
    counts = [int(k) for k in counts]
    assert 1 <= len(counts) <= 8 and all(1 <= k <= 7 for k in counts), counts
    return sum(k << (3 * c) for c, k in enumerate(counts))


def clip_starts(counts):
    st = [0]
    for k in counts:
        st.append(st[-1] + int(k))
    return st


class Dyn:
    __slots__ = ('name', 'offset')

    def __init__(self, name, offset=0):
        self.name, self.offset = name, offset


def _ptr(t):
    if t is None:
        return 0
    if isinstance(t, int):
        return t
    return t.data_ptr()


JPEG_SYNC_ROUNDS = 4


class OpList:
    PRIO_KINDS = frozenset((UPSAMPLE2X_ADD, AREA_DOWN3, ECA_APPLY, GRU, UP4_SOFTMAX, ATTN_Q2P, ATTN_SELF, ATTN_P2Q, QFFN))

    def __init__(self, scratch_owner=None, touch_next_weights=True, prio=True):
        self.prio = prio
        self.scratch_owner = scratch_owner
        self.touch_next_weights = touch_next_weights
        self.recs = []
        self.keep = []
        self.wbytes = {}
        self.dyn = {}
        self.arr = None
        self._words = None

    def add(self, kind, flags=0, ints=(), floats=(), ptrs=()):
        idx = len(self.recs)
        if kind in self.PRIO_KINDS and self.prio:
            flags |= F_PRIO
        pl = []
        for slot, t in enumerate(ptrs):
            if isinstance(t, Dyn):
                self.dyn.setdefault(t.name, []).append((idx, slot, t.offset))
                pl.append(0)
            else:
                if isinstance(t, torch.Tensor):
                    self.keep.append(t)
                pl.append(_ptr(t))
        self.recs.append((kind, flags, [int(v) for v in ints], [float(v) for v in floats], pl))
        self.arr = self._words = None
        return idx

    def finalize(self):
        arr = np.zeros(len(self.recs), dtype=OP_DTYPE)
        for n, (kind, flags, ints, floats, ptrs) in enumerate(self.recs):
            arr['kind'][n] = kind
            arr['flags'][n] = flags
            arr['i'][n, :len(ints)] = ints
            arr['f'][n, :len(floats)] = floats
            arr['p'][n, :len(ptrs)] = ptrs
        self.arr = arr
        self._words = None
        self.wire_next_weights()
        return arr

    def wire_next_weights(self):
        arr = self.arr
        convs = [n for n in range(len(arr)) if arr['kind'][n] == CONV]
        for n in convs:
            arr['p'][n, 9:11] = 0
            arr['i'][n, 22:24] = 0
        if not (WEIGHT_PREFETCH and self.touch_next_weights):
            return
        nxt, nxt2 = None, None
        for n in reversed(convs):
            i = arr['i'][n]
            pc = int(i[17]) in PC_TILES
            if nxt is not None and pc:
                budget = WEIGHT_PREFETCH_BLOCK * -(-pc_blocks(int(i[17]), int(i[0]), int(i[7]), int(i[8]), int(i[9])) // 8)
                n1 = min(nxt[1], WEIGHT_PREFETCH, budget)
                arr['p'][n, 9], arr['i'][n, 22] = nxt[0], n1
                n2 = min(nxt2[1], WEIGHT_PREFETCH, budget - n1) if (nxt2 is not None and not nxt[2]) else 0
                if n2 > 0:
                    arr['p'][n, 10], arr['i'][n, 23] = nxt2[0], n2
            nxt, nxt2 = (int(arr['p'][n, 2]), self.wbytes[n], pc), nxt

    def patch_ints(self, op, start, values):
        values = [int(v) for v in values]
        ints = self.recs[op][2]
        end = start + len(values)
        if len(ints) < end:
            ints.extend([0] * (end - len(ints)))
        ints[start:end] = values
        if self.arr is not None:
            self.arr['i'][op, start:end] = values

    def bind(self, **tensors):
        if self.arr is None:
            self.finalize()
        words = self._words
        if words is None:
            assert OP_DTYPE.itemsize == 256 and OP_DTYPE.fields['p'][1] == 128
            words = self._words = ({name: tuple((idx * 32 + 16 + slot, off) for (idx, slot, off) in sl) for name, sl in self.dyn.items()},
                                   memoryview(self.arr).cast('B').cast('Q'))
        table, mv = words
        for name, t in tensors.items():
            sl = table.get(name)
            if sl is None:
                continue
            base = 0 if t is None else (t if type(t) is int else t.data_ptr())
            if base:
                for w, off in sl:
                    mv[w] = base + off
            else:
                for w, off in sl:
                    mv[w] = 0

    def run(self, _stream=None, **tensors):
        if self.arr is None:
            self.finalize()
        if tensors:
            self.bind(**tensors)
        ex = _lib.get_executor()
        if _stream is None:
            ex.run(self.arr)
        elif hasattr(ex, 'run_on'):
            ex.run_on(self.arr, _stream)
        else:
            with torch.cuda.stream(_stream):
                ex.run(self.arr)

    def __len__(self):
        return len(self.recs)

    def conv(self, x1, w, y, *, B, H, W, C1, ldx1, OH, OW, ldy, stride=1, pad=0, x2=None, C2=0, ldx2=0,
             res=None, ldr=0, res_bcast=False, relu_in=False, act=ACT_NONE, out_f32=False, tile=None, splitk=1,
             gap_acc=None, zero=None, prio=False, res_group=None):
        flags = (F_RELU_IN if relu_in else 0) | (F_OUT_F32 if out_f32 else 0) | (F_RES_BCAST if res_bcast else 0) | (act << ACT_SHIFT) | F_TILE_OFF | \
            (F_PRIO if prio else 0)
        assert C1 + C2 == w.cin_padded, (C1, C2, w.cin_padded)
        M = B * OH * OW
        side = gap_acc is not None or zero is not None
        if tile is None:
            tile = static_tile(M, w.cout, C1 + C2, w.kh, C2, res is not None, side)
        if side:
            assert (tile in DMA_TILES or tile in PC_TILES) and not out_f32 and w.cout % 8 == 0 and ldy % 8 == 0, 'GAP accumulation needs an LDS-DMA conv (see conv_side_jobs_ok)'
        part = splitk_scratch(w.weight.device, self.scratch_owner)
        self.wbytes[len(self.recs)] = w.weight.numel() * w.weight.element_size()
        return self.add(CONV, flags,
                        [B, H, W, C1, C2, ldx1, ldx2, OH, OW, w.cout, ldy, w.kh, w.kw, stride, pad, ldr, w.kpad, tile, w.cin_real,
                         splitk, part.numel() // 1024, 0 if zero is None else zero.numel()],
                        self._res_group(res_group, res_bcast, B, OH * OW), [x1, x2, w.weight, w.bias, res, y, part, gap_acc, zero])

    @staticmethod
    def _res_group(res_group, res_bcast, B, OHW):
        if res_group is None:
            return []
        kg, stride = int(res_group[0]), int(res_group[1])
        assert res_bcast and kg > 0 and B % kg == 0 and stride >= OHW and stride < (1 << 24), (res_group, B, OHW)
        return [float(kg), float(stride)]

    def maxpool(self, x, y, *, B, H, W, C, relu=False):
        OH, OW = (H + 2 - 3) // 2 + 1, (W + 2 - 3) // 2 + 1
        return self.add(MAXPOOL, 1 if relu else 0, [B, H, W, C, OH, OW], [], [x, y])

    STEM_MAX_IMAGES = 12

    def stem(self, image, masks, w, y, *, h0, w0, H, W, pad_left, pad_top, K, mean, std, relu=True, more_images=(), mask_stride=0, counts=None):
        assert w.cout == 64 and w.kh == 7 and w.cin_padded == 8 and H % 16 == 0 and W % 16 == 0
        more = list(more_images)
        assert len(more) < self.STEM_MAX_IMAGES
        if counts is not None:
            assert len(counts) == 1 + len(more) and len(counts) > 1
            ints = [h0, w0, H, W, pad_left, pad_top, max(counts), w.kpad, len(counts), 0, pack_counts(counts)]
            return self.add(STEM, 1 if relu else 0, ints, list(mean) + list(std), [image, masks, w.weight, w.bias, y] + more)
        ints = [h0, w0, H, W, pad_left, pad_top, K, w.kpad] + ([1 + len(more), int(mask_stride)] if more else [])
        return self.add(STEM, 1 if relu else 0, ints, list(mean) + list(std), [image, masks, w.weight, w.bias, y] + more)

    def img_prep(self, image, masks, y, *, h0, w0, H, W, pad_left, pad_top, K, mean, std):
        return self.add(IMG_PREP, 0, [h0, w0, H, W, pad_left, pad_top, K], list(mean) + list(std), [image, masks, y])

    def upsample2x_add(self, g, skip, y, *, B, h, w, C, skip_group=None):
        ints = [B, h, w, C]
        if skip_group is not None and not isinstance(skip_group[0], int):
            counts, stride = skip_group
            assert sum(counts) == B and stride >= 4 * h * w
            ints += [0, int(stride), pack_counts(counts)]
        elif skip_group is not None:
            kg, stride = int(skip_group[0]), int(skip_group[1])
            assert kg > 0 and B % kg == 0 and stride >= 4 * h * w
            ints += [kg, stride]
        return self.add(UPSAMPLE2X_ADD, 0, ints, [], [g, skip, y])

    def area_down(self, x, y, *, B, H, W, C, ldx, ldy, r, f32_in=False, Cz=None):
        return self.add(AREA_DOWN, 1 if f32_in else 0, [B, H, W, C, ldx, ldy, r, C if Cz is None else Cz], [], [x, y])

    def area_down3(self, segs):
        assert len(segs) == 3
        ints, ptrs, flags = [], [], 0
        for q, g in enumerate(segs):
            ints += [g['B'], g['H'], g['W'], g['C'], g['ldx'], g['ldy'], g['r'], g['C'] if g.get('Cz') is None else g['Cz']]
            ptrs += [g['x'], g['y']]
            flags |= (1 << q) if g.get('f32_in') else 0
        return self.add(AREA_DOWN3, flags | AREA_RT, ints, [], ptrs)

    def mask_down(self, masks, pair, m16, *, K, H, W, r=16, pair_channels=8):
        assert pair_channels % 8 == 0
        return self.add(MASK_DOWN, 0, [K, H, W, r, pair_channels], [], [masks, pair, m16])

    def gap(self, x, y, *, B, HW, C, scratch=None, partial_only=False):
        if scratch is None:
            scratch = torch.zeros((B, -(-HW // 64), C), dtype=torch.float32, device=y.device)
        self._last_gap_scratch = scratch
        return self.add(GAP, 1 if partial_only else 0, [B, HW, C], [], [x, y, scratch])

    def eca_apply(self, x, gap, wk, r, y, *, B, HW, C, part=None, fixed_sums=None, head=None):
        tail = []
        if head is not None:
            w, out = head
            assert C == 256 and w.cout == 1 and w.kh == 1 and w.cin_padded == 256
            tail = [w.weight, w.bias, out]
        if fixed_sums is not None:
            return self.add(ECA_APPLY, 1, [B, HW, C], [], [x, gap, wk, r, y, fixed_sums] + tail)
        if part is None:
            part = self._last_gap_scratch
        return self.add(ECA_APPLY, 0, [B, HW, C], [], [x, gap, wk, r, y, part] + tail)

    def gru(self, values, h, hb, *, n, C):
        return self.add(GRU, GRU_SCALAR, [n, C], [], [values, h, hb])

    def seg_agg(self, logits, agg, *, K, hw):
        return self.add(SEG_AGG, 0, [K, hw], [], [logits, agg])

    def up4_softmax(self, agg, prob, logits_up, *, P, h, w, from_logits=False, mask_down=None, clips=1):
        if not isinstance(clips, int):
            counts = [int(k) for k in clips]
            assert from_logits and len(counts) > 1 and h % 4 == 0 and w % 4 == 0 and not UP4_RTK, 'the mixed form: compile-time object counts'
            ints = [max(counts) + 1, h, w, 0, len(counts), pack_counts(counts)]
            if mask_down is not None:
                m16, pair, ints[3] = mask_down
                return self.add(UP4_SOFTMAX, 1 | 4 | UP4_LANES, ints, [], [agg, prob, logits_up, m16, pair])
            return self.add(UP4_SOFTMAX, 1, ints, [], [agg, prob, logits_up])
        if mask_down is not None:
            assert from_logits and P <= 8 and h % 4 == 0 and w % 4 == 0
            m16, pair, pitch = mask_down
            return self.add(UP4_SOFTMAX, 1 | 4 | UP4_RTK | UP4_LANES, [P, h, w, pitch, clips], [], [agg, prob, logits_up, m16, pair])
        assert clips == 1 or (from_logits and P <= 8)
        return self.add(UP4_SOFTMAX, (1 | UP4_RTK) if from_logits else 0, [P, h, w, 0, clips], [], [agg, prob, logits_up])

    def mask_merge(self, inmask, pred, src, planes, *, h0, w0, H, W, pad_left, pad_top, Knew, Kold, nfloat, float_mode):
        return self.add(MASK_MERGE, 1 if float_mode else 0, [h0, w0, H, W, pad_left, pad_top, Knew, Kold, nfloat], [],
                        [inmask, pred, src, planes])

    def agg_softmax(self, planes, prob, *, K, HW):
        return self.add(AGG_SOFTMAX, 0, [K, HW], [], [planes, prob])

    def linear(self, x, w, y, *, M, ldx=None, ldy=None, x_add=None, add_rows=0, res=None, relu=False, add_cols=0,
               ln=None, ln_out=None, eps=1e-5):
        flags = (1 if relu else 0) | (2 if ln is not None else 0)
        return self.add(LINEAR, flags,
                        [M, w.n, w.kd, w.kd if ldx is None else ldx, w.n if ldy is None else ldy, add_rows, add_cols], [eps],
                        [x, x_add, w.weight, w.bias, res, y, ln[0] if ln else None, ln[1] if ln else None, ln_out])

    def layernorm(self, x, g, b, y, *, M, C):
        return self.add(LAYERNORM, 0, [M, C], [], [x, g, b, y])

    def query_init(self, obj_mem, y, *, rows, C):
        return self.add(QUERY_INIT, 0, [rows, C], [], [obj_mem, y])

    def query_init2(self, obj_mem, query, query_emb, *, rows, w_init, res_init, w_emb, res_emb, zero=None):
        assert w_init.kd == 256 and w_init.n == 256 and w_emb.kd == 256 and w_emb.n == 256 and rows % 16 == 0
        nz = 0
        if zero is not None:
            nb = zero.numel() * zero.element_size()
            assert nb % 16 == 0 and zero.is_contiguous()
            nz = nb // 16
        return self.add(QUERY_INIT, 1, [rows, 256, nz], [], [obj_mem, query, query_emb, w_init.weight, w_init.bias, res_init,
                                                             w_emb.weight, w_emb.bias, res_emb, zero])

    def aux_mask(self, logits, fg, nfg, *, K, HW):
        self.memset32(nfg, K, 0)
        return self.add(AUX_MASK, 0, [K, HW], [], [logits, fg, nfg])

    @staticmethod
    def _proj(proj):
        ln = proj.get('ln') or (None, None)
        assert proj['W'].kd == 256
        return proj.get('ldx', 256), proj.get('ln_out'), [proj['W'].weight, proj['W'].bias, proj.get('emb'), ln[0], ln[1]]

    QACC_SCALE = 4294967296.0

    @staticmethod
    def _proj_extras(flags, ints, ptrs, acc_in, out_proj):
        ints = list(ints) + [0] * (9 - len(ints))
        ptrs = list(ptrs) + [None] * (14 - len(ptrs))
        if acc_in is not None:
            assert acc_in[0].dtype == torch.int64
            flags |= 4
            ptrs[10], ptrs[11] = acc_in[0], acc_in[1]
        if out_proj is not None:
            assert out_proj[0].kd == 256 and out_proj[0].n == 256 and out_proj[1].dtype == torch.int64
            flags |= 8
            ptrs[12], ptrs[13] = out_proj[0].weight, out_proj[1]
        return flags, ints, ptrs

    def attn_q2p(self, q, kv, fg, nfg, y, *, K, Q, HW, C, heads, ldkv, voff, logits=None, proj=None, acc_in=None, out_proj=None, q_pre=None, hstride=None,
                 clip_objects=None):
        hs = 0 if hstride in (None, C // heads) else hstride
        mixed = []
        if clip_objects is not None and not isinstance(clip_objects, int):
            assert out_proj is not None and sum(clip_objects) == K and len(clip_objects) > 1, 'clips in lock step need the chain form'
            mixed, clip_objects = [pack_counts(clip_objects)], None
        kg = 0 if clip_objects in (None, K) else int(clip_objects)
        assert kg == 0 or (out_proj is not None and K % kg == 0), 'clips in lock step need the chain form'
        if q_pre is not None:
            assert proj is None and acc_in is None and out_proj is not None and logits is not None
            flags, ints, ptrs = self._proj_extras(3 | 16, [K, Q, HW, C, heads, ldkv, voff, 256], [q_pre, kv, logits, None, None], None, out_proj)
            ints[8] = hs
            return self.add(ATTN_Q2P, flags, ints + [kg] + mixed, [], ptrs)
        if proj is not None:
            assert logits is not None
            ldx, ln_out, tail = self._proj(proj)
            assert out_proj is not None or acc_in is None, 'the chain form of ATTN_Q2P needs out_proj'
            flags, ints, ptrs = self._proj_extras(3, [K, Q, HW, C, heads, ldkv, voff, ldx], [proj['x'], kv, logits, ln_out, y] + tail, acc_in, out_proj)
            assert hs == 0 or out_proj is not None, 'a head stride needs the chain form'
            ints[8] = hs
            return self.add(ATTN_Q2P, flags, ints + [kg] + mixed, [], ptrs)
        assert acc_in is None and out_proj is None
        if logits is not None:
            return self.add(ATTN_Q2P, 1, [K, Q, HW, C, heads, ldkv, voff], [], [q, kv, logits, None, y])
        return self.add(ATTN_Q2P, 0, [K, Q, HW, C, heads, ldkv, voff], [], [q, kv, fg, nfg, y])

    def attn_self(self, qk, v, y, *, K, Q, C, heads, ldqk=0, ldv=0, proj=None, acc_in=None, out_proj=None):
        if proj is not None:
            ldx, ln_out, tail = self._proj(proj)
# ... 536 lines not shown
```

Before: 1165.

## Fuse decoder area-down pooling into upsample and Cout=1 pred conv kernels

Removes the separate three-segment area_down launch after the mask decoder. The 2x pooling of p8 now runs in extra blocks appended to the upsample2x_add kernel. The 4x pooling of p4 and of the logits runs as extra blocks and an epilogue inside the Cout=1 tiled pred conv kernel. This cuts one launch and one round-trip of the logits through memory, at the cost of more validation paths and an LDS buffer plus a barrier in the conv kernel.

```diff
diff --git a/cutie_amd/_lib.py b/cutie_amd/_lib.py
--- a/cutie_amd/_lib.py
+++ b/cutie_amd/_lib.py
@@ -69,6 +69,10 @@
 
 def has_track_stats():
     return bool(load().cutie_hip_build_flags() & 16)
+
+
+def has_decoder_riders():
+    return bool(load().cutie_hip_build_flags() & 32)
 
 
 class HipExecutor:
diff --git a/cutie_amd/csrc/api.hip b/cutie_amd/csrc/api.hip
--- a/cutie_amd/csrc/api.hip
+++ b/cutie_amd/csrc/api.hip
@@ -127,7 +127,7 @@
 int cutie_hip_abi_version(void) { return 11; }
 int cutie_op_struct_size(void) { return (int)sizeof(cutie_op); }
 int cutie_hip_build_flags(void) {
-    const int forms = 2 | 4 | 8 | 16;
+    const int forms = 2 | 4 | 8 | 16 | 32;
 #ifdef CUTIE_DIAG
     return forms | 1;
 #else
diff --git a/cutie_amd/csrc/common.h b/cutie_amd/csrc/common.h
--- a/cutie_amd/csrc/common.h
+++ b/cutie_amd/csrc/common.h
@@ -95,6 +95,49 @@
     return n;
 }
 
+template <int R = 0>
+__device__ __forceinline__ void area_down_bf16_body(const bf16_t* __restrict__ x, bf16_t* __restrict__ y, int B, int H, int W, int C,
+                                                    int ldx, int ldy, int rrt, long idx) {
+    const int r = R > 0 ? R : rrt;
+    int C8 = C >> 3, OH = H / r, OW = W / r;
+    long total = (long)B * OH * OW * C8;
+    if (idx >= total) return;
+    int c = idx % C8; long t = idx / C8;
+    int ox = t % OW; t /= OW; int oy = t % OH; int b = t / OH;
+    float acc[8] = {0, 0, 0, 0, 0, 0, 0, 0};
+    if (R > 0) {
+        uint4 v[R > 0 ? R * R : 1];
+#pragma unroll
+        for (int dy = 0; dy < R; ++dy)
+#pragma unroll
+            for (int dx = 0; dx < R; ++dx)
+                v[dy * R + dx] = *reinterpret_cast<const uint4*>(x + (((long)b * H + oy * R + dy) * W + ox * R + dx) * ldx + c * 8);
+#pragma unroll
+        for (int e = 0; e < R * R; ++e) {
+            const uint32_t* u = &v[e].x;
+#pragma unroll
+            for (int i = 0; i < 4; ++i) {
+                acc[2 * i] += __uint_as_float(u[i] << 16);
+                acc[2 * i + 1] += __uint_as_float(u[i] & 0xffff0000u);
+            }
+        }
+    } else
+    for (int dy = 0; dy < r; ++dy)
+        for (int dx = 0; dx < r; ++dx) {
+            const uint4 v = *reinterpret_cast<const uint4*>(x + (((long)b * H + oy * r + dy) * W + ox * r + dx) * ldx + c * 8);
+            const uint32_t* u = &v.x;
+#pragma unroll
+            for (int i = 0; i < 4; ++i) {
+                acc[2 * i] += __uint_as_float(u[i] << 16);
+                acc[2 * i + 1] += __uint_as_float(u[i] & 0xffff0000u);
+            }
+        }
+    float inv = 1.f / (float)(r * r);
+    uint4 o = make_uint4(pack_bf2(acc[0] * inv, acc[1] * inv), pack_bf2(acc[2] * inv, acc[3] * inv),
+                         pack_bf2(acc[4] * inv, acc[5] * inv), pack_bf2(acc[6] * inv, acc[7] * inv));
+    *reinterpret_cast<uint4*>(y + (((long)b * OH + oy) * OW + ox) * ldy + c * 8) = o;
+}
+
 int launch_conv(const cutie_op* op, hipStream_t s);
 int launch_elementwise(const cutie_op* op, hipStream_t s);
 int launch_attention(const cutie_op* op, hipStream_t s);
diff --git a/cutie_amd/csrc/conv_common.h b/cutie_amd/csrc/conv_common.h
--- a/cutie_amd/csrc/conv_common.h
+++ b/cutie_amd/csrc/conv_common.h
@@ -10,6 +10,7 @@
     const unsigned char* pf; int pf_bytes;
     const unsigned char* pf2; int pf2_bytes;
     int res_grp_rows, res_grp_stride;
+    bf16_t* pool_x; bf16_t* pool_y; int pool_ld, pool_cz;
 };
 #define GAP_FIXED_SCALE 16777216.f
 #define GAP_ELEM_SHIFT 4
diff --git a/cutie_amd/csrc/conv_igemm.hip b/cutie_amd/csrc/conv_igemm.hip
--- a/cutie_amd/csrc/conv_igemm.hip
+++ b/cutie_amd/csrc/conv_igemm.hip
@@ -295,14 +295,19 @@
     }
 }
 
-template <int TR>
+template <int TR, bool RIDERS = false>
 __global__ __launch_bounds__(256) void conv_cout1_tile_kernel(ConvParams p) {
     if (p.flags & CUTIE_F_PRIO) __builtin_amdgcn_s_setprio(1);
     static_assert(TR % 4 == 0, "rows per wave");
     constexpr int TC = 16, PW = TC + 2, NPIX = (TR + 2) * PW, RW = TR / 4;
     __shared__ u32x4 tile[NPIX * 16];
+    __shared__ float outs[RIDERS ? TR * TC : 1];
     const int tid = threadIdx.x, lane = tid & 63, wave = tid >> 6, n = lane & 15, g = lane >> 4;
     const int tiles_x = (p.W + TC - 1) / TC, tiles_y = (p.H + TR - 1) / TR;
+    if (RIDERS && blockIdx.x >= p.B * tiles_x * tiles_y) {
+        area_down_bf16_body<4>(p.x1, p.pool_x, p.B, p.H, p.W, p.Cin, p.ldx1, p.pool_ld, 4, (long)(blockIdx.x - p.B * tiles_x * tiles_y) * 256 + tid);
+        return;
+    }
     const int b = blockIdx.x / (tiles_x * tiles_y), rem = blockIdx.x - b * tiles_x * tiles_y;
     const int ty = rem / tiles_x, tx = rem - ty * tiles_x;
     const int x0 = tx * TC, y0 = ty * TR;
@@ -362,8 +367,25 @@
                     const long m = ((long)b * p.H + oy) * p.W + x;
                     if (p.flags & CUTIE_F_OUT_F32) reinterpret_cast<float*>(p.y)[m * p.ldy] = v;
                     else reinterpret_cast<bf16_t*>(p.y)[m * p.ldy] = f2bf(v);
+                    if (RIDERS) outs[(wave * RW + r) * TC + 4 * g + q] = v;
                 }
             }
+        }
+    }
+    if (RIDERS && p.pool_y) {
+        __syncthreads();
+        const int cy = tid / (TC / 4), cx = tid % (TC / 4);
+        const int cy0 = y0 + 4 * cy, cx0 = x0 + 4 * cx;
+        if (tid < (TR / 4) * (TC / 4) && cy0 < p.H && cx0 < p.W) {
+            float v[16];
+#pragma unroll
+            for (int e = 0; e < 16; ++e) v[e] = outs[(4 * cy + (e >> 2)) * TC + 4 * cx + (e & 3)];
+            float acc = 0.f;
+#pragma unroll
+            for (int e = 0; e < 16; ++e) acc += v[e];
+            bf16_t* yp = p.pool_y + (((long)b * (p.H / 4) + (cy0 >> 2)) * (p.W / 4) + (cx0 >> 2)) * p.pool_ld;
+            yp[0] = f2bf(acc * (1.f / 16.f));
+            for (int c = 1; c < p.pool_cz; ++c) yp[c] = 0;
         }
     }
 }
@@ -477,6 +499,8 @@
     p.pf = (const unsigned char*)op->p[9]; p.pf_bytes = op->p[9] ? i[22] : 0;
     p.pf2 = (const unsigned char*)op->p[10]; p.pf2_bytes = op->p[10] ? i[23] : 0;
     p.res_grp_rows = p.res_grp_stride = 0;
+    p.pool_x = (bf16_t*)op->p[11]; p.pool_y = (bf16_t*)op->p[12]; p.pool_ld = (int)op->f[2]; p.pool_cz = (int)op->f[3];
+    const bool riders = p.pool_x || p.pool_y;
     if ((p.flags & CUTIE_F_RES_BCAST) && op->f[0] > 0.f) {
         const int kg = (int)op->f[0];
         if (kg <= 0 || p.B % kg || op->f[1] < (float)p.OHW || op->f[1] != (float)(int)op->f[1]) { cutie_set_error("conv: residual groups of %d objects do not divide B = %d (or stride %g < OH*OW)", kg, p.B, (double)op->f[1]); return -2; }
@@ -496,6 +520,12 @@
                         p.C1, p.C2, p.ldx1, p.ldx2, p.Kpad, p.M, p.Cout);
         return -2;
     }
+    if (riders && (i[17] != 19 || (p.flags & (CUTIE_F_PLAIN | CUTIE_F_TILE_OFF)) || p.Cin != 128 || p.KH != 3 || p.KW != 3 || p.stride != 1 || p.pad != 1 ||
+                   p.OH != p.H || p.OW != p.W || p.H * p.W < 4096)) {
+        cutie_set_error("conv: the pooling riders (p11 / p12) ride on the Cout == 1 tile kernel only (tile 19, Cin = 128, 3x3 / stride 1 / pad 1, "
+                        "H * W >= 4096; tile %d, Cin %d, %d x %d)", i[17], p.Cin, p.H, p.W);
+        return -2;
+    }
     if (i[17] == 19) {
         const int LP = p.Cin >> 3;
         if (p.Cout != 1 || p.C2 != 0 || p.res || LP > 64 || (LP & (LP - 1)) || LP < 1) {
@@ -507,6 +537,18 @@
             if (LP == 16 && !(p.flags & CUTIE_F_TILE_OFF)) {
                 constexpr int TR = 8;
                 const int blocks = p.B * ((p.H + TR - 1) / TR) * ((p.W + 15) / 16);
+                if (riders) {
+                    static_assert(TR % 4 == 0, "a tile holds whole 4 x 4 cells");
+                    if (!(p.flags & CUTIE_F_OUT_F32) || (p.H & 3) || (p.W & 3) || op->f[2] != (float)p.pool_ld || op->f[3] != (float)p.pool_cz || (p.pool_ld & 7) ||
+                        (p.pool_x && (p.pool_ld < p.Cin || ((uintptr_t)p.pool_x & 15))) || (p.pool_y && (p.pool_cz < 1 || p.pool_cz > p.pool_ld))) {
+                        cutie_set_error("conv cout1 tile (pooling riders): needs an fp32 output, H and W multiples of 4 (%d x %d), a pitch f2 = %g (whole, %% 8, >= Cin "
+                                        "for the 16-byte aligned p11) and 1 <= f3 = %g <= f2 channels of p12", p.H, p.W, (double)op->f[2], (double)op->f[3]);
+                        return -2;
+                    }
+                    const long npool = p.pool_x ? (long)p.B * (p.H / 4) * (p.W / 4) * LP : 0;
+                    hipLaunchKernelGGL((conv_cout1_tile_kernel<TR, true>), dim3(blocks + (unsigned)((npool + 255) / 256)), dim3(256), 0, s, p);
+                    return (int)hipGetLastError();
+                }
                 hipLaunchKernelGGL(conv_cout1_tile_kernel<TR>, dim3(blocks), dim3(256), 0, s, p);
                 return (int)hipGetLastError();
             }
diff --git a/cutie_amd/csrc/elementwise.hip b/cutie_amd/csrc/elementwise.hip
--- a/cutie_amd/csrc/elementwise.hip
+++ b/cutie_amd/csrc/elementwise.hip
@@ -66,14 +66,17 @@
     lam = src - (float)i0;
 }
 
-template <bool MIXED = false>
+template <bool MIXED = false, bool POOL = false>
 __global__ void upsample2x_add_kernel(const uint4* __restrict__ g, const uint4* __restrict__ skip, uint4* __restrict__ y,
-                                      int B, int h, int w, int C8, int Kg, long gstride, int prio) {
+                                      int B, int h, int w, int C8, int Kg, long gstride, int prio, bf16_t* __restrict__ y_pool, int ldyp) {
     if (prio) __builtin_amdgcn_s_setprio(1);
     long idx = (long)blockIdx.x * blockDim.x + threadIdx.x;
     int OH = 2 * h, OW = 2 * w;
     long total = (long)B * OH * OW * C8;
-    if (idx >= total) return;
+    if (idx >= total) {
+        if (POOL) area_down_bf16_body<2>(reinterpret_cast<const bf16_t*>(g), y_pool, B, h, w, C8 * 8, C8 * 8, ldyp, 2, idx - total);
+        return;
+    }
     int c = idx % C8; long t = idx / C8;
     int ox = t % OW; t /= OW; int oy = t % OH; int b = t / OH;
     int y0, y1, x0, x1; float ly, lx;
@@ -102,48 +105,6 @@
     y[idx] = make_uint4(out[0], out[1], out[2], out[3]);
 }
 
-template <int R = 0>
-__device__ __forceinline__ void area_down_bf16_body(const bf16_t* __restrict__ x, bf16_t* __restrict__ y, int B, int H, int W, int C,
-                                                    int ldx, int ldy, int rrt, long idx) {
-    const int r = R > 0 ? R : rrt;
-    int C8 = C >> 3, OH = H / r, OW = W / r;
-    long total = (long)B * OH * OW * C8;
-    if (idx >= total) return;
-    int c = idx % C8; long t = idx / C8;
-    int ox = t % OW; t /= OW; int oy = t % OH; int b = t / OH;
-    float acc[8] = {0, 0, 0, 0, 0, 0, 0, 0};
-    if (R > 0) {
-        uint4 v[R > 0 ? R * R : 1];
-#pragma unroll
-        for (int dy = 0; dy < R; ++dy)
-#pragma unroll
-            for (int dx = 0; dx < R; ++dx)
-                v[dy * R + dx] = *reinterpret_cast<const uint4*>(x + (((long)b * H + oy * R + dy) * W + ox * R + dx) * ldx + c * 8);
-#pragma unroll
-        for (int e = 0; e < R * R; ++e) {
-            const uint32_t* u = &v[e].x;
-#pragma unroll
-            for (int i = 0; i < 4; ++i) {
-                acc[2 * i] += __uint_as_float(u[i] << 16);
-                acc[2 * i + 1] += __uint_as_float(u[i] & 0xffff0000u);
-            }
-        }
-    } else
-    for (int dy = 0; dy < r; ++dy)
-        for (int dx = 0; dx < r; ++dx) {
-            const uint4 v = *reinterpret_cast<const uint4*>(x + (((long)b * H + oy * r + dy) * W + ox * r + dx) * ldx + c * 8);
-            const uint32_t* u = &v.x;
-#pragma unroll
-            for (int i = 0; i < 4; ++i) {
-                acc[2 * i] += __uint_as_float(u[i] << 16);
-                acc[2 * i + 1] += __uint_as_float(u[i] & 0xffff0000u);
-            }
-        }
-    float inv = 1.f / (float)(r * r);
-    uint4 o = make_uint4(pack_bf2(acc[0] * inv, acc[1] * inv), pack_bf2(acc[2] * inv, acc[3] * inv),
-                         pack_bf2(acc[4] * inv, acc[5] * inv), pack_bf2(acc[6] * inv, acc[7] * inv));
-    *reinterpret_cast<uint4*>(y + (((long)b * OH + oy) * OW + ox) * ldy + c * 8) = o;
-}
 __global__ void area_down_bf16_kernel(const bf16_t* __restrict__ x, bf16_t* __restrict__ y, int B, int H, int W, int C,
                                       int ldx, int ldy, int r) {
     area_down_bf16_body(x, y, B, H, W, C, ldx, ldy, r, (long)blockIdx.x * blockDim.x + threadIdx.x);
@@ -1363,12 +1324,19 @@
             long n = (long)i[0] * 4 * i[1] * i[2] * C8;
             if (i[6]) {
                 int objs; const int nc = mixed_clips((unsigned)i[6], &objs);
+                if (p[3]) { cutie_set_error("upsample2x_add: the pooling rider (p3) has no mixed form"); return -2; }
                 if (nc < 1 || objs != i[0] || i[4] != 0 || i[5] < 4 * i[1] * i[2]) { cutie_set_error("upsample2x_add (mixed form): the counts 0x%x do not add up to B = %d (or i4 != 0, or the stride is below one map)", i[6], i[0]); return -2; }
-                hipLaunchKernelGGL(upsample2x_add_kernel<true>, GRID1D(n, BS), dim3(BS), 0, s, (const uint4*)p[0], (const uint4*)p[1], (uint4*)p[2], i[0], i[1], i[2], C8, i[6], (long)i[5], PRIO);
+                hipLaunchKernelGGL(upsample2x_add_kernel<true>, GRID1D(n, BS), dim3(BS), 0, s, (const uint4*)p[0], (const uint4*)p[1], (uint4*)p[2], i[0], i[1], i[2], C8, i[6], (long)i[5], PRIO, (bf16_t*)nullptr, 0);
                 break;
             }
             if (i[4] < 0 || (i[4] > 0 && (i[0] % i[4] || i[5] < 4 * i[1] * i[2]))) { cutie_set_error("upsample2x_add: skip groups of %d objects do not divide B = %d (or their stride is below one map)", i[4], i[0]); return -2; }
-            hipLaunchKernelGGL(upsample2x_add_kernel<false>, GRID1D(n, BS), dim3(BS), 0, s, (const uint4*)p[0], (const uint4*)p[1], (uint4*)p[2], i[0], i[1], i[2], C8, i[4], (long)i[5], PRIO);
+            if (p[3]) {
+                if ((i[1] | i[2]) & 1 || (i[3] & 7) || i[7] < i[3] || (i[7] & 7) || (p[3] & 15)) { cutie_set_error("upsample2x_add (pooling rider): needs even h, w (%d x %d), C %% 8, a 16-byte aligned y_pool of pitch i7 = %d >= C, i7 %% 8", i[1], i[2], i[7]); return -2; }
+                const long n2 = (long)i[0] * (i[1] / 2) * (i[2] / 2) * C8;
+                hipLaunchKernelGGL((upsample2x_add_kernel<false, true>), GRID1D(n + n2, BS), dim3(BS), 0, s, (const uint4*)p[0], (const uint4*)p[1], (uint4*)p[2], i[0], i[1], i[2], C8, i[4], (long)i[5], PRIO, (bf16_t*)p[3], i[7]);
+                break;
+            }
+            hipLaunchKernelGGL(upsample2x_add_kernel<false>, GRID1D(n, BS), dim3(BS), 0, s, (const uint4*)p[0], (const uint4*)p[1], (uint4*)p[2], i[0], i[1], i[2], C8, i[4], (long)i[5], PRIO, (bf16_t*)nullptr, 0);
             break;
         }
         case CUTIE_OP_AREA_DOWN: {
diff --git a/cutie_amd/model/plans.py b/cutie_amd/model/plans.py
--- a/cutie_amd/model/plans.py
+++ b/cutie_amd/model/plans.py
@@ -43,6 +43,7 @@
 GRAPH_MIN_OPS = 8
 QINIT_SKIP = os.environ.get('CUTIE_AMD_QINIT_SKIP', '1') not in ('', '0')
 AUTOTUNE = os.environ.get('CUTIE_AMD_AUTOTUNE', '0') not in ('', '0')
+DECODER_RIDERS = True
 PACKAGED_TILES = os.path.join(os.path.dirname(os.path.abspath(__file__)), '..', 'tiles_gfx950.json')
 
 
@@ -301,6 +302,8 @@
         tuned_any = False
         for n in range(len(arr)):
             if arr['kind'][n] != O.CONV:
+                continue
+            if arr['p'][n, 11] or arr['p'][n, 12]:
                 continue
             i = arr['i'][n]
             M, cout, cin = int(i[0]) * int(i[7]) * int(i[8]), int(i[9]), int(i[3]) + int(i[4])
@@ -352,7 +355,7 @@
             save_tile_cache(cache)
 
     def conv(self, wname, x, *, name=None, out=None, stride=1, pad=None, x2=None, res=None, res_bcast=False,
-             relu_in=False, act=O.ACT_NONE, out_f32=False, ldy=None, gap_acc=None, zero=None, persistent=False, res_group=None):
+             relu_in=False, act=O.ACT_NONE, out_f32=False, ldy=None, gap_acc=None, zero=None, persistent=False, res_group=None, riders=None):
         w = self.eng.w[wname]
         if pad is None:
             pad = (w.kh - 1) // 2
@@ -373,7 +376,9 @@
                                 pad=pad, x2=None if x2 is None else cut(x2, 2), C2=0 if x2 is None else x2.C,
                                 ldx2=0 if x2 is None else x2.ld, res=None if res is None else (res.t if res_bcast else cut(res, 2)),
                                 ldr=0 if res is None else res.ld, res_bcast=res_bcast, relu_in=relu_in, act=act, out_f32=out_f32,
-                                gap_acc=gap_acc if (gap_acc is None or whole) else gap_acc[s0:], zero=zero, prio=self.prio, res_group=res_group)
+                                gap_acc=gap_acc if (gap_acc is None or whole) else gap_acc[s0:], zero=zero, prio=self.prio, res_group=res_group,
+                                riders=riders)
+        assert riders is None or self.mixed is None
         if self.mixed is None or x.B != sum(self.mixed):
             emit(0, x.B, zero)
             return out
@@ -705,6 +710,17 @@
     return P
 
 
+def decoder_riders_ok(eng, K, h4, w4, cin):
+    ex = _lib.get_executor()
+    if not DECODER_RIDERS or getattr(ex, 'ex', ex).is_mock or not _lib.has_decoder_riders():
+        return False
+    wp = eng.w['mask_decoder.pred']
+    M = K * h4 * w4
+    tile = (eng.tile_cache.get(O.conv_tile_key(M, wp.cout, cin, wp.kh, 1, True, True, h4, w4)) or (O.static_tile(M, wp.cout, cin, wp.kh), 1))[0]
+    return tile == O.COUT1_TILE and wp.cin_padded == cin and \
+        O.cout1_tile_form(cin=cin, kh=wp.kh, stride=1, pad=(wp.kh - 1) // 2, H=h4, W=w4, OH=h4, OW=w4)
+
+
 def build_segment(eng, K, h, w, update_sensory, pre=False, md=False, clips=1, wstride=1):
     G, counts, st, mixed = clip_layout(K, clips)
     K = st[-1]
@@ -733,20 +749,26 @@
     t1 = P.conv('mask_decoder.up_16_8.out_conv.conv1', u8, relu_in=True, act=O.ACT_RELU)
     ds = P.conv('mask_decoder.up_16_8.out_conv.downsample', u8)
     p8 = P.conv('mask_decoder.up_16_8.out_conv.conv2', t1, res=ds, name='p8')
+    gcat = riders = None
+    if update_sensory:
+        CT = up[1] + up[2] + 64
+        gcat = P.buf('gcat', (K, h, w, CT), persistent=True)
+        if G == 1 and decoder_riders_ok(eng, K, h4, w4, up[2]):
+            riders = dict(pool_x=gcat.view(-1)[up[1]:], pool_y=gcat.view(-1)[up[1] + up[2]:], ld=CT, cz=8)
     u4 = P.buf('u4', (K, h4, w4, up[1]))
-    ol.upsample2x_add(p8.t, f4p.t, u4, B=K, h=h8, w=w8, C=up[1], skip_group=(sgrp, wstride * h4 * w4) if G > 1 else None)
+    ol.upsample2x_add(p8.t, f4p.t, u4, B=K, h=h8, w=w8, C=up[1], skip_group=(sgrp, wstride * h4 * w4) if G > 1 else None,
+                      pool=(gcat, CT) if riders else None)
     u4 = Act(u4, K, h4, w4, up[1])
     t2 = P.conv('mask_decoder.up_8_4.out_conv.conv1', u4, relu_in=True, act=O.ACT_RELU)
     p4 = P.conv('mask_decoder.up_8_4.out_conv.conv2', t2, res=u4, name='p4')
     logits = P.buf('logits', (K, h4, w4), F32)
-    P.conv('mask_decoder.pred', p4, relu_in=True, out_f32=True, out=Act(logits, K, h4, w4, 1))
+    P.conv('mask_decoder.pred', p4, relu_in=True, out_f32=True, out=Act(logits, K, h4, w4, 1), riders=riders)
     P.meta['logits_done'] = len(ol.recs)
     if update_sensory:
-        CT = up[1] + up[2] + 64
-        gcat = P.buf('gcat', (K, h, w, CT), persistent=True)
-        ol.area_down3([dict(x=p8.t, y=gcat, B=K, H=h8, W=w8, C=up[1], ldx=up[1], ldy=CT, r=2),
-                       dict(x=p4.t, y=gcat.view(-1)[up[1]:], B=K, H=h4, W=w4, C=up[2], ldx=up[2], ldy=CT, r=4),
-                       dict(x=logits, y=gcat.view(-1)[up[1] + up[2]:], B=K, H=h4, W=w4, C=1, ldx=1, ldy=CT, r=4, f32_in=True, Cz=8)])
+        if not riders:
+            ol.area_down3([dict(x=p8.t, y=gcat, B=K, H=h8, W=w8, C=up[1], ldx=up[1], ldy=CT, r=2),
+                           dict(x=p4.t, y=gcat.view(-1)[up[1]:], B=K, H=h4, W=w4, C=up[2], ldx=up[2], ldy=CT, r=4),
+                           dict(x=logits, y=gcat.view(-1)[up[1] + up[2]:], B=K, H=h4, W=w4, C=1, ldx=1, ldy=CT, r=4, f32_in=True, Cz=8)])
         g3 = P.conv('mask_decoder.sensory_update.g_all', p16, x2=Act(gcat, K, h, w, CT), name='g3')
         vals = P.conv('mask_decoder.sensory_update.transform', g3, x2=Act(Dyn('sensory_bf16'), K, h, w, CS),
                       out_f32=True, name='gru_vals')
diff --git a/cutie_amd/ops.py b/cutie_amd/ops.py
--- a/cutie_amd/ops.py
+++ b/cutie_amd/ops.py
@@ -112,6 +112,10 @@
 def cout1_ok(cout, cin, c2=0, res=False):
     lp = cin // 8
     return cout == 1 and c2 == 0 and not res and cin % 8 == 0 and 1 <= lp <= 64 and (lp & (lp - 1)) == 0
+
+
+def cout1_tile_form(*, cin, kh, stride, pad, H, W, OH, OW):
+    return not F_TILE_OFF and cin == 128 and kh == 3 and stride == 1 and pad == 1 and OH == H and OW == W and H * W >= 4096
 
 
 def tile_candidates(M, cout, cin, kpad=None, geom=None):
@@ -390,7 +394,7 @@
 
     def conv(self, x1, w, y, *, B, H, W, C1, ldx1, OH, OW, ldy, stride=1, pad=0, x2=None, C2=0, ldx2=0,
              res=None, ldr=0, res_bcast=False, relu_in=False, act=ACT_NONE, out_f32=False, tile=None, splitk=1,
-             gap_acc=None, zero=None, prio=False, res_group=None):
+             gap_acc=None, zero=None, prio=False, res_group=None, riders=None):
         flags = (F_RELU_IN if relu_in else 0) | (F_OUT_F32 if out_f32 else 0) | (F_RES_BCAST if res_bcast else 0) | (act << ACT_SHIFT) | F_TILE_OFF | \
             (F_PRIO if prio else 0)
         assert C1 + C2 == w.cin_padded, (C1, C2, w.cin_padded)
@@ -402,10 +406,15 @@
             assert (tile in DMA_TILES or tile in PC_TILES) and not out_f32 and w.cout % 8 == 0 and ldy % 8 == 0, 'GAP accumulation needs an LDS-DMA conv (see conv_side_jobs_ok)'
         part = splitk_scratch(w.weight.device, self.scratch_owner)
         self.wbytes[len(self.recs)] = w.weight.numel() * w.weight.element_size()
+        floats, ptrs = self._res_group(res_group, res_bcast, B, OH * OW), [x1, x2, w.weight, w.bias, res, y, part, gap_acc, zero]
+        if riders is not None:
+            assert tile == COUT1_TILE and out_f32 and H % 4 == 0 and W % 4 == 0 and riders['ld'] % 8 == 0 and 1 <= riders['cz'] <= riders['ld'] and \
+                cout1_tile_form(cin=C1 + C2, kh=w.kh, stride=stride, pad=pad, H=H, W=W, OH=OH, OW=OW), 'the pooling riders need the Cout = 1 tile kernel'
+            floats = (floats or [0.0, 0.0]) + [float(riders['ld']), float(riders['cz'])]
+            ptrs += [None, None, riders.get('pool_x'), riders.get('pool_y')]
         return self.add(CONV, flags,
                         [B, H, W, C1, C2, ldx1, ldx2, OH, OW, w.cout, ldy, w.kh, w.kw, stride, pad, ldr, w.kpad, tile, w.cin_real,
-                         splitk, part.numel() // 1024, 0 if zero is None else zero.numel()],
-                        self._res_group(res_group, res_bcast, B, OH * OW), [x1, x2, w.weight, w.bias, res, y, part, gap_acc, zero])
+                         splitk, part.numel() // 1024, 0 if zero is None else zero.numel()], floats, ptrs)
 
     @staticmethod
     def _res_group(res_group, res_bcast, B, OHW):
@@ -435,7 +444,10 @@
     def img_prep(self, image, masks, y, *, h0, w0, H, W, pad_left, pad_top, K, mean, std):
         return self.add(IMG_PREP, 0, [h0, w0, H, W, pad_left, pad_top, K], list(mean) + list(std), [image, masks, y])
 
-    def upsample2x_add(self, g, skip, y, *, B, h, w, C, skip_group=None):
+    def upsample2x_add(self, g, skip, y, *, B, h, w, C, skip_group=None, pool=None):
+        if pool is not None:
+            assert skip_group is None and h % 2 == 0 and w % 2 == 0 and C % 8 == 0 and pool[1] >= C and pool[1] % 8 == 0
+            return self.add(UPSAMPLE2X_ADD, 0, [B, h, w, C, 0, 0, 0, int(pool[1])], [], [g, skip, y, pool[0]])
         ints = [B, h, w, C]
         if skip_group is not None and not isinstance(skip_group[0], int):
             counts, stride = skip_group
```

After: 1170 (median of 6 runs). No clear change (+0.5%).
